# cliarie/radix-join

Hardware: AMD Instinct MI355X
Metric: probe_tuples_per_sec (higher is better)
Workload: dtype int32

## Files before the change

### radix-join_amd/csrc/rj_context.hip

```cpp
#include <dlfcn.h>

#include <chrono>
#include <cstdlib>

#include "rj_internal.hpp"

namespace rj {

[[noreturn]] void launch_failed(const char* kernel, const char* what, bool unsupported) {
    throw_fmt(unsupported ? RJ_ERR_UNSUPPORTED : RJ_ERR_DEVICE, "launch %s: %s", kernel, what);
}

static int env_int(const char* name, int def) {
    const char* v = getenv(name);
    return v && *v ? atoi(v) : def;
}

void Tuning::from_env() {
    blocked_mid = env_int("RJ_TUNE_BLOCKED_MID", blocked_mid);
    mall_chunk = env_int("RJ_TUNE_MALL_CHUNK", mall_chunk);
    radix_bits = env_int("RJ_TUNE_RADIX_BITS", radix_bits);
    p1_bits = env_int("RJ_TUNE_P1_BITS", p1_bits);
    fine = env_int("RJ_TUNE_FINE", fine);
    pack = env_int("RJ_TUNE_PACK", pack);
    aos3 = env_int("RJ_TUNE_AOS3", aos3);
    aos_mid = env_int("RJ_TUNE_AOS_MID", aos_mid);
    tpg1 = env_int("RJ_TUNE_TPG1", tpg1);
    xcd_split = env_int("RJ_TUNE_XCD_SPLIT", xcd_split);
    tpg2 = env_int("RJ_TUNE_TPG2", tpg2);
    packed_side = env_int("RJ_TUNE_PACKED_SIDE", packed_side);
    xcd_min_rows = env_int("RJ_TUNE_XCD_MIN_ROWS", xcd_min_rows);
    bcast = env_int("RJ_TUNE_BCAST", bcast);
    diag = env_int("RJ_DIAG", diag);
    varchar_dev_rows = env_int("RJ_TUNE_VARCHAR_DEV", varchar_dev_rows);
    vkey_hash_bits = env_int("RJ_DEBUG_VKEY_HASH_BITS", vkey_hash_bits);
    sync_upload = env_int("RJ_SYNC_UPLOAD", sync_upload);
    wide_carry = env_int("RJ_TUNE_WIDE_CARRY", wide_carry);
    fold_owner = env_int("RJ_TUNE_FOLD_OWNER", fold_owner);
    group_grid = env_int("RJ_TUNE_GROUP_GRID", group_grid);
    win_grid = env_int("RJ_TUNE_WIN_GRID", win_grid);
    map_grid = env_int("RJ_TUNE_MAP_GRID", map_grid);
    setop_grid = env_int("RJ_TUNE_SETOP_GRID", setop_grid);
    exchange_timeout_ms = env_int("RJ_EXCHANGE_TIMEOUT_MS", exchange_timeout_ms);
    bringup_timeout_ms = env_int("RJ_BRINGUP_TIMEOUT_MS", bringup_timeout_ms);
    debug_shard_fail = env_int("RJ_DEBUG_SHARD_FAIL", debug_shard_fail);
    debug_shard_fail_rank = env_int("RJ_DEBUG_SHARD_FAIL_RANK", debug_shard_fail_rank);
    if (const char* v = getenv("RJ_DEBUG_POISON"))
        debug_poison = (int)strtol(v, nullptr, 0) & 0x1ff;
}

static size_t round_size(size_t n) {
    const size_t small = 256, big = size_t(2) << 20;
    if (n < (size_t(1) << 20)) return (n + small - 1) / small * small;
    return (n + big - 1) / big * big;
}

void* DevPool::alloc(size_t bytes) {
    size_t need = round_size(bytes ? bytes : 1);
    int    best = -1;
    for (size_t i = 0; i < blocks_.size(); ++i) {
        Block& b = blocks_[i];
        if (!b.free || b.size < need) continue;
        if (b.size > need + need / 2 + (size_t(4) << 20)) continue;
        if (best < 0 || b.size < blocks_[best].size) best = (int)i;
    }
    if (best >= 0) {
        if (poison_) {
            hipError_t e = fill(blocks_[best].p, blocks_[best].size);
            if (e != hipSuccess) throw_fmt(RJ_ERR_DEVICE, "RJ_DEBUG_POISON: fill on alloc failed: %s", hipGetErrorString(e));
        }
        blocks_[best].free = false;
        in_use_ += blocks_[best].size;
        cached_ -= blocks_[best].size;
        return blocks_[best].p;
    }
    void*      p = nullptr;
    auto       t0 = std::chrono::steady_clock::now();
    hipError_t e = hipMalloc(&p, need);
    if (e != hipSuccess) {
        (void)hipGetLastError();
        trim();
        ++n_trim;
        e = hipMalloc(&p, need);
        if (e != hipSuccess) {
            (void)hipGetLastError();
            throw_fmt(RJ_ERR_NOMEM, "hipMalloc(%zu bytes) failed: %s", need, hipGetErrorString(e));
        }
    }
    ++n_malloc;
    malloc_ms += std::chrono::duration<double, std::milli>(std::chrono::steady_clock::now() - t0).count();
    if (poison_) {
        hipError_t f = fill(p, need);
        if (f != hipSuccess) {
            (void)hipFree(p);
            throw_fmt(RJ_ERR_DEVICE, "RJ_DEBUG_POISON: fill on alloc failed: %s", hipGetErrorString(f));
        }
    }
    blocks_.push_back({p, need, false});
    in_use_ += need;
    return p;
}

hipError_t DevPool::fill(void* p, size_t bytes) {
    Context* c = owner_;
    int      prev = -1;
    if (hipGetDevice(&prev) != hipSuccess) prev = -1;
    hipError_t e = prev == c->device ? hipSuccess : hipSetDevice(c->device);
    for (hipStream_t s : {c->stream, c->aux, c->copy_stream})
        if (e == hipSuccess && s) e = hipStreamSynchronize(s);
    if (e == hipSuccess) e = hipMemsetAsync(p, poison_ & 0xff, bytes, c->stream);
    if (e == hipSuccess) e = hipStreamSynchronize(c->stream);
    if (e == hipSuccess) {
        n_fill_.fetch_add(1, std::memory_order_relaxed);
        fill_bytes_.fetch_add(bytes, std::memory_order_relaxed);
    } else {
        (void)hipGetLastError();
    }
    if (prev >= 0 && prev != c->device) (void)hipSetDevice(prev);
    return e;
}

void DevPool::release(void* p) {
    if (!p) return;
    for (Block& b : blocks_)
        if (b.p == p && !b.free) {
            if (poison_ & 0x100) (void)fill(b.p, b.size);
            b.free = true;
            in_use_ -= b.size;
            cached_ += b.size;
            return;
        }
}

void DevPool::trim() {
    std::vector<Block> keep;
    for (Block& b : blocks_) {
        if (b.free) {
            (void)hipFree(b.p);
            cached_ -= b.size;
        } else {
            keep.push_back(b);
        }
    }
    blocks_.swap(keep);
}

DevPool::~DevPool() {
    for (Block& b : blocks_) (void)hipFree(b.p);
}

Buf::Buf(Context* c, size_t n) : ctx(c), bytes(n) { p = c->pool.alloc(n); }
Buf::~Buf() {
    if (ctx && p) ctx->pool.release(p);
}

hipEvent_t Profiler::get_event() {
    if (!spare_.empty()) {
        hipEvent_t e = spare_.back();
        spare_.pop_back();
        return e;
    }
    hipEvent_t e;
    RJ_HIP(hipEventCreate(&e));
    return e;
}

static bool hot_kernel(const char* n) {
    return !strncmp(n, "pass", 4) || !strncmp(n, "join_build", 10) || !strncmp(n, "exchange", 8);
}

bool Profiler::timed(const char* name, hipEvent_t* start, hipEvent_t* stop) {
    if (!on || (level < 2 && !hot_kernel(name))) return false;
    Rec r{name, get_event(), get_event()};
    open_.push_back(r);
    *start = r.a;
    *stop = r.b;
    return true;
}

void Profiler::drain() {
    if (open_.empty()) return;
    RJ_HIP(hipStreamSynchronize(stream));
    for (Rec& r : open_) {
        float ms = 0;
// ... 161 lines not shown
```

### radix-join_amd/csrc/rj_device.hpp

```cpp
#pragma once
#include <stdint.h>

namespace rj {

constexpr uint32_t PAGE_BYTES = 8192;
constexpr uint32_t ROWS32 = 1984;
constexpr uint32_t ROWS64 = 1007;
constexpr uint32_t HDR32 = 4;
constexpr uint32_t HDR64 = 8;

enum ColKind : int32_t {
    COL_NONE  = 0,
    COL_PAGED = 1,
    COL_DENSE = 2,
    COL_IOTA  = 3
};

struct ColRef {
    const uint8_t* ptr;
    const uint8_t* valid;
    int32_t        kind;
    int32_t        width;
};

enum CarryMode : int32_t {
    CARRY_NONE   = 0,
    CARRY_ROWIDX = 1,
    CARRY_COLUMN = 2,
    CARRY_WIDE   = 3
};

enum WideLayout : int32_t {
    WIDE_NONE = 0,
    WIDE_32S  = 1,
    WIDE_64_32 = 2
};

struct TupleSrc {
    ColRef   key;
    ColRef   carry;
    uint32_t n_rows;
    int32_t  carry_mode;
    int32_t  key_f64;
    int32_t  prehashed;
    int32_t  wide;
    int32_t  pad;
    ColRef   carry2, carry3;
};

constexpr int MAX_WORDS = 4;
struct Words {
    uint32_t* w[MAX_WORDS];
};

#ifndef RJ_PT_THREADS
#define RJ_PT_THREADS 1024
#endif
#ifndef RJ_PT_ITEMS
#define RJ_PT_ITEMS 16
#endif
constexpr int PT_THREADS = RJ_PT_THREADS;
constexpr int PT_ITEMS   = RJ_PT_ITEMS;
constexpr int PT_TILE    = PT_THREADS * PT_ITEMS;
constexpr uint32_t PT_ALL_ITEMS = PT_ITEMS >= 32 ? 0xffffffffu : ((1u << (PT_ITEMS & 31)) - 1u);
#ifndef RJ_PT_CAPBITS
#define RJ_PT_CAPBITS 9
#endif
constexpr int PT_CAPBITS = RJ_PT_CAPBITS;
constexpr int PT_MAXF    = 1 << PT_CAPBITS;
constexpr int PT_MAXBITS = 9;
static_assert(PT_CAPBITS >= PT_MAXBITS && PT_CAPBITS <= 10, "fan-out capacity");
constexpr int PT_FINEBITS = 15;
constexpr int LDS_BYTES  = 160 * 1024;
static_assert(PT_THREADS >= PT_MAXF, "thread d scans digit d");
constexpr int PT_DUMMY   = 32;
static_assert(PT_TILE * 8 + (3 * PT_MAXF + PT_DUMMY) * 4 + (PT_THREADS / 64) * 4 <= LDS_BYTES,
              "scatter tile does not fit the 160 KiB of LDS");
static_assert((4 << PT_FINEBITS) <= LDS_BYTES, "fine histogram does not fit the LDS");
constexpr uint32_t PT_RANK_MASK = PT_TILE <= 16384 ? 0x3fffu : 0x7fffu;
static_assert(PT_TILE <= 32768 && PT_ITEMS % 2 == 0, "ranks and LDS positions are packed two per register");
static_assert(PT_ITEMS % 4 == 0 && PT_ITEMS <= 32, "full tiles are loaded as 16-byte vectors; one mask bit per item");

struct PassParams {
    const uint32_t* seg_off;
    const uint32_t* grp_start;
    uint32_t        nseg;
    uint32_t        n;
    uint32_t        shift;
    uint32_t        fanout_log2;
    uint32_t        tiles_per_group;
    uint32_t*       hist;
    uint32_t*       cursor;
    uint32_t        xcd_log2;
    uint32_t        xcd_remap;
    uint16_t*       side_out;
    uint32_t        next_shift, next_mask;
    const uint32_t* seg_end;
    uint32_t        oseg_shift;
    uint32_t        grp_base;
    uint32_t        hi_shift, lo_bits;
};

__host__ __device__ inline uint32_t pass_digit(const PassParams& pp, uint32_t w, uint32_t mask) {
    if (pp.hi_shift) return (((w >> pp.shift) & ((1u << pp.lo_bits) - 1u)) | ((w >> pp.hi_shift) << pp.lo_bits)) & mask;
    return (w >> pp.shift) & mask;
}

#ifndef RJ_JN_THREADS
#define RJ_JN_THREADS 512
#endif
#ifndef RJ_JN_SPT
#define RJ_JN_SPT 8
#endif
#ifndef RJ_JN_CAP
#define RJ_JN_CAP 8192
#endif
constexpr int      JN_THREADS = RJ_JN_THREADS;
constexpr int      JN_SPT     = RJ_JN_SPT;
constexpr int      JN_SUB     = JN_THREADS * JN_SPT;
constexpr int      JN_CAP     = RJ_JN_CAP;
constexpr int      JN_RMAX    = JN_CAP / 2;
constexpr int      JN_RPT     = (JN_RMAX + JN_THREADS - 1) / JN_THREADS;
constexpr int jn_threads(int table_words) { return table_words >= 3 ? 2 * JN_THREADS : JN_THREADS; }
constexpr int jn_min_waves(int table_words) {
    int blocks = (160 * 1024) / (JN_CAP * 4 * table_words + JN_CAP + 1024);
    int w = blocks * jn_threads(table_words) / 256;
    return w > 8 ? 8 : (w < 1 ? 1 : w);
}
static_assert(JN_RPT % 4 == 0 && JN_SPT % 4 == 0, "tuples are loaded as 16-byte vectors");
static_assert(JN_CAP * 4 * 4 + JN_CAP + 1024 <= 160 * 1024, "a four-array join table does not fit the LDS");
#ifndef RJ_JN_PPW
#define RJ_JN_PPW 1
#endif
#ifndef RJ_JN_PPW3
#define RJ_JN_PPW3 4
#endif
constexpr int jn_ppw(int table_words) { return table_words >= 3 ? RJ_JN_PPW3 : RJ_JN_PPW; }
#ifndef RJ_JN_HEAVY
#define RJ_JN_HEAVY 65536
#endif
constexpr uint32_t JN_HEAVY   = RJ_JN_HEAVY;
constexpr uint32_t JN_TARGET_BUILD = JN_RMAX * 3 / 4;

enum StreamMode : int32_t {
    ST_NONE    = 0,
    ST_DENSE32 = 1,
    ST_DENSE64 = 2,
    ST_PAGED32 = 3,
    ST_PAGED64 = 4,
    ST_DENSE96 = 5
};

struct OutStream {
    uint8_t* base;
    int32_t  mode;
    int32_t  pad;
};

struct JoinParams {
    Words           R, S;
    const uint32_t* offR;
    const uint32_t* offS;
    uint32_t        NP;
    uint32_t        radix_bits;
    uint32_t        n_pass;
    uint32_t        pass_bits[4];
    OutStream       key, bc, pc;
    unsigned long long* out_cursor;
    uint64_t        out_cap;
    const uint32_t* heavy_tasks;
    const uint32_t* n_heavy;
    uint32_t        heavy_grid;
    int32_t         packR, packS;
    int32_t         aosR, aosS;
    int32_t         pad;
    unsigned long long* diag;
};

struct SplitParams {
    const uint32_t* rec;
    uint32_t        cw;
    int32_t         n_cols;
    int32_t         valid_word;
    int32_t         pad;
    struct Col {
        uint8_t* out;
        uint8_t* valid;
        int32_t  word;
        int32_t  width;
        int32_t  valid_bit;
        int32_t  paged;
    } col[3];
};

struct VcRow {
    uint32_t page;
    uint32_t beg;
    uint32_t len;
};
struct VcPage {
    uint32_t first;
    uint32_t nr;
    uint32_t kind;
};
constexpr uint32_t VC_CHUNK = 512;

struct BcastParams {
    TupleSrc        R, S;
    OutStream       key, bc, pc;
    unsigned long long* out_cursor;
    uint64_t        out_cap;
};

struct FilterParams {
    TupleSrc        F, P;
    Words           Fw, Pw;
    const uint32_t* offF;
    const uint32_t* offP;
    uint32_t        NP;
    uint32_t        radix_bits;
    int32_t         packP, aosP;
    const uint32_t* heavy_tasks;
    const uint32_t* n_heavy;
    uint32_t        heavy_grid;
    int32_t         anti;
    int32_t         keyless;
    int32_t         pad;
    OutStream       key, pc;
    unsigned long long* out_cursor;
    uint64_t        out_cap;
};

constexpr uint32_t OUTER_NO_ROW = 0xffffffffu;
struct OuterParams {
    TupleSrc        B, P;
    Words           Bw, Pw;
    const uint32_t* offB;
    const uint32_t* offP;
    uint32_t        NP;
    uint32_t        radix_bits;
    int32_t         packB, aosB;
    int32_t         packP, aosP;
    const uint32_t* heavy_tasks;
    const uint32_t* n_heavy;
    uint32_t        heavy_grid;
    int32_t         keyless;
    uint32_t        pad_bc;
    int32_t         pad;
    OutStream       key, bc, pc;
    unsigned long long* out_cursor;
    uint64_t        out_cap;
};

struct FullParams {
    OuterParams     o;
    uint32_t*       flags;
    uint32_t        pad_pc;
    int32_t         use_flags;
};
// ... 160 lines not shown
```

### radix-join_amd/csrc/rj_exec.hip

```cpp
#include <algorithm>
#include <chrono>
#include <cstdlib>
#include <functional>
#include <set>

#include "rj_expr.hpp"
#include "rj_internal.hpp"
#include "rj_xplan.hpp"

namespace rj {

const NodeKind* node_kind(int kind) {
    static const NodeKind kinds[] = {
        {RJ_NODE_SCAN, "a scan", "RJ_NODE_SCAN", 0, true},
        {RJ_NODE_JOIN, "a join", "RJ_NODE_JOIN", 2, true},
        {RJ_NODE_SEMI, "a semi join", "RJ_NODE_SEMI", 2, false},
        {RJ_NODE_ANTI, "an anti join", "RJ_NODE_ANTI", 2, false},
        {RJ_NODE_OUTER, "an outer join", "RJ_NODE_OUTER", 2, false},
        {RJ_NODE_FULL, "a full outer join", "RJ_NODE_FULL", 2, false},
        {RJ_NODE_AGG, "an aggregation", "RJ_NODE_AGG", 1, false},
        {RJ_NODE_SELECT, "a selection", "RJ_NODE_SELECT", 1, false},
        {RJ_NODE_SORT, "a sort", "RJ_NODE_SORT", 1, false},
        {RJ_NODE_GROUP, "a grouping", "RJ_NODE_GROUP", 1, false},
        {RJ_NODE_WINDOW, "a window", "RJ_NODE_WINDOW", 1, false},
        {RJ_NODE_MAP, "a map", "RJ_NODE_MAP", 1, false},
        {RJ_NODE_SETOP, "a set operation", "RJ_NODE_SETOP", 2, false},
    };
    for (const NodeKind& k : kinds)
        if (k.kind == kind) return &k;
    return nullptr;
}

namespace {

template <class T>
T* ptr(const BufP& b) {
    return b ? b->as<T>() : nullptr;
}

struct DCol {
    int32_t        type = RJ_INT32;
    int32_t        kind = COL_NONE;
    int32_t        width = 4;
    const uint8_t* ptr = nullptr;
    const uint8_t* valid = nullptr;
    BufP           hold, hold_valid;
    int            vc_table = -1, vc_col = -1;
    const TableColumn* tcol = nullptr;
    ColRef ref() const { return ColRef{ptr, valid, kind, width}; }
};

struct Rel {
    uint64_t          n = 0;
    std::vector<DCol> cols;
};

struct Parted {
    int      NW = 0;
    BufP     wbuf[MAX_WORDS];
    Words    w{};
    BufP     off;
    uint32_t NP = 0;
    std::vector<uint32_t> pbits;
    bool     packed = false;
    bool     aos3 = false;
    uint64_t n_tuples = 0;
};

struct WordSrc {
    Words    w{};
    uint64_t n = 0;
    bool     packed = false;
};

struct PassShape {
    uint32_t        hi_shift = 0, lo_bits = 0;
    const uint32_t* seg_begin = nullptr;
    const uint32_t* seg_end = nullptr;
    uint32_t        nseg = 0;
    uint32_t        oseg_shift = 0;
    const uint32_t* oseg_off = nullptr;
    uint32_t        n_oseg = 0;
    std::vector<uint32_t> prior_bits;
};

struct JoinSpec {
    bool                  build_left = true;
    uint64_t              left_attr = 0, right_attr = 0;
    std::vector<uint64_t> out_idx;
    std::vector<int32_t>  out_type;
    bool                  prehashed = false;
    int                   forced_bits = 0;
    uint32_t              top_bits_taken = 0;
};

JoinSpec join_spec(const rj_node& n, int forced_bits) {
    JoinSpec js;
    js.build_left = n.build_left != 0;
    js.left_attr = n.left_attr;
    js.right_attr = n.right_attr;
    js.out_idx.assign(n.out_idx, n.out_idx + n.n_out);
    js.out_type.assign(n.out_type, n.out_type + n.n_out);
    js.forced_bits = forced_bits;
    return js;
}

struct JoinKind {
    int         node;
    const char* name;
    bool        emits_unmatched;
    bool        build_optional, probe_optional;
    int         attempts;
};
const JoinKind& join_kind(int node) {
    static const JoinKind kinds[] = {
        {RJ_NODE_JOIN, "join", false, false, false, 2},
        {RJ_NODE_SEMI, "semi join", false, false, false, 1},
        {RJ_NODE_ANTI, "anti join", true, false, false, 1},
        {RJ_NODE_OUTER, "outer join", true, true, false, 2},
        {RJ_NODE_FULL, "full outer join", true, true, true, 2},
    };
    for (const JoinKind& k : kinds)
        if (k.node == node) return k;
    throw_fmt(RJ_ERR_ARG, "bad node kind");
}

uint32_t ceil_log2(uint64_t v) {
    uint32_t b = 0;
    while ((uint64_t(1) << b) < v) ++b;
    return b;
}

class Exec {
   public:
    Exec(Context* c, const rj_plan* p, Table* const* t, uint64_t nt, int fl)
        : ctx(c), plan(p), tables(t), n_tables(nt), flags(fl), L(c->launch()) {}
    void set_fetch(TableFetch* f) { fetch = f; }

    Result* run() {
        if (!plan || plan->root >= plan->n_nodes) throw_fmt(RJ_ERR_ARG, "bad plan root");
        std::unique_ptr<Result> res(new rj_result());
        res->ctx = ctx;
        const rj_node& root = plan->nodes[plan->root];
        if (root.kind == RJ_NODE_SCAN) {
            root_scan(root, *res);
        } else {
            (void)node(plan->root, res.get(), 0);
        }
        ctx->sync();
        return res.release();
    }

    Result* run_tuples(const rj_tuples* b, const rj_tuples* p, uint32_t skip_rank_bits) {
        std::unique_ptr<Result> res(new rj_result());
        res->ctx = ctx;
        auto mk = [](const rj_tuples* t) {
            Rel r;
            r.n = t->n;
            DCol k = dense_col(RJ_INT32, BufP());
            k.ptr = static_cast<const uint8_t*>(t->key);
            DCol c = k;
            c.ptr = static_cast<const uint8_t*>(t->carry);
            r.cols = {k, c};
            return r;
        };
        if (b->n > 0xfffffff0ull || p->n > 0xfffffff0ull)
            throw_fmt(RJ_ERR_UNSUPPORTED, "more than 2^32 tuples");
        if (b->hashed != p->hashed) throw_fmt(RJ_ERR_ARG, "build/probe disagree on `hashed`");
        Rel      lb = mk(b), rp = mk(p);
        JoinSpec js;
        js.build_left = true;
        js.out_idx = {0, 1, 3};
        js.out_type = {RJ_INT32, RJ_INT32, RJ_INT32};
        js.prehashed = b->hashed != 0;
        if (skip_rank_bits > 16) throw_fmt(RJ_ERR_ARG, "skip_rank_bits > 16");
        js.top_bits_taken = js.prehashed ? skip_rank_bits : 0u;
        (void)join_core(lb, rp, js, res.get());
        ctx->sync();
        return res.release();
    }

    void run_shard(const Table* t, uint64_t key_col, uint64_t carry_col, uint32_t n_ranks,
                   rj_tuples* out, uint64_t* counts) {
        if (n_ranks == 0 || (n_ranks & (n_ranks - 1)) || n_ranks > (1u << PT_MAXBITS))
            throw_fmt(RJ_ERR_UNSUPPORTED, "n_ranks must be a power of two <= %d", 1 << PT_MAXBITS);
        if (key_col >= t->cols.size() || carry_col >= t->cols.size())
            throw_fmt(RJ_ERR_ARG, "column out of range");
        DCol k = table_col(t, (int)key_col), c = table_col(t, (int)carry_col);
        if (k.type != RJ_INT32 || c.type != RJ_INT32)
            throw_fmt(RJ_ERR_UNSUPPORTED, "sharded path carries INT32 key + INT32 payload");
        if (c.valid) throw_fmt(RJ_ERR_UNSUPPORTED, "sharded path: payload column has NULLs");
        TupleSrc src{};
        src.key = k.ref();
        src.carry = c.ref();
        src.n_rows = (uint32_t)t->num_rows;
        src.carry_mode = CARRY_COLUMN;
        if (!out->key || !out->carry) throw_fmt(RJ_ERR_ARG, "rj_shard_partition: null output buffers");
        uint32_t rb = ceil_log2(n_ranks);
        Words    ext{};
        ext.w[0] = static_cast<uint32_t*>(out->key);
        ext.w[1] = static_cast<uint32_t*>(out->carry);
        Parted P = partition(&src, nullptr, 1, 1, rb, rb ? 32 - rb : 31,  true, &ext);
        std::vector<uint32_t> off(n_ranks + 1);
        read_back(off.data(), P.off->p, (n_ranks + 1) * 4);
        for (uint32_t r = 0; r < n_ranks; ++r) counts[r] = off[r + 1] - off[r];
        out->n = off[n_ranks];
        out->hashed = 1;
        out->reserved = 0;
    }

    Context*       ctx;
    const rj_plan* plan;
    Table* const*  tables;
    uint64_t       n_tables;
    int            flags;
    TableFetch*    fetch = nullptr;
    Launch         L;
    std::map<std::pair<const Table*, int>, DCol> decoded_;
    std::map<std::pair<int, int>, std::vector<uint64_t>> vc_dir_;
// ... 55 lines not shown
        void add(uint64_t id, Make&& make) {
            if (!made.count(id)) made[id] = make();
            if (!res) {
                out.cols.push_back(made.at(id));
                return;
            }
            if (!encoded.count(id)) encoded[id] = E->col_to_result(made.at(id), out.n);
            res->cols.push_back(encoded.at(id));
        }
    };

    DCol table_col(const Table* t, int c) {
        const TableColumn& tc = t->cols[c];
        if (tc.skipped) throw_fmt(RJ_ERR_ARG, "column was not uploaded (not referenced by a scan)");
        DCol d = dense_col(tc.type, BufP());
        d.tcol = &tc;
        if (tc.type == RJ_VARCHAR) {
            d.kind = COL_IOTA;
            return d;
        }
        if (t->num_rows == 0) return d;
        if (tc.regular) {
            d.kind = COL_PAGED;
            d.ptr = tc.dev_pages;
            return d;
        }
        auto key = std::make_pair(t, c);
        auto it = decoded_.find(key);
        if (it != decoded_.end()) return it->second;
        uint64_t n = t->num_rows;
        d = new_col(tc.type, n, true);
        d.tcol = &tc;
        RJ_HIP(hipMemsetAsync(d.hold->p, 0, n * d.width, ctx->stream));
        RJ_HIP(hipMemsetAsync(d.hold_valid->p, 0, n, ctx->stream));
        if (tc.n_pages) {
            BufP row_base = ctx->buf((tc.n_pages + 1) * 4);
            launch_scan_bins(L, tc.page_rows->as<uint32_t>(), (uint32_t)tc.n_pages,
                             row_base->as<uint32_t>(), nullptr);
            launch_decode_pages(L, tc.dev_pages, (uint32_t)tc.n_pages, d.width,
                                row_base->as<uint32_t>(), n, d.hold->as<uint8_t>(),
                                d.hold_valid->as<uint8_t>());
        }
        decoded_[key] = d;
        return d;
    }

    const Table* table_of(const rj_node& n) {
        return table_by_id(n.base_table_id);
    }
    const Table* table_by_id(uint64_t id) {
        if (id >= n_tables) throw_fmt(RJ_ERR_ARG, "scan: bad base_table_id");
        return fetch ? fetch->get(id) : tables[id];
    }

    Rel scan(const rj_node& n) {
        const Table* t = table_of(n);
        Rel          r;
        r.n = t->num_rows;
        for (uint64_t k = 0; k < n.n_out; ++k) {
            uint64_t c = n.out_idx[k];
            if (c >= t->cols.size()) throw_fmt(RJ_ERR_ARG, "scan: output attr out of range");
            if (t->cols[c].type != n.out_type[k])
                throw_fmt(RJ_ERR_ARG, "scan: declared type differs from the column's type");
            DCol d = table_col(t, (int)c);
            if (d.type == RJ_VARCHAR) {
                d.vc_table = (int)n.base_table_id;
                d.vc_col = (int)c;
            }
            r.cols.push_back(d);
        }
        return r;
    }

    void root_scan(const rj_node& n, Result& res) {
        const Table* t = table_of(n);
        res.num_rows = t->num_rows;
        for (uint64_t k = 0; k < n.n_out; ++k) {
            uint64_t c = n.out_idx[k];
            if (c >= t->cols.size()) throw_fmt(RJ_ERR_ARG, "scan: output attr out of range");
            const TableColumn& tc = t->cols[c];
            if (tc.type != n.out_type[k])
                throw_fmt(RJ_ERR_ARG, "scan: declared type differs from the column's type");
            ResultColumn rc;
            rc.type = tc.type;
            if (tc.skipped) throw_fmt(RJ_ERR_ARG, "column was not uploaded");
            if (t->num_rows == 0) {
            } else if (tc.type == RJ_VARCHAR) {
                if (vc_directory((int)n.base_table_id, (int)c, t).back() == t->num_rows) {
                    rc.n_pages = tc.vc_pages.size();
                    rc.host_pages.resize(rc.n_pages * PAGE_BYTES);
                    for (uint64_t pg = 0; pg < rc.n_pages; ++pg)
                        memcpy(rc.host_pages.data() + pg * PAGE_BYTES, tc.vc_pages[pg], PAGE_BYTES);
                } else {
                    DCol d = table_col(t, (int)c);
                    d.vc_table = (int)n.base_table_id;
                    d.vc_col = (int)c;
                    BufP rowids = ctx->buf(t->num_rows * 4);
                    launch_gather(L, d.ref(), nullptr, t->num_rows, OutStream{rowids->as<uint8_t>(), ST_DENSE32, 0}, nullptr);
                    varchar_root(rowids->as<uint32_t>(), t->num_rows, d, rc);
                }
            } else if (tc.regular) {
                rc.n_pages = tc.n_pages;
                rc.dev_pages = ctx->buf(tc.n_pages * PAGE_BYTES);
                RJ_HIP(hipMemcpyAsync(rc.dev_pages->p, tc.dev_pages, tc.n_pages * PAGE_BYTES,
                                      hipMemcpyDeviceToDevice, ctx->stream));
            } else {
                rc = col_to_result(table_col(t, (int)c), t->num_rows);
            }
            res.cols.push_back(std::move(rc));
        }
    }

    Rel node(uint64_t idx, Result* root_res, int depth, bool ordered = false) {
        if (idx >= plan->n_nodes) throw_fmt(RJ_ERR_ARG, "bad node index");
        if (depth > 4096) throw_fmt(RJ_ERR_ARG, "plan too deep (cycle?)");
        const rj_node& n = plan->nodes[idx];
        if (n.kind == RJ_NODE_SCAN) return scan(n);
        const NodeKind* nk = node_kind(n.kind);
        if (nk && nk->children == 1) {
            Rel child = node(n.left, nullptr, depth + 1, n.kind == RJ_NODE_MAP && (root_res != nullptr || ordered));
            switch (n.kind) {
            case RJ_NODE_AGG: return agg(child, n, root_res);
            case RJ_NODE_SELECT: return select(child, n, root_res);
            case RJ_NODE_SORT: return sort(child, n, root_res, ordered);
            case RJ_NODE_GROUP: return group(child, n, root_res);
            case RJ_NODE_WINDOW: return window(child, n, root_res);
            case RJ_NODE_MAP: return map(child, n, root_res);
            }
        }
        if (n.kind == RJ_NODE_SETOP) {
            Rel l = node(n.left, nullptr, depth + 1);
            Rel r = node(n.right, nullptr, depth + 1);
            return setop(l, r, n, root_res);
        }
        const JoinKind& K = join_kind(n.kind);
        Rel             l = node(n.left, nullptr, depth + 1);
        Rel             r = node(n.right, nullptr, depth + 1);
        const JoinSpec  js = join_spec(n, ctx->radix_bits_override);
        if (n.kind == RJ_NODE_OUTER) return outer_join(l, r, js, K, root_res);
        if (n.kind == RJ_NODE_FULL) return full_join(l, r, js, K, root_res);
        if (n.kind != RJ_NODE_JOIN) return filter_join(l, r, js, K, root_res);
        return join_core(l, r, js, root_res);
    }

    static uint32_t tiles_per_group(uint64_t tuples_per_segment, uint64_t target_groups) {
        uint64_t k = (tuples_per_segment + (uint64_t)PT_TILE * target_groups - 1) /
                     ((uint64_t)PT_TILE * target_groups);
        return (uint32_t)std::min<uint64_t>(std::max<uint64_t>(k, 1), 8);
    }

    Parted partition(const TupleSrc* srcp, const WordSrc* ws, int KW, int CW, uint32_t bits,
                     uint32_t shift0 = 0, bool single_pass = false, const Words* external = nullptr,
                     const std::function<void(const uint32_t*)>* after_offsets = nullptr,
                     const PassShape* shape = nullptr) {
        Parted P;
        const bool preseg = shape && shape->nseg > 0;
        P.NW = KW + CW;
        const TupleSrc none{};
        const TupleSrc& src = srcp ? *srcp : none;
        const uint64_t  n = ws ? ws->n : src.n_rows;
        uint32_t       passes = single_pass ? 1 : (bits + PT_MAXBITS - 1) / PT_MAXBITS;
        if (passes == 0) passes = 1;
        std::vector<uint32_t> pbits(passes, bits / passes);
        for (uint32_t i = 0; i < bits % passes; ++i) pbits[i]++;
        if (passes == 2 && ctx->tune.p1_bits > 0) {
            uint32_t b1 = (uint32_t)ctx->tune.p1_bits;
            if (b1 < bits && b1 <= PT_CAPBITS && bits - b1 <= PT_CAPBITS) {
                pbits[0] = b1;
                pbits[1] = bits - b1;
            }
        }

        const bool fine = passes == 2 && bits <= (uint32_t)PT_FINEBITS && !external && !shape &&
                          ctx->tune.fine != 0;
        const int pack_mode = ctx->tune.pack;
        P.packed = ws ? ws->packed
                      : (!external && KW == 1 && CW == 1 && (pack_mode == 1 || (pack_mode == 2 && fine)));
        P.aos3 = KW == 1 && CW == 2 && !external && !single_pass && ctx->tune.aos3 != 0;
        const bool aos_mid = P.aos3 && passes >= 2 &&
                             (ctx->tune.aos_mid == 1 || ctx->tune.aos_mid == 3 || (ctx->tune.aos_mid == 2 && fine));
        const bool mid_side = aos_mid && !fine && ctx->tune.aos_mid != 3;
        BufP  A[MAX_WORDS], B[MAX_WORDS], AOS, MID[2], SIDE[2];
        Words wa{}, wb{}, waos{};
        if (P.aos3) {
            AOS = ctx->buf(std::max<uint64_t>(n, 1) * 12);
            waos.w[0] = AOS->as<uint32_t>();
        }
        if (aos_mid) {
            for (uint32_t k = 0; k < std::min<uint32_t>(passes - 1, 2); ++k) {
                MID[k] = ctx->buf(std::max<uint64_t>(n, 1) * 12);
                if (mid_side) SIDE[k] = ctx->buf(std::max<uint64_t>(n, 1) * 2 + 16);
            }
        }
        const bool packed_side = P.packed && !fine && passes >= 2 && ctx->tune.packed_side != 0 &&
                                 n >= (uint64_t)ctx->tune.xcd_min_rows;
        if (packed_side)
            for (uint32_t k = 0; k < std::min<uint32_t>(passes - 1, 2); ++k)
                SIDE[k] = ctx->buf(std::max<uint64_t>(n, 1) * 2 + 16);
        const int pair_word = CW >= 2 ? KW + CW - 2 : -1;
        for (int a = 0; a < (P.packed ? 1 : P.NW); ++a) {
            if (pair_word >= 0 && a == pair_word + 1) continue;
            const uint64_t wbytes = (P.packed || a == pair_word) ? 8 : 4;
            if (external) {
                wa.w[a] = external->w[a];
                continue;
            }
            if ((P.aos3 && passes == 1) || aos_mid) continue;
            A[a] = ctx->buf(n * wbytes + 2048);
            wa.w[a] = A[a]->as<uint32_t>();
            if (passes > (P.aos3 ? 2u : 1u)) {
                B[a] = ctx->buf(n * wbytes + 2048);
                wb.w[a] = B[a]->as<uint32_t>();
            }
        }
        BufP     seg_off;
        uint32_t nseg = 1, shift = shift0;
        Words    cur = ws ? ws->w : Words{}, nxt = (P.aos3 && passes == 1) ? waos : wa;
        bool     cur_is_a = false;
        BufP       fine_off, fine_cursor, coarse_off, coarse_cursor;
        uint32_t tpg_first = tiles_per_group(n, 4096);
        if (ctx->tune.tpg1 > 0) tpg_first = (uint32_t)ctx->tune.tpg1;
        bool fine_xcd = false;
        if (fine) {
            const uint32_t NB = 1u << bits, F1 = 1u << pbits[0], F2 = 1u << pbits[1];
            BufP           fh = ctx->buf((uint64_t)NB * 4);
            const uint64_t tiles = (n + PT_TILE - 1) / PT_TILE;
            uint32_t       fgrid = (uint32_t)std::min<uint64_t>(tiles, (uint64_t)ctx->compute_units());
            fine_xcd = ctx->tune.xcd_split && n >= (uint64_t)ctx->tune.xcd_min_rows && fgrid >= 8;
            if (fine_xcd) fgrid &= ~7u;
            fine_off = ctx->buf(((uint64_t)NB + 1) * 4);
            fine_cursor = ctx->buf((uint64_t)NB * 4);
            coarse_off = ctx->buf(((uint64_t)F1 + 1) * 4);
            coarse_cursor = ctx->buf((uint64_t)F1 * 4 * (fine_xcd ? 8 : 1));
            BufP coarse_x;
            RJ_HIP(hipMemsetAsync(fh->p, 0, (uint64_t)NB * 4, ctx->stream));
            if (fine_xcd) {
                coarse_x = ctx->buf((uint64_t)F1 * 8 * 4);
                RJ_HIP(hipMemsetAsync(coarse_x->p, 0, (uint64_t)F1 * 8 * 4, ctx->stream));
            }
            uint32_t* cx = fine_xcd ? coarse_x->as<uint32_t>() : nullptr;
            if (ws)
                launch_fine_hist_words(L, ws->w, ws->packed, (uint32_t)n, shift0, pbits[0], pbits[1], fgrid,
                                       fh->as<uint32_t>(), fine_xcd ? tpg_first : 0u, cx);
            else
                launch_fine_hist_src(L, src, KW, shift0, pbits[0], pbits[1], fgrid, fh->as<uint32_t>(),
                                     fine_xcd ? tpg_first : 0u, cx);
            launch_scan_fine(L, fh->as<uint32_t>(), F1, F2, fine_off->as<uint32_t>(),
                             fine_cursor->as<uint32_t>(), coarse_off->as<uint32_t>(),
                             coarse_cursor->as<uint32_t>(), cx);
        }
        struct Ev2 {
            hipEvent_t e = nullptr;
            void       make() { RJ_HIP(hipEventCreateWithFlags(&e, hipEventDisableTiming)); }
            ~Ev2() {
                if (e) (void)hipEventDestroy(e);
            }
        } chunk_ev;
        const bool chunk_second = ctx->tune.mall_chunk > 0 && passes == 2 && !fine && !shape && !ws && !external && P.packed &&
                                  !packed_side && ctx->tune.xcd_split && n >= (uint64_t)ctx->tune.xcd_min_rows;
        const bool blocked_mid = ctx->tune.blocked_mid != 0 && P.packed && passes >= 2 && !fine && !shape && !ws && !external &&
                                 !packed_side && !chunk_second;
        for (uint32_t p = 0; p < passes; ++p) {
            const uint32_t F = 1u << pbits[p];
            PassParams     pp{};
            pp.nseg = nseg;
            pp.n = (uint32_t)n;
            pp.shift = shift;
            pp.fanout_log2 = pbits[p];
            uint32_t n_groups;
            BufP     grp_start;
            const bool      first_preseg = p == 0 && preseg;
            const uint32_t  nseg_in = first_preseg ? shape->nseg : nseg;
            const uint32_t  n_oseg = first_preseg ? shape->n_oseg : nseg;
            const uint64_t  bins = (uint64_t)n_oseg * F;
            if (p == 0 && shape && shape->hi_shift) {
                pp.hi_shift = shape->hi_shift;
                pp.lo_bits = shape->lo_bits;
            }
            if (p == 0 && !preseg) {
                pp.tiles_per_group = tpg_first;
                uint64_t gt = (uint64_t)pp.tiles_per_group * PT_TILE;
                n_groups = (uint32_t)((n + gt - 1) / gt);
            } else {
                pp.tiles_per_group = tiles_per_group(n / nseg_in + 1, 16);
                if (P.aos3 && p + 1 == passes) pp.tiles_per_group = std::min<uint32_t>(pp.tiles_per_group, 2u);
                uint64_t gt = (uint64_t)pp.tiles_per_group * PT_TILE;
                if (ctx->tune.tpg2 > 0) {
                    pp.tiles_per_group = (uint32_t)ctx->tune.tpg2;
                    gt = (uint64_t)pp.tiles_per_group * PT_TILE;
                }
                n_groups = (uint32_t)(n / gt + nseg_in);
                if (ctx->tune.xcd_split && n >= (uint64_t)ctx->tune.xcd_min_rows) {
                    pp.xcd_remap = 1;
                    n_groups += 8;
                }
                const uint32_t* in_off = first_preseg ? shape->seg_begin : seg_off->as<uint32_t>();
                grp_start = ctx->buf(((uint64_t)nseg_in + 1) * 4);
                launch_group_table(L, in_off, nseg_in, (uint32_t)gt, grp_start->as<uint32_t>(),
                                   first_preseg ? shape->seg_end : nullptr);
                pp.nseg = nseg_in;
                pp.seg_off = in_off;
                pp.seg_end = first_preseg ? shape->seg_end : nullptr;
                pp.oseg_shift = first_preseg ? shape->oseg_shift : 0u;
                pp.grp_start = grp_start->as<uint32_t>();
            }
            BufP off, hist, cursor;
            if (fine) {
                off = p == 0 ? coarse_off : fine_off;
                cursor = p == 0 ? coarse_cursor : fine_cursor;
                pp.cursor = cursor->as<uint32_t>();
                pp.xcd_log2 = (p == 0 && fine_xcd) ? 3u : 0u;
            } else {
                pp.xcd_log2 = (ctx->tune.xcd_split && p == 0 && !preseg && n >= (uint64_t)ctx->tune.xcd_min_rows) ? 3u : 0u;
                hist = ctx->buf((bins << pp.xcd_log2) * 4);
                off = ctx->buf((bins + 1) * 4);
                cursor = ctx->buf((bins << pp.xcd_log2) * 4);
                RJ_HIP(hipMemsetAsync(hist->p, 0, (bins << pp.xcd_log2) * 4, ctx->stream));
                pp.hist = hist->as<uint32_t>();
                pp.cursor = cursor->as<uint32_t>();
                if (p == 1 && chunk_second) {
                    RJ_HIP(hipEventSynchronize(chunk_ev.e));
                    const uint32_t* hoff = static_cast<const uint32_t*>(ctx->small_pinned());
                    const uint64_t  gt = (uint64_t)pp.tiles_per_group * PT_TILE;
                    std::vector<uint32_t> gstart(nseg_in + 1, 0);
                    for (uint32_t sgi = 0; sgi < nseg_in; ++sgi)
                        gstart[sgi + 1] = gstart[sgi] + (uint32_t)(((uint64_t)(hoff[sgi + 1] - hoff[sgi]) + gt - 1) / gt);
                    Ev2 e_in, e_aux;
                    e_in.make();
                    e_aux.make();
                    hipStream_t aux = ctx->aux_stream();
                    RJ_HIP(hipEventRecord(e_in.e, ctx->stream));
                    RJ_HIP(hipStreamWaitEvent(aux, e_in.e, 0));
                    Launch L2 = L;
                    L2.stream = aux;
                    const uint32_t CH = (uint32_t)ctx->tune.mall_chunk;
                    uint32_t       c = 0;
                    for (uint32_t s0 = 0; s0 < nseg_in; s0 += CH, ++c) {
                        const uint32_t s1 = std::min(nseg_in, s0 + CH), G = gstart[s1] - gstart[s0];
                        const Launch& Lc = (c & 1u) ? L2 : L;
                        PassParams    pc = pp;
                        pc.nseg = s1 - s0;
                        pc.seg_off = pp.seg_off + s0;
                        pc.grp_start = pp.grp_start + s0;
                        pc.grp_base = gstart[s0];
                        pc.hist = pp.hist + (size_t)s0 * F;
                        pc.cursor = pp.cursor + (size_t)s0 * F;
                        const uint32_t grid = pp.xcd_remap ? ((G + 7u) & ~7u) : G;
                        if (G) launch_pass_hist_packed(Lc, cur.w[0], pc, grid);
                        launch_scan_segments(Lc, pc.hist, pc.seg_off, pc.nseg, F, 0, off->as<uint32_t>() + (size_t)s0 * F, pc.cursor);
                        if (G) launch_pass_scatter_packed(Lc, cur.w[0], pc, grid, nxt.w[0]);
                    }
                    RJ_HIP(hipEventRecord(e_aux.e, aux));
                    RJ_HIP(hipStreamWaitEvent(ctx->stream, e_aux.e, 0));
                    seg_off = off;
                    nseg = (uint32_t)bins;
                    shift += pbits[p];
                    cur = nxt;
                    cur_is_a = (p % 2 == 0);
                    nxt = cur_is_a ? wb : wa;
                    continue;
                }
                if (p == 0 && !ws)
                    launch_pass_hist_src(L, src, KW, pp, n_groups);
                else if ((mid_side || packed_side) && p > 0)
                    launch_pass_hist_digits(L, SIDE[(p - 1) % 2]->as<uint16_t>(), pp, n_groups);
                else if (aos_mid && p > 0)
                    launch_pass_hist_aos3(L, MID[(p - 1) % 2]->as<uint32_t>(), pp, n_groups);
                else if (P.packed && blocked_mid && p > 0)
                    launch_pass_hist_blocked(L, cur.w[0], pp, n_groups);
                else if (P.packed)
                    launch_pass_hist_packed(L, cur.w[0], pp, n_groups);
                else
                    launch_pass_hist_dense(L, cur, pp, n_groups);
                launch_scan_segments(L, pp.hist, first_preseg ? shape->oseg_off : (p == 0 ? nullptr : pp.seg_off),
                                     n_oseg, F, pp.xcd_log2, off->as<uint32_t>(), pp.cursor);
            }
            if (p == 0 && after_offsets) (*after_offsets)(off->as<uint32_t>());
            if (p == 0 && chunk_second) {
                if ((bins + 1) * 4 > Context::SMALL_PINNED / 4) throw_fmt(RJ_ERR_DEVICE, "chunked pass: too many segments");
                RJ_HIP(hipMemcpyAsync(ctx->small_pinned(), off->p, (bins + 1) * 4, hipMemcpyDeviceToHost, ctx->stream));
                chunk_ev.make();
                RJ_HIP(hipEventRecord(chunk_ev.e, ctx->stream));
            }
            if (aos_mid) {
                const bool last = p + 1 == passes;
                Words      o{};
                o.w[0] = last ? waos.w[0] : MID[p % 2]->as<uint32_t>();
                if (!last && mid_side) {
                    pp.side_out = SIDE[p % 2]->as<uint16_t>();
                    pp.next_shift = shift + pbits[p];
                    pp.next_mask = (1u << pbits[p + 1]) - 1u;
                }
                if (p == 0 && !ws)
                    launch_pass_scatter_src(L, src, KW, CW, pp, n_groups, o, true);
                else if (p == 0)
                    launch_pass_scatter_dense(L, cur, P.NW, KW, pp, n_groups, o, true);
                else
                    launch_pass_scatter_aos3(L, MID[(p - 1) % 2]->as<uint32_t>(), pp, n_groups, o.w[0]);
                nxt = o;
            } else if (P.packed) {
                if (packed_side && p + 1 < passes) {
                    pp.side_out = SIDE[p % 2]->as<uint16_t>();
                    pp.next_shift = shift + pbits[p];
                    pp.next_mask = (1u << pbits[p + 1]) - 1u;
                }
                const bool blk_out = blocked_mid && p + 1 < passes;
                if (p == 0 && !ws)
                    launch_pass_scatter_src_packed(L, src, pp, n_groups, nxt.w[0], blk_out);
                else if (blocked_mid)
                    launch_pass_scatter_blocked(L, cur.w[0], pp, n_groups, nxt.w[0], blk_out);
                else
                    launch_pass_scatter_packed(L, cur.w[0], pp, n_groups, nxt.w[0]);
            } else if (p == 0 && !ws) {
                launch_pass_scatter_src(L, src, KW, CW, pp, n_groups, nxt, P.aos3 && p + 1 == passes);
            } else {
                launch_pass_scatter_dense(L, cur, P.NW, pair_word, pp, n_groups, nxt,
                                          P.aos3 && p + 1 == passes);
            }
            seg_off = off;
            nseg = (uint32_t)bins;
            shift += pbits[p];
            cur = nxt;
            cur_is_a = (p % 2 == 0);
            nxt = cur_is_a ? wb : wa;
            if (P.aos3 && p + 2 == passes) nxt = waos;
            if (aos_mid) {
            }
        }
        P.w = cur;
        for (int a = 0; a < P.NW; ++a) P.wbuf[a] = cur_is_a ? A[a] : B[a];
        if (P.aos3) P.wbuf[0] = AOS;
        P.off = seg_off;
        P.NP = nseg;
        P.pbits = pbits;
        if (shape && !shape->prior_bits.empty()) P.pbits.insert(P.pbits.begin(), shape->prior_bits.begin(), shape->prior_bits.end());
        P.n_tuples = n;
        return P;
    }

    struct Side {
        Rel*          rel = nullptr;
        uint64_t      key_col = 0;
        std::set<int> need;
        int           carry_mode = CARRY_NONE;
        int           carry_col = -1;
        int           CW = 0;
        BufP          stream;
        int           stream_mode = ST_NONE;
        std::vector<int> wide_cols;
        int              wide = WIDE_NONE;
        int              valid_word = -1;
        BufP             vword;
        struct WideOut {
            BufP values, valid;
            int  mode = ST_NONE;
        };
        std::map<int, WideOut> wide_out;
        uint64_t null_mask = 0;
        bool     shared = false;
        bool     optional = false;
        bool     nullable(int c) const {
            if (optional || rel->cols[c].valid != nullptr) return true;
            return shared && (c >= 64 || ((null_mask >> c) & 1u));
        }
    };
    static uint64_t null_columns(const Rel& r) {
        uint64_t m = 0;
        for (size_t c = 0; c < r.cols.size() && c < 64; ++c)
            if (r.cols[c].valid != nullptr) m |= 1ull << c;
        return m;
    }

    static uint64_t pages_for(uint64_t rows, int width) {
        uint64_t rf = width == 4 ? ROWS32 : ROWS64;
        return (rows + rf - 1) / rf;
    }

    Rel empty_rel(const int32_t* types, uint64_t n_types, Result* root_res) {
        Rel r;
        r.n = 0;
        if (root_res) root_res->num_rows = 0;
        for (uint64_t k = 0; k < n_types; ++k) {
            r.cols.push_back(dense_col(types[k], BufP()));
            if (!root_res) continue;
            ResultColumn rc;
            rc.type = types[k];
            root_res->cols.push_back(std::move(rc));
        }
        return r;
    }
    Rel empty_rel(const rj_node& n, Result* root_res) { return empty_rel(n.out_type, n.n_out, root_res); }
    Rel empty_rel(const JoinSpec& js, Result* root_res) { return empty_rel(js.out_type.data(), js.out_type.size(), root_res); }

    struct JoinState {
        Side     ls, rs;
        bool     build_left = true, is_root = false, f64 = false, need_key_stream = false;
        bool     type_mismatch = false;
        size_t   lw = 0, rw = 0;
        int      KW = 1;
        uint64_t cap_hint = 0;
        const JoinKind* kind = nullptr;
        bool vkey = false;
        struct VKey {
            Rel            rel;
            BufP           rows, hash, valid;
            const uint8_t* pages = nullptr;
            uint32_t       n_pages = 0;
        } vk[2];
        Side&    bs() { return build_left ? ls : rs; }
        Side&    ps() { return build_left ? rs : ls; }
    };

    void join_prepare(Rel& left, Rel& right, const JoinSpec& js, bool is_root, JoinState& st, const JoinKind& K,
                      const uint64_t* shared_nulls = nullptr) {
        st.kind = &K;
        const size_t lw = left.cols.size(), rw = right.cols.size();
        st.lw = lw;
        st.rw = rw;
        st.is_root = is_root;
        st.build_left = js.build_left;
        if (js.left_attr >= lw || js.right_attr >= rw)
            throw_fmt(RJ_ERR_ARG, "join: key attr out of range");
        for (size_t k = 0; k < js.out_idx.size(); ++k) {
            if (js.out_idx[k] >= lw + rw) throw_fmt(RJ_ERR_ARG, "join: output attr out of range");
            const DCol& c = js.out_idx[k] < lw ? left.cols[js.out_idx[k]]
                                               : right.cols[js.out_idx[k] - lw];
            if (c.type != js.out_type[k])
                throw_fmt(RJ_ERR_ARG, "join: declared type differs from the child column's type");
        }
        Side &ls = st.ls, &rs = st.rs;
        ls.rel = &left;
        ls.key_col = js.left_attr;
        rs.rel = &right;
        rs.key_col = js.right_attr;
        if (shared_nulls) {
            ls.shared = rs.shared = true;
            ls.null_mask = shared_nulls[0];
            rs.null_mask = shared_nulls[1];
        }
        const DCol& bk = st.bs().rel->cols[st.bs().key_col];
        const DCol& pk = st.ps().rel->cols[st.ps().key_col];
        if (bk.type < RJ_INT32 || bk.type > RJ_VARCHAR) throw_fmt(RJ_ERR_ARG, "Unsupported join type");
        st.type_mismatch = pk.type != bk.type;
        st.vkey = bk.type == RJ_VARCHAR && !st.type_mismatch;
        st.KW = bk.type == RJ_INT32 ? 1 : 2;
        st.f64 = bk.type == RJ_FP64;
        const bool key_stream_ok =
            K.node == RJ_NODE_JOIN ||
            (!st.type_mismatch && !(K.emits_unmatched && st.ps().rel->cols[st.ps().key_col].valid));
        st.bs().optional = K.build_optional;
        st.ps().optional = K.probe_optional;
        for (size_t k = 0; k < js.out_idx.size(); ++k) {
            bool  is_left = js.out_idx[k] < lw;
            Side& s = is_left ? ls : rs;
            int   c = (int)(is_left ? js.out_idx[k] : js.out_idx[k] - lw);
            if ((uint64_t)c == s.key_col && !st.vkey && key_stream_ok && !s.optional)
                st.need_key_stream = true;
            else
                s.need.insert(c);
        }
        for (Side* s : {&ls, &rs}) {
            if (st.vkey) {
                s->carry_mode = CARRY_ROWIDX;
                s->CW = 1;
            } else if (s->need.empty()) {
                s->carry_mode = CARRY_NONE;
                s->CW = 0;
            } else if (s->need.size() == 1 && !s->nullable(*s->need.begin())) {
                s->carry_mode = CARRY_COLUMN;
                s->carry_col = *s->need.begin();
                s->CW = s->rel->cols[s->carry_col].width / 4;
            } else if (plan_wide_carry(*s, st.KW)) {
                s->carry_mode = CARRY_WIDE;
            } else {
                s->carry_mode = CARRY_ROWIDX;
                s->CW = 1;
            }
        }
        st.cap_hint = std::max(left.n, right.n);
    }

    bool plan_wide_carry(Side& s, int KW, bool honour_switch = true) {
        if ((honour_switch && !ctx->tune.wide_carry) || s.need.empty()) return false;
        int  words = 0, n64 = 0;
        bool any_null = false;
        for (int c : s.need) {
            const DCol& col = s.rel->cols[c];
            if (col.width != 4 && col.width != 8) return false;
            words += col.width / 4;
            n64 += col.width == 8;
            any_null = any_null || s.nullable(c);
        }
        if (any_null) ++words;
        if (words < 2 || words > MAX_WORDS - KW || n64 > 1 || (n64 == 1 && words != 3)) return false;
        s.wide_cols.clear();
        for (int c : s.need)
            if (s.rel->cols[c].width == 8) s.wide_cols.push_back(c);
        for (int c : s.need)
            if (s.rel->cols[c].width == 4) s.wide_cols.push_back(c);
        s.wide = n64 ? WIDE_64_32 : WIDE_32S;
        s.valid_word = any_null ? words - 1 : -1;
        s.CW = words;
        return true;
    }

    void prepare_wide(Side& s) {
        if (s.carry_mode != CARRY_WIDE || s.valid_word < 0 || s.rel->n == 0) return;
        const uint8_t* v[3] = {nullptr, nullptr, nullptr};
        for (size_t i = 0; i < s.wide_cols.size() && i < 3; ++i) v[i] = s.rel->cols[s.wide_cols[i]].valid;
        s.vword = ctx->buf(s.rel->n * 4);
        launch_pack_validity(L, v[0], v[1], v[2], (uint32_t)s.rel->n, s.vword->as<uint32_t>());
    }

    uint32_t join_bits(const JoinSpec& js, uint64_t build_n, uint32_t top_bits_taken = 0) {
        uint32_t bits = js.forced_bits > 0 ? (uint32_t)js.forced_bits
                                           : ceil_log2((build_n + JN_TARGET_BUILD - 1) / JN_TARGET_BUILD);
        if (js.forced_bits <= 0 && bits > 2 * PT_MAXBITS &&
            (build_n >> (2 * PT_MAXBITS)) <= (uint64_t)(JN_RMAX * 0.95))
            bits = 2 * PT_MAXBITS;
        bits = std::min<uint32_t>(std::max<uint32_t>(bits, 1), 21);
        if (top_bits_taken && bits > 32 - top_bits_taken) bits = 32 - top_bits_taken;
        return bits;
    }

    TupleSrc make_src(const JoinState& st, const Side& s, const JoinSpec& js) {
        TupleSrc src{};
        src.key = s.rel->cols[s.key_col].ref();
        src.n_rows = (uint32_t)s.rel->n;
        src.carry_mode = s.carry_mode;
        if (s.carry_mode == CARRY_COLUMN) {
            src.carry = s.rel->cols[s.carry_col].ref();
            if (src.carry.kind == COL_IOTA) src.carry_mode = CARRY_ROWIDX;
        }
        if (s.carry_mode == CARRY_WIDE) {
            ColRef refs[3] = {};
            size_t k = 0;
            for (int c : s.wide_cols) refs[k++] = s.rel->cols[c].ref();
            if (s.valid_word >= 0)
                refs[k++] = ColRef{ptr<uint8_t>(s.vword), nullptr, COL_DENSE, 4};
            src.wide = s.wide;
            src.carry = refs[0];
            src.carry2 = refs[1];
            src.carry3 = refs[2];
        }
        src.key_f64 = st.f64 ? 1 : 0;
        src.prehashed = js.prehashed ? 1 : 0;
        return src;
    }


    bool broadcast_form(JoinState& st, const JoinSpec& js) const {
        const uint64_t nb = st.bs().rel->n;
        return (nb <= (uint64_t)JN_RMAX && js.forced_bits <= 0 && !js.prehashed && ctx->tune.bcast != 0) || nb == 0 ||
               st.type_mismatch;
    }
    uint32_t stride_grid(uint64_t rows) const {
        return (uint32_t)std::min<uint64_t>((rows + JN_SUB - 1) / JN_SUB, (uint64_t)ctx->compute_units() * 8);
    }

    struct CoParts {
        Parted   B, P;
        BufP     tasks;
        uint32_t max_tasks = 0;
    };
    CoParts partition_sides(JoinState& st, const JoinSpec& js, uint32_t bits) {
        CoParts        cp;
        const TupleSrc sb = make_src(st, st.bs(), js), sp = make_src(st, st.ps(), js);
        cp.B = partition(&sb, nullptr, st.KW, st.bs().CW, bits);
        cp.P = partition(&sp, nullptr, st.KW, st.ps().CW, bits);
        return cp;
    }
    void heavy_tasks(CoParts& cp, const BufP& counters) {
        cp.max_tasks = (uint32_t)(2 * (cp.P.n_tuples / JN_HEAVY) + 2);
        cp.tasks = ctx->buf((uint64_t)cp.max_tasks * 12);
        launch_heavy_tasks_zeroed(cp.B, cp.P, cp.tasks, counters, cp.max_tasks);
    }
    CoParts co_partition(JoinState& st, const JoinSpec& js, uint32_t bits, const BufP& counters) {
        CoParts cp = partition_sides(st, js, bits);
        heavy_tasks(cp, counters);
        return cp;
    }
    BufP zeroed_counters() {
        BufP counters = ctx->buf(16);
        RJ_HIP(hipMemsetAsync(counters->p, 0, 16, ctx->stream));
        return counters;
    }
    template <class Params>
    static void set_heavy(Params& p, const CoParts& cp, const BufP& counters, uint32_t bits) {
        p.NP = cp.B.NP;
        p.radix_bits = bits;
        p.heavy_tasks = cp.tasks->as<uint32_t>();
        p.n_heavy = counters->as<uint32_t>() + 2;
        p.heavy_grid = cp.max_tasks;
    }
    static void set_parts(OuterParams& op, const CoParts& cp, const BufP& counters, uint32_t bits) {
        set_heavy(op, cp, counters, bits);
        op.Bw = cp.B.w;
        op.Pw = cp.P.w;
        op.offB = cp.B.off->as<uint32_t>();
        op.offP = cp.P.off->as<uint32_t>();
        op.packB = cp.B.packed ? 1 : 0;
        op.aosB = cp.B.aos3 ? 1 : 0;
        op.packP = cp.P.packed ? 1 : 0;
        op.aosP = cp.P.aos3 ? 1 : 0;
    }

    static OutStream out_stream(const BufP& b, int mode) { return OutStream{ptr<uint8_t>(b), mode, 0}; }
    static OutStream out_stream(const Side& s) { return out_stream(s.stream, s.stream_mode); }
    static uint64_t first_cap(uint64_t rows) { return std::min<uint64_t>(rows + 1024, 0xfffffff0ull); }

    struct Emitted {
        uint64_t        nrows = 0;
        BufP            key_stream;
        int             key_mode = ST_NONE;
        std::set<void*> finished;
    };
    template <class LaunchFn>
    Emitted emit_with_retry(JoinState& st, const BufP& counters, uint64_t cap, LaunchFn&& launch) {
        const JoinKind& K = *st.kind;
        Emitted         e;
        e.key_mode = st.need_key_stream ? stream_mode_of(st.is_root, st.KW * 4, true) : ST_NONE;
        for (int attempt = 1;; ++attempt) {
            e.key_stream = e.key_mode != ST_NONE ? ctx->buf(stream_bytes(e.key_mode, cap)) : BufP();
            for (Side* s : {&st.ls, &st.rs})
                s->stream = s->stream_mode != ST_NONE ? ctx->buf(stream_bytes(s->stream_mode, cap)) : BufP();
            if (K.attempts > 1) RJ_HIP(hipMemsetAsync(counters->p, 0, 8, ctx->stream));
            launch(out_stream(e.key_stream, e.key_mode), cap);
            e.finished.clear();
            finish_paged_streams(st, e, counters, cap);
            unsigned long long h = 0;
            read_back(&h, counters->p, 8);
            e.nrows = h;
            if (e.nrows <= cap) return e;
            if (K.attempts == 1)
                throw_fmt(RJ_ERR_DEVICE, "%s emitted %llu rows out of %llu", K.name, h, (unsigned long long)cap);
            if (e.nrows > 0xfffffff0ull) throw_fmt(RJ_ERR_UNSUPPORTED, "%s result exceeds 2^32 rows (%llu)", K.name, h);
            if (attempt == K.attempts) throw_fmt(RJ_ERR_DEVICE, "%s output overflowed twice", K.name);
            cap = e.nrows;
        }
    }

    Rel join_core(Rel& left, Rel& right, const JoinSpec& js, Result* root_res) {
        if (left.n == 0 || right.n == 0) return empty_rel(js, root_res);
        JoinState st;
        join_prepare(left, right, js, root_res != nullptr, st, join_kind(RJ_NODE_JOIN));
        if (st.type_mismatch) return empty_rel(js, root_res);
        if (st.vkey) hash_varchar_keys(st);
        prepare_wide(st.ls);
        prepare_wide(st.rs);
        Side&          bs = st.bs();
        Side&          ps = st.ps();
        const uint32_t bits = join_bits(js, bs.rel->n, js.top_bits_taken);
        if (ctx->tune.diag >= 2)
            fprintf(stderr, "[rj diag] join build=%llu probe=%llu bits=%u cw=%d/%d\n",
                    (unsigned long long)bs.rel->n, (unsigned long long)ps.rel->n, bits, bs.CW, ps.CW);
        if (broadcast_form(st, js)) return join_finish(st, js, nullptr, bits, root_res);
        CoParts cp = partition_sides(st, js, bits);
        return join_finish(st, js, &cp, bits, root_res);
    }

    Rel join_finish(JoinState& st, const JoinSpec& js, CoParts* cp, uint32_t bits, Result* root_res) {
        Side &    bs = st.bs(), &ps = st.ps();
        const int KW = st.KW;
        BufP counters = ctx->buf(16);
        if (cp) heavy_tasks(*cp, counters);
        plan_carry_streams(st);
        Emitted e = emit_with_retry(st, counters, first_cap(st.cap_hint), [&](const OutStream& key, uint64_t cap) {
            if (!cp) {
                BcastParams bp{};
                bp.R = make_src(st, bs, js);
                bp.S = make_src(st, ps, js);
                bp.key = key;
                bp.bc = out_stream(bs);
                bp.pc = out_stream(ps);
                bp.out_cursor = counters->as<unsigned long long>();
                bp.out_cap = cap;
                launch_join_bcast(L, KW, bs.CW, ps.CW, bp, stride_grid(ps.rel->n));
                return;
            }
            const Parted &PB = cp->B, &PP = cp->P;
            JoinParams    jp{};
            set_heavy(jp, *cp, counters, bits);
            jp.R = PB.w;
            jp.S = PP.w;
            jp.packR = PB.packed ? 1 : 0;
            jp.packS = PP.packed ? 1 : 0;
            jp.aosR = PB.aos3 ? 1 : 0;
            jp.aosS = PP.aos3 ? 1 : 0;
            jp.offR = PB.off->as<uint32_t>();
            jp.offS = PP.off->as<uint32_t>();
            jp.n_pass = (uint32_t)PB.pbits.size();
            for (size_t i = 0; i < PB.pbits.size() && i < 4; ++i) jp.pass_bits[i] = PB.pbits[i];
            jp.key = key;
            jp.bc = out_stream(bs);
            jp.pc = out_stream(ps);
            jp.out_cursor = counters->as<unsigned long long>();
            jp.out_cap = cap;
            BufP diag;
            if (ctx->tune.diag) {
                diag = ctx->buf(16 * 8);
                RJ_HIP(hipMemsetAsync(diag->p, 0, 16 * 8, ctx->stream));
                jp.diag = diag->as<unsigned long long>();
            }
            const uint32_t ppw = join_partitions_per_workgroup(KW, bs.CW, jp);
            launch_join(L, KW, bs.CW, ps.CW, jp, cp->max_tasks + (PB.NP + ppw - 1) / ppw);
            if (diag) {
                unsigned long long hd[16];
                read_back(hd, diag->p, sizeof hd);
                static const char* names[] = {"loads issued", "table clear", "build", "count/probe",
                                              "prefix+barrier", "reserve", "emit"};
                double tot = 0;
                for (int i = 0; i < 7; ++i) tot += (double)hd[i];
                fprintf(stderr, "[rj diag] join phases (cycles of thread 0, summed over %u workgroups):\n", PB.NP);
                for (int i = 0; i < 7; ++i)
                    fprintf(stderr, "[rj diag]   %-16s %6.1f %%  %8.0f cyc/wg\n", names[i],
                            100.0 * hd[i] / tot, (double)hd[i] / PB.NP);
            }
        });
        if (st.vkey && e.nrows) e.nrows = verify_varchar_pairs(st, e.nrows);
        return join_assemble(st, js, e, root_res);
    }

    Rel filter_join(Rel& left, Rel& right, const JoinSpec& js, const JoinKind& K, Result* root_res) {
        const bool   anti = K.node == RJ_NODE_ANTI;
        Rel&         fil = js.build_left ? left : right;
        Rel&         pre = js.build_left ? right : left;
        const size_t lw = left.cols.size();
        for (uint64_t o : js.out_idx)
            if (o < lw + right.cols.size() && (o < lw) == js.build_left)
                throw_fmt(RJ_ERR_ARG, "%s: output attr %llu names a column of the filter side", K.name,
                          (unsigned long long)o);
        const uint64_t fattr = js.build_left ? js.left_attr : js.right_attr;
        if (fattr < fil.cols.size() && fil.cols[fattr].type == RJ_VARCHAR)
            throw_fmt(RJ_ERR_UNSUPPORTED, "%s on a VARCHAR key", K.name);
        if (pre.n == 0 || (!anti && fil.n == 0)) return empty_rel(js, root_res);
        JoinState st;
        join_prepare(left, right, js, root_res != nullptr, st, K);
        if (st.type_mismatch && !anti) return empty_rel(js, root_res);
        Side&     fs = st.bs();
        Side&     ps = st.ps();
        const int KW = st.KW;
        prepare_wide(ps);
        plan_carry_streams(st);
        const bool     bcast = broadcast_form(st, js);
        const uint32_t bits = join_bits(js, fs.rel->n);
        if (ctx->tune.diag >= 2)
            fprintf(stderr, "[rj diag] %s filter=%llu preserved=%llu %s bits=%u cw=%d\n", K.name,
                    (unsigned long long)fs.rel->n, (unsigned long long)ps.rel->n, bcast ? "broadcast" : "partitioned",
                    bits, ps.CW);

        FilterParams fp{};
        fp.anti = anti ? 1 : 0;
        fp.keyless = st.type_mismatch ? 1 : 0;
        fp.P = make_src(st, ps, js);
        if (bcast && !fp.keyless) fp.F = make_src(st, fs, js);
        BufP counters = zeroed_counters();
        fp.out_cursor = counters->as<unsigned long long>();
        CoParts cp;
        if (!bcast) {
            cp = co_partition(st, js, bits, counters);
            set_heavy(fp, cp, counters, bits);
            fp.Fw = cp.B.w;
            fp.Pw = cp.P.w;
            fp.offF = cp.B.off->as<uint32_t>();
            fp.offP = cp.P.off->as<uint32_t>();
            fp.packP = cp.P.packed ? 1 : 0;
            fp.aosP = cp.P.aos3 ? 1 : 0;
        }
        Emitted e = emit_with_retry(st, counters, ps.rel->n, [&](const OutStream& key, uint64_t cap) {
            fp.key = key;
            fp.pc = out_stream(ps);
            fp.out_cap = cap;
            if (bcast) {
                launch_filter_bcast(L, KW, ps.CW, fp, stride_grid(ps.rel->n));
            } else {
                launch_filter_join(L, KW, ps.CW, fp, cp.max_tasks + cp.B.NP);
                if (anti && (fp.P.key.valid || fp.P.key_f64))
                    launch_filter_nullkeys(L, KW, ps.CW, fp, stride_grid(ps.rel->n));
            }
        });
        return join_assemble(st, js, e, root_res);
    }

    Rel outer_join(Rel& left, Rel& right, const JoinSpec& js, const JoinKind& K, Result* root_res) {
        Rel&           opt = js.build_left ? left : right;
        Rel&           pre = js.build_left ? right : left;
        const uint64_t oattr = js.build_left ? js.left_attr : js.right_attr;
        if (oattr < opt.cols.size() && opt.cols[oattr].type == RJ_VARCHAR)
            throw_fmt(RJ_ERR_UNSUPPORTED, "%s on a VARCHAR key", K.name);
        if (pre.n == 0) return empty_rel(js, root_res);
        JoinState st;
        join_prepare(left, right, js, root_res != nullptr, st, K);
        return outer_probe(st, js, root_res);
    }

    Rel full_join(Rel& left, Rel& right, const JoinSpec& js_in, const JoinKind& K, Result* root_res) {
        for (int side = 0; side < 2; ++side) {
            const Rel&     r = side == 0 ? left : right;
            const uint64_t a = side == 0 ? js_in.left_attr : js_in.right_attr;
            if (a < r.cols.size() && r.cols[a].type == RJ_VARCHAR)
                throw_fmt(RJ_ERR_UNSUPPORTED, "%s on a VARCHAR key", K.name);
        }
        if (left.n == 0 && right.n == 0) {
            JoinState chk;
            join_prepare(left, right, js_in, root_res != nullptr, chk, K);
            refuse_varchar_outputs(chk);
            return empty_rel(js_in, root_res);
        }
        JoinSpec js = js_in;
        if ((js.build_left ? right : left).n == 0) js.build_left = !js.build_left;
        JoinState st;
        join_prepare(left, right, js, root_res != nullptr, st, K);
        return outer_probe(st, js, root_res);
    }

    static void refuse_varchar_outputs(JoinState& st) {
        for (Side* s : {&st.ls, &st.rs})
            for (int c : s->need) {
                if (!s->optional || s->rel->cols[c].type != RJ_VARCHAR) continue;
                if (st.kind->probe_optional)
                    throw_fmt(RJ_ERR_UNSUPPORTED,
                              "full outer join: a VARCHAR column in the output is not supported (%s child column %d)",
                              s == &st.ls ? "left" : "right", c);
                throw_fmt(RJ_ERR_UNSUPPORTED,
                          "outer join: a VARCHAR column of the optional side in the output is not supported "
                          "(child column %d)", c);
            }
    }

    Rel outer_probe(JoinState& st, const JoinSpec& js, Result* root_res) {
        const bool full = st.kind->probe_optional;
        Side&      bs = st.bs();
        Side&      ps = st.ps();
        const int  KW = st.KW;
        refuse_varchar_outputs(st);
        prepare_wide(bs);
        prepare_wide(ps);
        plan_carry_streams(st);
        const bool     bcast = broadcast_form(st, js);
        const uint32_t bits = join_bits(js, bs.rel->n);
        if (ctx->tune.diag >= 2)
            fprintf(stderr, "[rj diag] %s %s=%llu %s=%llu %s bits=%u cw=%d/%d\n", st.kind->name, full ? "built" : "optional",
                    (unsigned long long)bs.rel->n, full ? "probed" : "preserved", (unsigned long long)ps.rel->n,
                    bcast ? "broadcast" : "partitioned", bits, bs.CW, ps.CW);

        FullParams   fp{};
        OuterParams& op = fp.o;
        op.keyless = st.type_mismatch ? 1 : 0;
        op.pad_bc = bs.carry_mode == CARRY_ROWIDX ? OUTER_NO_ROW : 0u;
        op.P = make_src(st, ps, js);
        if (full || !op.keyless) op.B = make_src(st, bs, js);
        BufP counters = zeroed_counters();
        op.out_cursor = counters->as<unsigned long long>();
        CoParts cp;
        if (!bcast) {
            cp = co_partition(st, js, bits, counters);
            set_parts(op, cp, counters, bits);
        }
        BufP flags;
        if (full) {
            fp.pad_pc = ps.carry_mode == CARRY_ROWIDX ? OUTER_NO_ROW : 0u;
            const uint64_t flag_bytes = ((bcast ? (uint64_t)JN_RMAX : cp.B.n_tuples) / 32 + 2) * 4;
            flags = ctx->buf(flag_bytes);
            RJ_HIP(hipMemsetAsync(flags->p, 0, flag_bytes, ctx->stream));
            fp.flags = flags->as<uint32_t>();
            fp.use_flags = bcast ? 1 : 0;
        }
        const uint32_t probe_grid = stride_grid(ps.rel->n), build_grid = stride_grid(bs.rel->n);
        const uint64_t rows0 = std::max(st.cap_hint, full ? bs.rel->n + ps.rel->n : ps.rel->n);
        Emitted e = emit_with_retry(st, counters, first_cap(rows0), [&](const OutStream& key, uint64_t cap) {
            op.key = key;
            op.bc = out_stream(bs);
            op.pc = out_stream(ps);
            op.out_cap = cap;
            const bool probe_dropped = !bcast && (op.P.key.valid || op.P.key_f64);
            if (!full) {
                if (bcast)
                    launch_outer_bcast(L, KW, bs.CW, ps.CW, op, probe_grid);
                else
                    launch_outer_join(L, KW, bs.CW, ps.CW, op, cp.max_tasks + cp.B.NP);
                if (probe_dropped) launch_outer_nullkeys(L, KW, ps.CW, op, probe_grid);
            } else if (bcast) {
                launch_full_bcast(L, KW, bs.CW, ps.CW, fp, probe_grid);
                launch_full_buildrows(L, KW, bs.CW, fp, build_grid);
            } else {
                launch_full_join(L, KW, bs.CW, ps.CW, fp, cp.max_tasks + cp.B.NP);
                launch_full_unmatched(L, KW, bs.CW, fp, build_grid);
                if (probe_dropped) launch_outer_nullkeys(L, KW, ps.CW, op, probe_grid);
                if (op.B.key.valid || op.B.key_f64) launch_full_buildrows(L, KW, bs.CW, fp, build_grid);
            }
        });
        return join_assemble(st, js, e, root_res);
    }

    struct AggOut {
        uint32_t func;
        int      col;
        int      slot;
    };
    uint32_t agg_bits(uint64_t rows) const {
        uint32_t bits = ctx->radix_bits_override > 0 ? (uint32_t)ctx->radix_bits_override
                                                     : ceil_log2((rows + AGG_TARGET - 1) / AGG_TARGET);
        return std::min<uint32_t>(std::max<uint32_t>(bits, 1), 21);
    }
    Rel agg(Rel& child, const rj_node& n, Result* root_res) {
        const size_t cw = child.cols.size();
        if (n.left_attr >= cw) throw_fmt(RJ_ERR_ARG, "aggregation: key attr out of range");
        const DCol& kc = child.cols[n.left_attr];
        if (kc.type != RJ_INT32 && kc.type != RJ_INT64)
            throw_fmt(RJ_ERR_UNSUPPORTED, "aggregation on %s key: group keys are INT32 or INT64",
                      kc.type == RJ_FP64 ? "an FP64" : "a VARCHAR");
        Side s;
        s.rel = &child;
        s.key_col = n.left_attr;
        std::vector<AggOut> outs;
        for (uint64_t k = 0; k < n.n_out; ++k) {
            const uint32_t func = RJ_AGG_FUNC(n.out_idx[k]);
            const uint64_t col = RJ_AGG_COL(n.out_idx[k]);
            const int32_t  type = n.out_type[k];
            if (func == RJ_AGG_FSUM) throw_fmt(RJ_ERR_ARG, "aggregation: RJ_AGG_FSUM is RJ_NODE_GROUP's, this kind has no FP64 sum");
            if (func > RJ_AGG_MAX) throw_fmt(RJ_ERR_ARG, "aggregation: unknown function code %u", func);
            int32_t expect = RJ_INT64;
            if (func == RJ_AGG_COUNT_STAR) {
                if (col != 0) throw_fmt(RJ_ERR_ARG, "aggregation: COUNT(*) takes no column");
            } else {
                if (col >= cw) throw_fmt(RJ_ERR_ARG, "aggregation: output attr out of range");
                const DCol& c = child.cols[col];
                if (func == RJ_AGG_KEY) {
                    if (col != n.left_attr) throw_fmt(RJ_ERR_ARG, "aggregation: RJ_AGG_KEY names another column than the key");
                    expect = kc.type;
                } else {
                    if (c.type != RJ_INT32 && c.type != RJ_INT64)
                        throw_fmt(RJ_ERR_UNSUPPORTED, "aggregation over %s column (child column %llu): INT32 and INT64 only",
                                  c.type == RJ_FP64 ? "an FP64" : "a VARCHAR", (unsigned long long)col);
                    if (func == RJ_AGG_MIN || func == RJ_AGG_MAX) expect = c.type;
                    s.need.insert((int)col);
                }
            }
            if (type != expect) throw_fmt(RJ_ERR_ARG, "aggregation: declared type differs from the function's result type");
            outs.push_back(AggOut{func, (int)col, -1});
        }
        const int KW = kc.type == RJ_INT32 ? 1 : 2;
        if (s.need.empty()) {
            s.carry_mode = CARRY_NONE;
            s.CW = 0;
        } else if (s.need.size() == 1 && !s.nullable(*s.need.begin())) {
            s.carry_mode = CARRY_COLUMN;
            s.carry_col = *s.need.begin();
            s.CW = child.cols[s.carry_col].width / 4;
            s.wide_cols = {s.carry_col};
        } else if (plan_wide_carry(s, KW, false)) {
            s.carry_mode = CARRY_WIDE;
        } else {
            int words = 0;
            bool any_null = false;
            for (int c : s.need) {
                words += child.cols[c].width / 4;
                any_null = any_null || s.nullable(c);
            }
            throw_fmt(RJ_ERR_UNSUPPORTED,
                      "aggregation: the aggregated columns take %d carry words; at most %d travel behind an %s key (every "
                      "distinct column its width, one more word if any is nullable, at most one 64-bit column next to "
                      "another word)",
                      words + (any_null ? 1 : 0), MAX_WORDS - KW, KW == 1 ? "INT32" : "INT64");
        }
        if (child.n == 0) return empty_rel(n, root_res);
        check_rows(child);
        for (AggOut& o : outs)
            for (size_t i = 0; i < s.wide_cols.size(); ++i)
                if (o.func >= RJ_AGG_COUNT && s.wide_cols[i] == o.col) o.slot = (int)i;

        AggParams ap{};
        ap.n_cols = (int32_t)s.wide_cols.size();
        ap.valid_word = s.valid_word;
        bool need_key = false, need_rows = false;
        {
            int word = 0;
            for (int i = 0; i < ap.n_cols; ++i) {
                const DCol& c = child.cols[s.wide_cols[i]];
                ap.col[i].word = word;
                ap.col[i].width = c.width;
                ap.col[i].valid_bit = s.valid_word >= 0 ? i : -1;
                word += c.width / 4;
            }
            for (const AggOut& o : outs) {
                need_key = need_key || o.func == RJ_AGG_KEY;
                need_rows = need_rows || o.func == RJ_AGG_COUNT_STAR;
                if (o.slot < 0) continue;
                const bool nullable = s.nullable(o.col);
                uint32_t&  need = ap.col[o.slot].need;
                if (o.func == RJ_AGG_COUNT || nullable) need |= AGG_NEED_COUNT;
                if (o.func == RJ_AGG_SUM) need |= AGG_NEED_SUM;
                if (o.func == RJ_AGG_MIN) need |= AGG_NEED_MIN;
                if (o.func == RJ_AGG_MAX) need |= AGG_NEED_MAX;
            }
        }
        prepare_wide(s);
        const TupleSrc src = make_src(JoinState(), s, JoinSpec());
        const uint32_t bits = agg_bits(child.n);
        const uint64_t cap = child.n + 1;
        if (ctx->tune.diag >= 2)
            fprintf(stderr, "[rj diag] aggregation rows=%llu bits=%u cw=%d cols=%d\n", (unsigned long long)child.n, bits, s.CW,
                    ap.n_cols);

        struct Arrays {
            BufP key, keyvalid, rows, nn[AGG_MAX_COLS], sum[AGG_MAX_COLS], mn[AGG_MAX_COLS], mx[AGG_MAX_COLS];
        } O, M;
        auto fill = [](AggArrays& a, const Arrays& b) {
            a.key = ptr<uint8_t>(b.key);
            a.rows = ptr<unsigned long long>(b.rows);
            for (int i = 0; i < AGG_MAX_COLS; ++i) {
                a.nn[i] = ptr<unsigned long long>(b.nn[i]);
                a.sum[i] = ptr<unsigned long long>(b.sum[i]);
                a.mn[i] = ptr<long long>(b.mn[i]);
                a.mx[i] = ptr<long long>(b.mx[i]);
            }
        };
        if (need_key) O.key = ctx->buf(cap * KW * 4);
        if (need_key && kc.valid) O.keyvalid = ctx->buf(cap);
        if (need_rows) O.rows = ctx->buf(cap * 8);
        for (int i = 0; i < ap.n_cols; ++i) {
            if (ap.col[i].need & AGG_NEED_COUNT) O.nn[i] = ctx->buf(cap * 8);
            if (ap.col[i].need & AGG_NEED_SUM) O.sum[i] = ctx->buf(cap * 8);
            if (ap.col[i].need & AGG_NEED_MIN) O.mn[i] = ctx->buf(cap * 8);
            if (ap.col[i].need & AGG_NEED_MAX) O.mx[i] = ctx->buf(cap * 8);
        }
        fill(ap.out, O);
        ap.out_keyvalid = ptr<uint8_t>(O.keyvalid);
        ap.out_cap = cap;
        ap.src = src;

        uint64_t nrows = 0;
        for (int attempt = 0;; ++attempt) {
            BufP counters = zeroed_counters();
            Parted P = partition(&src, nullptr, KW, s.CW, bits);
            const uint32_t max_tasks = (uint32_t)(2 * (P.n_tuples / JN_HEAVY) + 2);
            BufP           tasks = ctx->buf((uint64_t)max_tasks * 12);
            launch_heavy_tasks(L, P.off->as<uint32_t>(), P.off->as<uint32_t>(), P.NP, tasks->as<uint32_t>(),
                               counters->as<uint32_t>() + 2, max_tasks);
            uint32_t n_heavy = 0;
            read_back(&n_heavy, counters->as<uint32_t>() + 2, 4);
            n_heavy = std::min(n_heavy, max_tasks);
            uint64_t heavy_tuples = std::min<uint64_t>(P.n_tuples, (uint64_t)n_heavy * JN_HEAVY);
            if (attempt == 0) heavy_tuples = std::min<uint64_t>(heavy_tuples, 1u << 20);
// ... 1831 lines not shown
```

### radix-join_amd/csrc/rj_internal.hpp

```cpp
#pragma once
#include <hip/hip_runtime.h>

#include <atomic>
#include <cstdarg>
#include <cstdio>
#include <cstring>
#include <functional>
#include <map>
#include <memory>
#include <mutex>
#include <stdexcept>
#include <string>
#include <vector>

#include "../../include/rj.h"
#include "rj_comm.hpp"
#include "rj_device.hpp"
#include "rj_kernels.hpp"

namespace rj {

struct Context;

struct Error : std::runtime_error {
// ... 7 lines not shown
    va_start(ap, fmt);
    vsnprintf(buf, sizeof buf, fmt, ap);
    va_end(ap);
    throw Error(code, buf);
}

#define RJ_HIP(expr)                                                                          \
    do {                                                                                      \
        hipError_t _e = (expr);                                                               \
        if (_e != hipSuccess)                                                                 \
            ::rj::throw_fmt(_e == hipErrorOutOfMemory ? RJ_ERR_NOMEM : RJ_ERR_DEVICE,         \
                            "%s failed: %s (%s:%d)", #expr, hipGetErrorString(_e), __FILE__, \
                            __LINE__);                                                        \
    } while (0)

class DevPool {
   public:
    void* alloc(size_t bytes);
    void  release(void* p);
    void     set_poison(Context* owner, int mode) { owner_ = owner, poison_ = mode; }
    int      poison() const { return poison_; }
    uint64_t n_fills() const { return n_fill_.load(std::memory_order_relaxed); }
    uint64_t bytes_filled() const { return fill_bytes_.load(std::memory_order_relaxed); }
    void  trim();
    ~DevPool();
    size_t bytes_in_use() const { return in_use_; }
    size_t bytes_cached() const { return cached_; }
    uint64_t n_malloc = 0, n_trim = 0;
    double   malloc_ms = 0;

   private:
    struct Block {
        void*  p;
        size_t size;
        bool   free;
    };
    std::vector<Block> blocks_;
    size_t             in_use_ = 0, cached_ = 0;
    Context*           owner_ = nullptr;
    int                poison_ = 0;
    std::atomic<uint64_t> n_fill_{0}, fill_bytes_{0};
    hipError_t         fill(void* p, size_t bytes);
};

struct Buf {
    Context* ctx = nullptr;
    void*    p = nullptr;
    size_t   bytes = 0;
    Buf(Context* c, size_t n);
    ~Buf();
    Buf(const Buf&) = delete;
    Buf& operator=(const Buf&) = delete;
    template <class T>
    T* as() const {
        return reinterpret_cast<T*>(p);
    }
};
using BufP = std::shared_ptr<Buf>;

class Profiler {
   public:
    bool        on = false;
    int         level = 1;
    hipStream_t stream = nullptr;
    bool        timed(const char* name, hipEvent_t* start, hipEvent_t* stop);
    void        drain();
    void        reset();
    struct Tot {
        uint64_t launches = 0;
        double   ms = 0;
    };
    std::map<std::string, Tot> totals;
    std::vector<std::string>   order;
    ~Profiler();

   private:
    struct Rec {
        const char* name;
        hipEvent_t  a, b;
    };
    std::vector<Rec>        open_;
    std::vector<hipEvent_t> spare_;
    hipEvent_t              get_event();
};

class LaunchLog {
   public:
    bool on = false;
    void add(const void* kernel);
    void clear();
    void merge_into(std::map<std::string, uint64_t>& out);

   private:
    std::mutex                         mu_;
    std::map<const void*, uint64_t>    counts_;
    std::map<const void*, std::string> names_;
};

struct TableColumn {
    int32_t  type = 0;
    uint64_t n_pages = 0;
    const uint8_t* dev_pages = nullptr;
    BufP           owned;
    bool           regular = false;
    uint64_t       page_rows_total = 0;
    BufP           page_rows;
    std::vector<uint32_t> page_rows_host;
    std::vector<uint8_t>        host_pages;
    std::vector<const uint8_t*> vc_pages;
    mutable BufP vc_dev, vc_dev_dir;
    bool                        skipped = false;
};

struct Table {
    Context*                 ctx = nullptr;
    uint64_t                 num_rows = 0;
    std::vector<TableColumn> cols;
};

struct ResultColumn {
    int32_t              type = 0;
    uint64_t             n_pages = 0;
    BufP                 dev_pages;
    std::vector<uint8_t> host_pages;
    struct Part {
        Context* ctx;
        BufP     pages;
        uint64_t n_pages;
    };
    std::vector<Part> more;
    uint64_t          n_first = 0;
};

struct Result {
    Context*                  ctx = nullptr;
    uint64_t                  num_rows = 0;
    std::vector<ResultColumn> cols;
};

struct Tuning {
    int blocked_mid = 1;
    int mall_chunk = 0;
    int radix_bits = 0;
    int p1_bits = 0;
    int fine = 1;
    int pack = 1;
    int aos3 = 1;
    int aos_mid = 2;
    int tpg1 = 0;
    int packed_side = 0;
    int tpg2 = 0;
    int xcd_min_rows = 40 << 20;
    int xcd_split = 1;
    int bcast = 1;
    int diag = 0;
    int varchar_dev_rows = 200000;
    int vkey_hash_bits = 0;
    int sync_upload = 0;
    int wide_carry = 1;
    int fold_owner = 1;
    int group_grid = 0;
    int map_grid = 0;
    int win_grid = 0;
    int setop_grid = 0;
    int exchange_timeout_ms = 120000;
    int bringup_timeout_ms = 0;
    int debug_shard_fail = 0, debug_shard_fail_rank = 0;
    int debug_poison = 0;
    void from_env();
};

struct Context {
    Tuning      tune;
    int         device = 0;
    hipStream_t stream = nullptr;
    bool        own_stream = false;
    int         radix_bits_override = 0;
    DevPool     pool;
    Profiler    prof;
    LaunchLog   klog;
    std::string last_error;
    void*  pinned = nullptr;
    size_t pinned_bytes = 0;
    static constexpr size_t SMALL_PINNED = 32768;
    void*  pinned_small = nullptr;
    void*  small_pinned();
    hipStream_t copy_stream = nullptr;
    void*       pinned_up = nullptr;
    size_t      pinned_up_bytes = 0;
    hipStream_t upload_stream();
    hipStream_t aux = nullptr;
    hipStream_t aux_stream();
    void*       upload_staging(size_t bytes);
    Launch launch() {
        Launch L;
        L.stream = stream;
        L.self = this;
        L.timed = prof.on ? [](void* s, const char* n, hipEvent_t* a, hipEvent_t* b) {
            return static_cast<Context*>(s)->prof.timed(n, a, b);
        } : (bool (*)(void*, const char*, hipEvent_t*, hipEvent_t*)) nullptr;
        L.logged = klog.on ? [](void* s, const void* k) { static_cast<Context*>(s)->klog.add(k); }
                           : (void (*)(void*, const void*)) nullptr;
        return L;
    }
    std::vector<Context*>  peers;
    std::unique_ptr<Comm>  comm;
    Context*               group = nullptr;
    int                    n_lanes() const { return 1 + (int)peers.size(); }
    Context*               lane(int i) { return i == 0 ? this : peers[(size_t)i - 1]; }
    int   n_cu = 0;
    int   compute_units();
    void  prewarm();
    BufP  buf(size_t bytes) { return std::make_shared<Buf>(this, bytes ? bytes : 16); }
    void* staging(size_t bytes);
    void  sync() { RJ_HIP(hipStreamSynchronize(stream)); }
    ~Context();
};

struct TableFetch {
    virtual Table* get(uint64_t id) = 0;
    virtual ~TableFetch() = default;
};

Result* execute_plan(Context* ctx, const rj_plan* plan, Table* const* tables, uint64_t n_tables,
                     int flags, TableFetch* fetch = nullptr);
Result* join_tuples(Context* ctx, const rj_tuples* build, const rj_tuples* probe,
                    uint32_t skip_rank_bits, int flags);
void    execute_sharded(Context* group, const rj_plan* plan, Table* const* tables, uint64_t n_inputs,
                        int flags, Result** out);
bool    plan_shardable(const rj_plan* plan, std::string* why);
struct NodeKind {
    int         kind;
    const char* name;
    const char* token;
    int         children;
    bool        sharded;
};
const NodeKind* node_kind(int kind);
void    shard_partition(Context* ctx, const Table* t, uint64_t key_col, uint64_t carry_col,
                        uint32_t n_ranks, rj_tuples* out, uint64_t* counts);

struct MapOp;
struct MapExpr {
    int32_t f64;
    bool    nullable;
};
void map_check(const rj_expr_op* ops, uint64_t n_ops, uint64_t n_cols, const int32_t* col_type, const uint8_t* col_nullable,
               std::vector<MapOp>& dev_ops, std::vector<MapExpr>& exprs);
void map_eval_row(const rj_expr_op* ops, uint64_t n_ops, uint64_t n_cols, const int32_t* col_type, const uint64_t* col_bits,
                  const uint8_t* col_null, uint64_t out_cap, uint64_t* out_bits, uint8_t* out_null, int32_t* out_kind, uint64_t* n_out);

Table* table_upload(Context* ctx, const rj_input* host, const std::vector<bool>* col_used = nullptr,
                    bool borrow_varchar = false);
class AsyncUpload : public TableFetch {
   public:
    AsyncUpload(Context* ctx, const rj_plan* plan, const std::vector<bool>& used,
                const std::vector<std::vector<bool>>& col_used);
    ~AsyncUpload() override;
    Table* get(uint64_t id) override;
    double busy_ms() const { return busy_ms_; }
    double wait_ms() const { return wait_ms_; }

   private:
    struct Impl;
    std::unique_ptr<Impl> im_;
    double                busy_ms_ = 0, wait_ms_ = 0;
};
Table* table_adopt(Context* ctx, uint64_t num_rows, uint64_t n_cols, const int32_t* types,
                   const void* const* dev_pages, const uint64_t* n_pages);
void   result_copy_pages(Result* r, uint64_t col, void* const* dst, uint64_t n_dst);
void   upload_host_pages(Context* ctx, const uint8_t* const* pages, uint64_t n_pages, uint8_t* dev);
Result* execute_host_sharded(Context* group, const rj_plan* plan, const std::vector<bool>& used,
                             const std::vector<std::vector<bool>>& col_used);

Table*   table_from_csv(Context* ctx, const char* text, uint64_t n_bytes, uint64_t n_cols, const int32_t* col_type,
                        const rj_filter_op* filter, uint64_t n_filter_ops);
int parse_fp64_host(const char* s, uint64_t n, uint64_t* bits);
uint64_t table_col_pages(const Table* t, uint64_t col);
void     table_copy_pages(Context* ctx, const Table* t, uint64_t col, void* const* dst, uint64_t n_dst);

void parallel_for(size_t n, size_t grain, const std::function<void(size_t, size_t)>& fn);

void copy_page(void* dst, const void* src);
void copy_pages_fence();

void varchar_dir_build(const uint8_t* const* pages, uint64_t n_pages, uint64_t num_rows,
                       std::vector<uint64_t>& row_base);
void varchar_gather_encode(const uint8_t* const* pages, uint64_t n_pages,
                           const std::vector<uint64_t>& row_base, const uint32_t* idx, uint64_t n,
                           std::vector<uint8_t>& out_pages, uint64_t& n_out_pages);

}

struct rj_context : rj::Context {};
struct rj_table : rj::Table {};
struct rj_result : rj::Result {};
```

### radix-join_amd/csrc/rj_kernels.hpp

```cpp
#pragma once
#include <hip/hip_runtime.h>

#include "rj_device.hpp"

namespace rj {

struct Launch {
    hipStream_t stream;
    bool (*timed)(void* self, const char* name, hipEvent_t* start, hipEvent_t* stop);
    void* self;
    void (*logged)(void* self, const void* kernel);
};

[[noreturn]] void launch_failed(const char* kernel, const char* what, bool unsupported);

void launch_page_headers(const Launch& L, const uint8_t* pages, uint32_t n_pages, uint32_t rows_full,
                         uint32_t* page_rows, unsigned long long* flags);
void launch_rows_beyond(const Launch& L, const uint8_t* pages, uint32_t n_pages,
                        const uint32_t* row_base, uint64_t num_rows, unsigned long long* flag);
void launch_decode_pages(const Launch& L, const uint8_t* pages, uint32_t n_pages, int width,
                         const uint32_t* row_base, uint64_t num_rows, uint8_t* values,
                         uint8_t* valid);

void launch_gather(const Launch& L, const ColRef& src, const uint32_t* idx, uint64_t n,
                   const OutStream& dst, uint8_t* dst_valid);
void launch_outer_gather(const Launch& L, const ColRef& src, const uint32_t* idx, uint64_t n, uint8_t* dst,
                         uint8_t* dst_valid);
void launch_finish_pages(const Launch& L, uint8_t* pages, uint64_t n_rows, int width);
void launch_finish_streams(const Launch& L, uint8_t* const* pages, const int* widths, uint32_t n,
                           const unsigned long long* n_rows_dev, uint64_t cap_rows);
void launch_encode_nullable(const Launch& L, const uint8_t* values, const uint8_t* valid,
                            uint64_t n_rows, int width, uint8_t* pages);
void launch_pack_validity(const Launch& L, const uint8_t* v0, const uint8_t* v1, const uint8_t* v2, uint32_t n,
                          uint32_t* out);
void launch_split_records(const Launch& L, const SplitParams& sp, uint64_t n);
void launch_debug_stall(const Launch& L, uint32_t ms);

void launch_scan_bins(const Launch& L, const uint32_t* in, uint32_t n, uint32_t* off,
                      uint32_t* cursor);
void launch_scan_segments(const Launch& L, const uint32_t* hist, const uint32_t* seg_off,
                          uint32_t nseg, uint32_t F, uint32_t xcd_log2, uint32_t* off, uint32_t* cursor);
void launch_group_table(const Launch& L, const uint32_t* seg_off, uint32_t nseg,
                        uint32_t group_tuples, uint32_t* grp_start, const uint32_t* seg_end = nullptr);

void launch_pass_hist_src(const Launch& L, const TupleSrc& src, int key_words, const PassParams& pp,
                          uint32_t n_groups);
void launch_fine_hist_src(const Launch& L, const TupleSrc& src, int key_words, uint32_t shift,
                          uint32_t b1, uint32_t b2, uint32_t grid, uint32_t* fine, uint32_t xcd_tpg = 0,
                          uint32_t* coarse_x = nullptr);
void launch_fine_hist_words(const Launch& L, const Words& in, bool packed, uint32_t n, uint32_t shift,
                            uint32_t b1, uint32_t b2, uint32_t grid, uint32_t* fine, uint32_t xcd_tpg = 0,
                            uint32_t* coarse_x = nullptr);
void launch_scan_fine(const Launch& L, const uint32_t* fine, uint32_t F1, uint32_t F2,
                      uint32_t* off2, uint32_t* cursor2, uint32_t* off1, uint32_t* cursor1,
                      const uint32_t* coarse_x = nullptr);
void launch_pass_scatter_src(const Launch& L, const TupleSrc& src, int key_words, int carry_words,
                             const PassParams& pp, uint32_t n_groups, const Words& out, bool aos3 = false);
void launch_pass_hist_dense(const Launch& L, const Words& in, const PassParams& pp,
                            uint32_t n_groups);
void launch_pass_scatter_dense(const Launch& L, const Words& in, int n_words, int pair_word,
                               const PassParams& pp, uint32_t n_groups, const Words& out, bool aos3 = false);

void launch_pass_hist_digits(const Launch& L, const uint16_t* digits, const PassParams& pp, uint32_t n_groups);
void launch_pass_hist_aos3(const Launch& L, const uint32_t* in_tuples, const PassParams& pp, uint32_t n_groups);
void launch_pass_scatter_aos3(const Launch& L, const uint32_t* in_tuples, const PassParams& pp, uint32_t n_groups,
                              uint32_t* out_tuples);

void launch_pass_hist_packed(const Launch& L, const uint32_t* in_pairs, const PassParams& pp,
                             uint32_t n_groups);
void launch_pass_scatter_src_packed(const Launch& L, const TupleSrc& src, const PassParams& pp,
                                    uint32_t n_groups, uint32_t* out_pairs, bool blocked_out = false);
void launch_pass_hist_blocked(const Launch& L, const uint32_t* in_blocked, const PassParams& pp, uint32_t n_groups);
void launch_pass_scatter_blocked(const Launch& L, const uint32_t* in_blocked, const PassParams& pp, uint32_t n_groups,
                                 uint32_t* out_pairs, bool blocked_out);
void launch_pass_scatter_packed(const Launch& L, const uint32_t* in_pairs, const PassParams& pp,
                                uint32_t n_groups, uint32_t* out_pairs);

void launch_heavy_tasks(const Launch& L, const uint32_t* offR, const uint32_t* offS, uint32_t NP,
                        uint32_t* tasks, uint32_t* n_heavy, uint32_t max_tasks);

uint32_t join_partitions_per_workgroup(int key_words, int cw_build, const JoinParams& jp);
void launch_join(const Launch& L, int key_words, int cw_build, int cw_probe, const JoinParams& jp,
                 uint32_t grid);

void launch_join_bcast(const Launch& L, int key_words, int cw_build, int cw_probe,
                       const BcastParams& bp, uint32_t grid);

void launch_filter_bcast(const Launch& L, int key_words, int cw_preserved, const FilterParams& fp, uint32_t grid);
void launch_filter_join(const Launch& L, int key_words, int cw_preserved, const FilterParams& fp, uint32_t grid);
void launch_filter_nullkeys(const Launch& L, int key_words, int cw_preserved, const FilterParams& fp, uint32_t grid);

void launch_outer_bcast(const Launch& L, int key_words, int cw_optional, int cw_preserved, const OuterParams& op,
                        uint32_t grid);
void launch_outer_join(const Launch& L, int key_words, int cw_optional, int cw_preserved, const OuterParams& op,
                       uint32_t grid);
void launch_outer_nullkeys(const Launch& L, int key_words, int cw_preserved, const OuterParams& op, uint32_t grid);

void launch_full_bcast(const Launch& L, int key_words, int cw_optional, int cw_preserved, const FullParams& fp,
                       uint32_t grid);
void launch_full_join(const Launch& L, int key_words, int cw_optional, int cw_preserved, const FullParams& fp,
                      uint32_t grid);
void launch_full_unmatched(const Launch& L, int key_words, int cw_built, const FullParams& fp, uint32_t grid);
void launch_full_buildrows(const Launch& L, int key_words, int cw_built, const FullParams& fp, uint32_t grid);

void launch_agg_merge_init(const Launch& L, const AggParams& ap, uint32_t grid);
void launch_agg_parts(const Launch& L, int key_words, int carry_words, const AggParams& ap, uint32_t grid);
void launch_agg_nullkey(const Launch& L, int carry_words, const AggParams& ap, uint32_t grid);
void launch_agg_emit(const Launch& L, int key_words, const AggParams& ap, uint32_t grid);
void launch_agg_column(const Launch& L, const unsigned long long* src, const unsigned long long* nn, uint64_t n, int width,
                       uint8_t* dst, uint8_t* dst_valid);

void launch_select(const Launch& L, const SelectProg* prog, uint32_t n_ops, uint32_t n_rows, uint32_t* out_ids,
                   unsigned long long* cursor, uint32_t grid);

struct MapProg;
void launch_map(const Launch& L, const MapProg* prog, uint32_t n_ops, uint32_t n_rows, uint32_t grid);

void launch_sort_encode(const Launch& L, const ColRef& col, const uint32_t* perm, uint32_t n_rows, bool f64, int32_t flags,
                        uint8_t* keys_out, uint32_t* hist, uint32_t grid);
void launch_sort_count(const Launch& L, int mode, const uint8_t* keys, const uint32_t* ids, const uint8_t* valid, uint32_t null_digit,
                       uint32_t n_rows, uint32_t shift, uint32_t* table);
void launch_sort_scan(const Launch& L, const uint32_t* hist, uint32_t n_rows, uint32_t* table);
void launch_sort_scatter(const Launch& L, int mode, const uint8_t* keys_in, const uint32_t* ids_in, const uint8_t* valid,
                         uint32_t null_digit, uint32_t n_rows, uint32_t shift, const uint32_t* table, uint8_t* keys_out,
                         uint32_t* ids_out);
void launch_sort_iota(const Launch& L, uint32_t* out, uint32_t base, uint32_t n);

void launch_group_heads(const Launch& L, const ColRef& col, const uint32_t* perm, uint32_t n_rows, bool f64, bool first, bool last,
                        unsigned long long* masks, uint32_t* tile_heads);
void launch_group_scan(const Launch& L, const uint32_t* tile_heads, uint32_t n_rows, uint32_t* tile_base, uint32_t* total);
void launch_group_keys(const Launch& L, const ColRef& col, const uint32_t* perm, uint32_t n_rows, bool f64,
                       const unsigned long long* masks, const uint32_t* tile_base, uint32_t n_groups, uint8_t* out, uint8_t* out_valid);
void launch_group_reduce(const Launch& L, const ColRef* col, const uint32_t* perm, uint32_t n_rows, bool f64,
                         const unsigned long long* masks, const uint32_t* tile_base, uint32_t n_groups, const GroupAcc& acc,
                         uint32_t max_grid);
void launch_group_column(const Launch& L, const unsigned long long* src, const unsigned long long* nn, uint64_t n, int decode, int width,
                         uint8_t* dst, uint8_t* dst_valid);

uint64_t fsum_scratch_bytes(uint32_t n_rows, uint32_t max_grid);
void     launch_fsum(const Launch& L, const ColRef& col, const uint32_t* perm, uint32_t n_rows, const unsigned long long* masks,
                     const uint32_t* tile_base, uint32_t n_groups, unsigned long long* out, uint32_t max_grid, uint8_t* scratch);

void launch_win_one_head(const Launch& L, unsigned long long* masks, uint32_t n_rows);
void launch_win_ranks(const Launch& L, const unsigned long long* P, const unsigned long long* Q, uint32_t n_rows, const WinMarks& m,
                      const WinRanks& out, uint32_t max_chunk);
void launch_win_scan(const Launch& L, const ColRef& col, const uint32_t* perm, uint32_t n_rows, bool f64, const unsigned long long* P,
                     const WinTails& tails, const WinScan& out, uint32_t max_chunk);
void launch_win_column(const Launch& L, const unsigned long long* src, const uint32_t* nn, const uint32_t* peer_end, uint64_t n, int decode,
                       int width, uint8_t* dst, uint8_t* dst_valid);

void launch_setop_concat(const Launch& L, const ColRef& l, const ColRef& r, uint32_t n_left, uint64_t n, const OutStream& dst,
                         uint8_t* dst_valid);
void launch_setop_runs(const Launch& L, const uint32_t* perm, uint32_t n_rows, uint32_t n_left, const unsigned long long* masks,
                       const uint32_t* tile_base, uint32_t n_runs, uint32_t* tile_left, uint32_t* tile_lbase, const SetopRuns& runs,
                       uint32_t max_grid);
void launch_setop_offsets(const Launch& L, const SetopRuns& runs, uint32_t n_runs, int op, uint32_t* tile_m, uint32_t* tile_mbase,
                          uint32_t* off, uint32_t* total, uint32_t max_grid);
void launch_setop_emit(const Launch& L, const uint32_t* off, uint32_t n_runs, uint32_t n_out, uint32_t* run_of, uint32_t max_grid);

void launch_vc_resolve(const Launch& L, const uint8_t* pages, uint32_t n_pages, const uint32_t* row_base,
                       const uint32_t* rowids, uint32_t n, VcRow* out);
void launch_vc_hash(const Launch& L, const uint8_t* pages, uint32_t n_pages, const uint32_t* row_base,
                    const uint32_t* rowids, uint32_t n, VcRow* rows, uint64_t* hash, uint8_t* valid,
                    uint64_t hash_mask = ~0ull);
void launch_vc_verify(const Launch& L, const uint8_t* pages_b, uint32_t np_b, const VcRow* rows_b,
                      const uint8_t* pages_p, uint32_t np_p, const VcRow* rows_p, const uint32_t* bidx,
                      const uint32_t* pidx, uint32_t n, uint8_t* keep, unsigned long long* n_bad);
void launch_vc_compact(const Launch& L, const uint8_t* keep, const uint32_t* bidx, const uint32_t* pidx, uint32_t n,
                       uint32_t* out_b, uint32_t* out_p, unsigned long long* cursor);
void launch_vc_walk(const Launch& L, const VcRow* rows, uint32_t n, uint32_t* pages_in_chunk,
                    const uint32_t* page_base, VcPage* page_out);
void launch_vc_encode(const Launch& L, const uint8_t* pages, uint32_t n_pages, const VcRow* rows,
                      const VcPage* plist, uint32_t n_out_pages, uint8_t* out);

void prewarm_pages(const Launch& L, uint32_t* zeroed);
void prewarm_partition(const Launch& L, uint32_t* zeroed);
void prewarm_join(const Launch& L, uint32_t* zeroed);
void prewarm_bcast(const Launch& L, uint32_t* zeroed);
void prewarm_filter(const Launch& L, uint32_t* zeroed);
void prewarm_outer(const Launch& L, uint32_t* zeroed);
void prewarm_full(const Launch& L, uint32_t* zeroed);
void prewarm_agg(const Launch& L, uint32_t* zeroed);
void prewarm_select(const Launch& L, uint32_t* zeroed);
void prewarm_varchar_dev(const Launch& L, uint32_t* zeroed);

}
```

### radix-join_amd/csrc/rj_partition.hip

```cpp
#include <hip/hip_ext.h>

#include "rj_kernels.hpp"
#include "rj_kernel_util.hpp"
#include "rj_tuple_util.hpp"

#include <algorithm>
#include <type_traits>

namespace rj {

template <int MODE>
__global__ __launch_bounds__(1024) void k_scan_bins(const uint32_t* in, const uint32_t* in_end, uint32_t n,
                                                    uint32_t div, uint32_t* off, uint32_t* cursor) {
    __shared__ uint32_t s_wsum[16];
    const uint32_t      chunk = (n + 1023u) / 1024u;
    const uint32_t      b = threadIdx.x * chunk;
    const uint32_t      e = min(n, b + chunk);
    uint32_t            sum = 0;
    for (uint32_t i = b; i < e; ++i) {
        uint32_t v = MODE == 0 ? in[i] : ((in_end ? in_end[i] : in[i + 1]) - in[i] + div - 1u) / div;
        sum += v;
    }
    uint32_t total;
    uint32_t run = block_excl_scan(sum, s_wsum, total);
// ... 486 lines not shown
    }
    template <int NW>
    __device__ __forceinline__ uint32_t issue_tile(uint32_t base, uint32_t end,
                                                   uint32_t (&w)[PT_ITEMS][NW]) const {
        static_assert(NW == KW + CW, "word count");
        const bool vec = base + PT_TILE <= end;
        uint32_t   lo[PT_ITEMS], hi[PT_ITEMS];
        const uint32_t tid = tile_tid();
        uint32_t       ok = raw_keys(vec, base, end, lo, hi, tid);
        if constexpr (WIDE == WIDE_32S) {
            uint32_t c0[PT_ITEMS];
            load_col32_any(s.carry, vec, base, end, c0, tid);
#pragma unroll
            for (int j = 0; j < PT_ITEMS; ++j) w[j][KW] = c0[j];
            load_col32_any(s.carry2, vec, base, end, c0, tid);
#pragma unroll
            for (int j = 0; j < PT_ITEMS; ++j) w[j][KW + 1] = c0[j];
            if constexpr (CW == 3) {
                load_col32_any(s.carry3, vec, base, end, c0, tid);
#pragma unroll
                for (int j = 0; j < PT_ITEMS; ++j) w[j][KW + 2] = c0[j];
            }
        } else if constexpr (WIDE == WIDE_64_32) {
            uint32_t c0[PT_ITEMS], c1[PT_ITEMS];
            load_col64(s.carry, vec, base, end, c0, c1, tid);
#pragma unroll
            for (int j = 0; j < PT_ITEMS; ++j) {
                w[j][KW] = c0[j];
                w[j][KW + 1] = c1[j];
            }
            load_col32_any(s.carry2, vec, base, end, c0, tid);
#pragma unroll
            for (int j = 0; j < PT_ITEMS; ++j) w[j][KW + 2] = c0[j];
        } else if constexpr (CW == 1) {
            if (s.carry_mode == CARRY_ROWIDX) {
#pragma unroll
                for (int j = 0; j < PT_ITEMS; ++j) w[j][KW] = item_row(vec, base, j, tid);
            } else {
                uint32_t c0[PT_ITEMS];
                load_col32(s.carry, vec, base, end, c0, tid);
#pragma unroll
                for (int j = 0; j < PT_ITEMS; ++j) w[j][KW] = c0[j];
            }
        } else if constexpr (CW >= 2) {
            uint32_t c0[PT_ITEMS], c1[PT_ITEMS];
            load_col64(s.carry, vec, base, end, c0, c1, tid);
#pragma unroll
            for (int j = 0; j < PT_ITEMS; ++j) {
                w[j][KW] = c0[j];
                w[j][KW + 1] = c1[j];
            }
        }
#pragma unroll
        for (int j = 0; j < PT_ITEMS; ++j) {
            w[j][0] = lo[j];
            if constexpr (KW == 2) w[j][1] = hi[j];
        }
        return ok;
    }
    template <int NW>
    __device__ __forceinline__ uint32_t finish_tile(uint32_t base, uint32_t end, uint32_t ok,
                                                    uint32_t (&w)[PT_ITEMS][NW]) const {
        const bool vec = base + PT_TILE <= end;
        uint32_t   lo[PT_ITEMS], hi[PT_ITEMS];
#pragma unroll
        for (int j = 0; j < PT_ITEMS; ++j) {
            lo[j] = w[j][0];
            hi[j] = KW == 2 ? w[j][KW - 1] : 0u;
        }
        ok = drop_invalid(vec, base, end, ok, tile_tid());
        ok = hash_keys(ok, lo, hi);
#pragma unroll
        for (int j = 0; j < PT_ITEMS; ++j) {
            w[j][0] = lo[j];
            if constexpr (KW == 2) w[j][1] = hi[j];
        }
        return ok;
    }
    template <int NW>
    __device__ __forceinline__ uint32_t load_tile(uint32_t base, uint32_t end,
                                                  uint32_t (&w)[PT_ITEMS][NW]) const {
        return finish_tile<NW>(base, end, issue_tile<NW>(base, end, w), w);
    }
};

__device__ __forceinline__ bool group_range(const PassParams& pp, uint32_t g, uint32_t& seg,
                                            uint32_t& begin, uint32_t& end) {
    const uint32_t gt = pp.tiles_per_group * (uint32_t)PT_TILE;
    if (pp.seg_off == nullptr) {
        seg = 0;
        uint64_t b = (uint64_t)g * gt;
        if (b >= pp.n) return false;
        begin = (uint32_t)b;
        end = (uint32_t)min((uint64_t)pp.n, b + gt);
        return true;
    }
    const uint32_t G = pp.grp_start[pp.nseg] - pp.grp_base;
    if (pp.xcd_remap) {
        const uint32_t per = (G + 7u) >> 3;
        if ((g >> 3) >= per) return false;
        g = (g & 7u) * per + (g >> 3);
    }
    if (g >= G) return false;
    uint32_t lo = 0, hi = pp.nseg;
    while (hi - lo > 1) {
        uint32_t mid = (lo + hi) >> 1;
        if (pp.grp_start[mid] - pp.grp_base <= g)
            lo = mid;
        else
            hi = mid;
    }
    seg = lo >> pp.oseg_shift;
    uint32_t gi = g - (pp.grp_start[lo] - pp.grp_base);
    uint64_t b = (uint64_t)pp.seg_off[lo] + (uint64_t)gi * gt;
    begin = (uint32_t)b;
    end = (uint32_t)min((uint64_t)(pp.seg_end ? pp.seg_end[lo] : pp.seg_off[lo + 1]), b + gt);
    return begin < end;
}

template <class L, class = void>
struct loader_needs_begin : std::false_type {};
template <class L>
struct loader_needs_begin<L, std::enable_if_t<L::kNeedsBegin>> : std::true_type {};

template <class Loader>
__global__ __launch_bounds__(PT_THREADS) void k_pass_hist(Loader ld, PassParams pp) {
    __shared__ uint32_t s_h[PT_MAXF];
    uint32_t            seg, begin, end;
    if (!group_range(pp, blockIdx.x, seg, begin, end)) return;
    const uint32_t F = 1u << pp.fanout_log2, mask = F - 1u;
    for (uint32_t d = threadIdx.x; d < F; d += PT_THREADS) s_h[d] = 0;
    lds_barrier();
    for (uint32_t base = begin; base < end; base += PT_TILE) {
        uint32_t hk[PT_ITEMS];
        uint32_t ok;
        if constexpr (loader_needs_begin<Loader>::value)
            ok = ld.key_tile(base, begin, end, hk);
        else
            ok = ld.key_tile(base, end, hk);
#pragma unroll
        for (int j = 0; j < PT_ITEMS; ++j) {
            if ((ok >> j) & 1u) atomicAdd(&s_h[pass_digit(pp, hk[j], mask)], 1u);
        }
    }
    if constexpr (loader_needs_begin<Loader>::value) {
        uint32_t hx;
        if (ld.extra(begin, end, hx)) atomicAdd(&s_h[pass_digit(pp, hx, mask)], 1u);
    }
    lds_barrier();
    for (uint32_t d = threadIdx.x; d < F; d += PT_THREADS) {
        uint32_t c = s_h[d];
        if (c) atomicAdd(&pp.hist[(((size_t)seg * F + d) << pp.xcd_log2) | (blockIdx.x & ((1u << pp.xcd_log2) - 1u))], c);
    }
}

template <class Loader>
__global__ __launch_bounds__(PT_THREADS) void k_fine_hist(Loader ld, uint32_t n, uint32_t shift,
                                                          uint32_t b1, uint32_t b2,
                                                          uint32_t* fine, uint32_t xcd_tpg,
                                                          uint32_t* coarse_x) {
    __shared__ uint32_t s_f[1u << PT_FINEBITS];
    const uint32_t      NB = 1u << (b1 + b2), m1 = (1u << b1) - 1u, m2 = (1u << b2) - 1u;
    for (uint32_t d = threadIdx.x; d < NB; d += PT_THREADS) s_f[d] = 0;
    lds_barrier();
    const uint32_t tiles = (uint32_t)(((uint64_t)n + PT_TILE - 1) / PT_TILE);
    const uint32_t x = blockIdx.x & 7u, gstride = gridDim.x >> 3;
    uint32_t       gk = blockIdx.x >> 3, gj = 0;
    auto           tile_of = [&](uint32_t k, uint32_t j) { return (x + 8u * k) * xcd_tpg + j; };
    auto           advance = [&](uint32_t t) -> uint32_t {
        if (!xcd_tpg) return t + gridDim.x;
        if (++gj < xcd_tpg && tile_of(gk, gj) < tiles) return tile_of(gk, gj);
        gk += gstride;
        gj = 0;
        const uint64_t nt = (uint64_t)(x + 8ull * gk) * xcd_tpg;
        return nt < tiles ? (uint32_t)nt : 0xffffffffu;
    };
    uint32_t t = xcd_tpg ? tile_of(gk, 0) : blockIdx.x;
    uint32_t lo[PT_ITEMS], hi[PT_ITEMS], raw = 0;
    if (t < tiles) raw = ld.issue_keys(t * (uint32_t)PT_TILE, n, lo, hi);
    while (t < tiles) {
        const uint32_t ok = ld.finish_keys(t * (uint32_t)PT_TILE, n, raw, lo, hi);
        uint32_t       q[PT_ITEMS];
#pragma unroll
        for (int j = 0; j < PT_ITEMS; ++j) {
            const uint32_t h = lo[j] >> shift;
            q[j] = ((h & m1) << b2) | ((h >> b1) & m2);
        }
        const uint32_t t2 = advance(t);
        if (t2 < tiles) raw = ld.issue_keys(t2 * (uint32_t)PT_TILE, n, lo, hi);
#pragma unroll
        for (int j = 0; j < PT_ITEMS; ++j)
            if ((ok >> j) & 1u) atomicAdd(&s_f[q[j]], 1u);
        t = t2;
    }
    lds_barrier();
    for (uint32_t d = threadIdx.x; d < NB; d += PT_THREADS) {
        uint32_t c = s_f[d];
        if (c) atomicAdd(&fine[d], c);
    }
    if (xcd_tpg) {
        const uint32_t F2 = 1u << b2;
        for (uint32_t d1 = threadIdx.x; d1 <= m1; d1 += PT_THREADS) {
            uint32_t sum = 0;
            for (uint32_t i = 0; i < F2; ++i) sum += s_f[d1 * F2 + ((i + d1) & m2)];
            if (sum) atomicAdd(&coarse_x[(d1 << 3) | x], sum);
        }
    }
}

__global__ __launch_bounds__(PT_MAXF) void k_scan_fine(const uint32_t* fine, uint32_t F1,
                                                       uint32_t F2, uint32_t* off2,
                                                       uint32_t* cursor2, uint32_t* off1,
                                                       uint32_t* cursor1, const uint32_t* coarse_x) {
    __shared__ uint32_t s_wsum[PT_MAXF / 64];
    const uint32_t      d1 = blockIdx.x, below = d1 * F2;
    uint32_t            sum = 0;
    if ((F2 & 3u) == 0) {
        const uint4* f4 = reinterpret_cast<const uint4*>(fine);
        for (uint32_t i = threadIdx.x; i < below / 4; i += PT_MAXF) {
            const uint4 v = f4[i];
            sum += v.x + v.y + v.z + v.w;
        }
    } else {
        for (uint32_t i = threadIdx.x; i < below; i += PT_MAXF) sum += fine[i];
    }
    uint32_t base, tot;
    (void)block_excl_scan(sum, s_wsum, base);
    lds_barrier();
    const uint32_t v = threadIdx.x < F2 ? fine[below + threadIdx.x] : 0u;
    const uint32_t ex = block_excl_scan(v, s_wsum, tot);
    if (threadIdx.x < F2) {
        off2[below + threadIdx.x] = base + ex;
        cursor2[below + threadIdx.x] = base + ex;
    }
    if (threadIdx.x == 0) {
        off1[d1] = base;
        if (coarse_x) {
            uint32_t at = base;
            for (uint32_t x = 0; x < 8; ++x) {
                cursor1[(d1 << 3) | x] = at;
                at += coarse_x[(d1 << 3) | x];
            }
        } else {
            cursor1[d1] = base;
        }
        if (d1 + 1 == F1) {
            off1[F1] = base + tot;
            off2[(size_t)F1 * F2] = base + tot;
        }
    }
}

template <int NW>
__device__ __forceinline__ void rank_tile(const PassParams& pp, uint32_t mask, uint32_t ok,
                                          const uint32_t (&w)[PT_ITEMS][NW], uint32_t* s_cnt,
                                          uint32_t (&rk)[PT_ITEMS / 2]) {
    const uint32_t dummy = PT_MAXF + (threadIdx.x & (PT_DUMMY - 1));
    uint32_t       r[PT_ITEMS];
#pragma unroll
    for (int j = 0; j < PT_ITEMS; ++j) {
        const uint32_t m = 0u - ((ok >> j) & 1u);
        r[j] = atomicAdd(&s_cnt[(pass_digit(pp, w[j][0], mask) & m) | (dummy & ~m)], 1u);
    }
#pragma unroll
    for (int j = 0; j < PT_ITEMS; j += 2)
        rk[j / 2] = (r[j] & PT_RANK_MASK) | ((r[j + 1] & PT_RANK_MASK) << 16);
}
constexpr uint32_t PT_NO_POS = 0xffffu;
template <int NW>
__device__ __forceinline__ void place_tile(const PassParams& pp, uint32_t mask, uint32_t ok,
                                           const uint32_t (&w)[PT_ITEMS][NW], const uint32_t* s_base,
                                           uint32_t (&rk)[PT_ITEMS / 2]) {
    uint32_t b[PT_ITEMS];
#pragma unroll
    for (int j = 0; j < PT_ITEMS; ++j) b[j] = s_base[pass_digit(pp, w[j][0], mask)];
#pragma unroll
    for (int j = 0; j < PT_ITEMS; j += 2) {
        const uint32_t p0 = ((ok >> j) & 1u) ? b[j] + (rk[j / 2] & 0xffffu) : PT_NO_POS;
        const uint32_t p1 = ((ok >> (j + 1)) & 1u) ? b[j + 1] + (rk[j / 2] >> 16) : PT_NO_POS;
        rk[j / 2] = p0 | (p1 << 16);
    }
}
__device__ __forceinline__ uint32_t tile_pos(const uint32_t (&ps)[PT_ITEMS / 2], int j) {
    return (j & 1) ? ps[j / 2] >> 16 : ps[j / 2] & 0xffffu;
}

template <class L>
struct is_src_loader : std::false_type {};
template <int KW, int CW, int WIDE>
struct is_src_loader<SrcLoader<KW, CW, WIDE>> : std::true_type {};

template <int NW, class Loader, int PAIR, bool AOS>
__global__ __launch_bounds__(PT_THREADS) void k_pass_scatter(Loader ld, PassParams pp, Words out) {
    static_assert(PAIR < 0 || (PAIR >= 1 && PAIR + 1 < NW), "pair = two carry words behind the key");
    static_assert(!AOS || (NW == 3 && PAIR == 1), "12-byte tuples: one key word + a two-word carry");
    __shared__ uint2    s_stage2[PT_TILE];
    uint32_t* const     s_stage = reinterpret_cast<uint32_t*>(s_stage2);
    __shared__ uint32_t s_cnt[PT_MAXF + PT_DUMMY];
    __shared__ uint32_t s_base[PT_MAXF];
    __shared__ uint32_t s_delta[PT_MAXF];
    __shared__ uint32_t s_wsum[PT_THREADS / 64];
    uint32_t            seg, begin, end;
    if (!group_range(pp, blockIdx.x, seg, begin, end)) return;
    const uint32_t F = 1u << pp.fanout_log2, mask = F - 1u;

    uint32_t run = 0;
    uint32_t w[PT_ITEMS][NW];

    for (uint32_t base = begin; base < end; base += PT_TILE) {
        for (uint32_t d = threadIdx.x; d < F; d += PT_THREADS) s_cnt[d] = 0;
        lds_barrier();

        const uint32_t ok = ld.template load_tile<NW>(base, end, w);
        constexpr bool BATCHED = NW == 3 && PAIR == 1 && is_src_loader<Loader>::value;
        uint32_t       ps[PT_ITEMS / 2];
        uint32_t       dr[PT_ITEMS];
        if constexpr (BATCHED) {
            rank_tile<NW>(pp, mask, ok, w, s_cnt, ps);
        } else {
#pragma unroll
            for (int j = 0; j < PT_ITEMS; ++j) {
                dr[j] = 0xffffffffu;
                if ((ok >> j) & 1u) {
                    uint32_t d = pass_digit(pp, w[j][0], mask);
                    uint32_t r = atomicAdd(&s_cnt[d], 1u);
                    dr[j] = (d << 16) | r;
                }
            }
        }
        lds_barrier();

        uint32_t c = threadIdx.x < F ? s_cnt[threadIdx.x] : 0u;
        if (c) {
            run = atomicAdd(&pp.cursor[(((size_t)seg * F + threadIdx.x) << pp.xcd_log2) |
                                       (blockIdx.x & ((1u << pp.xcd_log2) - 1u))], c);
        }
        uint32_t total;
        uint32_t ex = block_excl_scan(c, s_wsum, total);
        if (threadIdx.x < F) s_base[threadIdx.x] = ex;
        lds_barrier();

        if constexpr (BATCHED) {
            place_tile<NW>(pp, mask, ok, w, s_base, ps);
        } else {
#pragma unroll
            for (int j = 0; j < PT_ITEMS; ++j)
                if (dr[j] != 0xffffffffu) dr[j] = s_base[dr[j] >> 16] + (dr[j] & 0xffffu);
        }

        const uint32_t tid = BATCHED ? tile_tid() : threadIdx.x;
        if constexpr (NW == 3 && PAIR == 1) {
            constexpr uint32_t HALF = PT_TILE / 2;
            uint2* const       s_p = s_stage2;
            uint32_t* const    s_k = reinterpret_cast<uint32_t*>(s_stage2 + HALF);
            if (!BATCHED && threadIdx.x < F) s_delta[threadIdx.x] = run - ex;
#pragma unroll
            for (int h = 0; h < 2; ++h) {
#pragma unroll
                for (int j = 0; j < PT_ITEMS; ++j) {
                    const uint32_t lp = (BATCHED ? tile_pos(ps, j) : dr[j]) - h * HALF;
                    if (lp < HALF) {
                        s_k[lp] = w[j][0];
                        s_p[lp] = make_uint2(w[j][1], w[j][2]);
                    }
                }
                if (BATCHED && h == 0 && threadIdx.x < F) s_delta[threadIdx.x] = run - ex;
                lds_barrier();
#pragma unroll
                for (int k = 0; k < PT_ITEMS / 2; ++k) {
                    const uint32_t i = k * PT_THREADS + tid, gi = h * HALF + i;
                    if (gi < total) {
                        const uint32_t v = s_k[i];
                        const uint2    c = s_p[i];
                        const uint32_t g = s_delta[pass_digit(pp, v, mask)] + gi;
                        if constexpr (AOS) {
                            uint32_t* o = out.w[0] + (size_t)g * 3u;
                            o[0] = v;
                            o[1] = c.x;
                            o[2] = c.y;
                            if (pp.side_out) pp.side_out[g] = (uint16_t)((v >> pp.next_shift) & pp.next_mask);
                        } else {
                            out.w[0][g] = v;
                            reinterpret_cast<uint2*>(out.w[1])[g] = c;
                        }
                    }
                }
                lds_barrier();
            }
            continue;
        }
#pragma unroll
        for (int j = 0; j < PT_ITEMS; ++j)
            if (dr[j] != 0xffffffffu) s_stage[dr[j]] = w[j][0];
        if (threadIdx.x < F) s_delta[threadIdx.x] = run - ex;
        lds_barrier();
        uint32_t dest[PT_ITEMS];
#pragma unroll
        for (int k = 0; k < PT_ITEMS; ++k) {
            const uint32_t i = k * PT_THREADS + tid;
            dest[k] = 0;
            if (i < total) {
                const uint32_t v = s_stage[i];
                dest[k] = s_delta[pass_digit(pp, v, mask)] + i;
                out.w[0][dest[k]] = v;
            }
        }
        lds_barrier();
#pragma unroll
        for (int a = 1; a < NW; ++a) {
            if constexpr (PAIR >= 0) {
                if (a == PAIR + 1) continue;
                if (a == PAIR) {
#pragma unroll
                    for (int j = 0; j < PT_ITEMS; ++j)
                        if (dr[j] != 0xffffffffu)
                            s_stage2[dr[j]] = make_uint2(w[j][a], w[j][a + 1 < NW ? a + 1 : a]);
                    lds_barrier();
                    uint2* dst2 = reinterpret_cast<uint2*>(out.w[a]);
#pragma unroll
                    for (int k = 0; k < PT_ITEMS; ++k) {
                        const uint32_t i = k * PT_THREADS + tid;
                        if (i < total) dst2[dest[k]] = s_stage2[i];
                    }
                    lds_barrier();
                    continue;
                }
            }
#pragma unroll
            for (int j = 0; j < PT_ITEMS; ++j)
                if (dr[j] != 0xffffffffu) s_stage[dr[j]] = w[j][a];
            lds_barrier();
            uint32_t* dst = out.w[a];
#pragma unroll
            for (int k = 0; k < PT_ITEMS; ++k) {
                const uint32_t i = k * PT_THREADS + tid;
                if (i < total) dst[dest[k]] = s_stage[i];
            }
            lds_barrier();
        }
    }
}

template <class Loader, bool BLK_OUT = false>
__global__ __launch_bounds__(PT_THREADS) void k_pass_scatter_packed(Loader ld, PassParams pp, uint2* out) {
    __shared__ uint2    s_stage[PT_TILE];
    __shared__ uint32_t s_cnt[PT_MAXF];
    __shared__ uint32_t s_base[PT_MAXF];
    __shared__ uint32_t s_delta[PT_MAXF];
    __shared__ uint32_t s_wsum[PT_THREADS / 64];
    uint32_t            seg, begin, end;
    if (!group_range(pp, blockIdx.x, seg, begin, end)) return;
    const uint32_t F = 1u << pp.fanout_log2, mask = F - 1u;

    uint32_t run = 0;
    uint32_t w[PT_ITEMS][2];
    uint32_t ok_raw = ld.template issue_tile<2>(begin, end, w);
    for (uint32_t base = begin; base < end; base += PT_TILE) {
        for (uint32_t d = threadIdx.x; d < F; d += PT_THREADS) s_cnt[d] = 0;
        lds_barrier();

        uint32_t       dr[PT_ITEMS];
        const uint32_t ok = ld.template finish_tile<2>(base, end, ok_raw, w);
#pragma unroll
        for (int j = 0; j < PT_ITEMS; ++j) {
            dr[j] = 0xffffffffu;
            if ((ok >> j) & 1u) {
                uint32_t d = pass_digit(pp, w[j][0], mask);
                uint32_t r = atomicAdd(&s_cnt[d], 1u);
                dr[j] = (d << 16) | r;
            }
        }
        lds_barrier();

        uint32_t c = threadIdx.x < F ? s_cnt[threadIdx.x] : 0u;
        if (c)
            run = atomicAdd(&pp.cursor[(((size_t)seg * F + threadIdx.x) << pp.xcd_log2) |
                                       (blockIdx.x & ((1u << pp.xcd_log2) - 1u))], c);
        uint32_t total;
        uint32_t ex = block_excl_scan(c, s_wsum, total);
        if (threadIdx.x < F) s_base[threadIdx.x] = ex;
        lds_barrier();

#pragma unroll
        for (int j = 0; j < PT_ITEMS; ++j)
            if (dr[j] != 0xffffffffu)
                s_stage[s_base[dr[j] >> 16] + (dr[j] & 0xffffu)] = make_uint2(w[j][0], w[j][1]);
        if (base + PT_TILE < end) ok_raw = ld.template issue_tile<2>(base + PT_TILE, end, w);
        if (threadIdx.x < F) s_delta[threadIdx.x] = run - ex;
        lds_barrier();

#pragma unroll
        for (int k = 0; k < PT_ITEMS; ++k) {
            const uint32_t i = k * PT_THREADS + threadIdx.x;
            if (i < total) {
                const uint2    v = s_stage[i];
                const uint32_t g = s_delta[pass_digit(pp, v.x, mask)] + i;
                if constexpr (BLK_OUT) {
                    uint32_t* o = reinterpret_cast<uint32_t*>(out) + BlockedLoader::key_at(g);
                    o[0] = v.x;
                    o[BlockedLoader::BLK] = v.y;
                } else {
                    out[g] = v;
                }
                if (pp.side_out) pp.side_out[g] = (uint16_t)((v.x >> pp.next_shift) & pp.next_mask);
            }
        }
    }
}

__global__ void k_heavy_tasks(const uint32_t* offR, const uint32_t* offS, uint32_t NP,
                              uint32_t* tasks, uint32_t* n_heavy, uint32_t max_tasks) {
    uint32_t q = blockIdx.x * blockDim.x + threadIdx.x;
    if (q >= NP) return;
    uint32_t sb = offS[q], se = offS[q + 1];
    uint32_t len = se - sb;
    if (len <= JN_HEAVY || offR[q + 1] == offR[q]) return;
    uint32_t nt = (len + JN_HEAVY - 1) / JN_HEAVY;
    uint32_t b = atomicAdd(n_heavy, nt);
    for (uint32_t t = 0; t < nt; ++t) {
        uint32_t k = b + t;
        if (k >= max_tasks) break;
        tasks[3 * k + 0] = q;
        tasks[3 * k + 1] = (uint32_t)((uint64_t)sb + (uint64_t)t * JN_HEAVY);
        tasks[3 * k + 2] = (uint32_t)min((uint64_t)se, (uint64_t)sb + (uint64_t)(t + 1) * JN_HEAVY);
    }
}

void launch_scan_bins(const Launch& L, const uint32_t* in, uint32_t n, uint32_t* off,
                      uint32_t* cursor) {
    RJ_KLAUNCH(L, "scan_bins", (k_scan_bins<0>), 1, 1024, in, (const uint32_t*)nullptr, n, 1u, off, cursor);
}

void launch_scan_segments(const Launch& L, const uint32_t* hist, const uint32_t* seg_off,
                          uint32_t nseg, uint32_t F, uint32_t xcd_log2, uint32_t* off, uint32_t* cursor) {
    RJ_KLAUNCH(L, "scan_segments", k_scan_segments, nseg, PT_MAXF, hist, seg_off, nseg, F, xcd_log2, off,
               cursor);
}

void launch_group_table(const Launch& L, const uint32_t* seg_off, uint32_t nseg,
                        uint32_t group_tuples, uint32_t* grp_start, const uint32_t* seg_end) {
    RJ_KLAUNCH(L, "group_table", (k_scan_bins<1>), 1, 1024, seg_off, seg_end, nseg, group_tuples, grp_start,
               (uint32_t*)nullptr);
}

void launch_pass_hist_src(const Launch& L, const TupleSrc& src, int key_words, const PassParams& pp,
                          uint32_t n_groups) {
    if (!n_groups) return;
    if (key_words == 1) {
        SrcLoader<1, 0> ld{src};
        RJ_KLAUNCH(L, "pass1_hist", (k_pass_hist<SrcLoader<1, 0>>), n_groups, PT_THREADS, ld, pp);
    } else {
        SrcLoader<2, 0> ld{src};
        RJ_KLAUNCH(L, "pass1_hist", (k_pass_hist<SrcLoader<2, 0>>), n_groups, PT_THREADS, ld, pp);
    }
}

void launch_fine_hist_src(const Launch& L, const TupleSrc& src, int key_words, uint32_t shift,
                          uint32_t b1, uint32_t b2, uint32_t grid, uint32_t* fine, uint32_t xcd_tpg,
                          uint32_t* coarse_x) {
    if (!grid || !src.n_rows) return;
    if (key_words == 1) {
        SrcLoader<1, 0> ld{src};
        RJ_KLAUNCH(L, "pass1_hist", (k_fine_hist<SrcLoader<1, 0>>), grid, PT_THREADS, ld, src.n_rows,
                   shift, b1, b2, fine, xcd_tpg, coarse_x);
    } else {
        SrcLoader<2, 0> ld{src};
        RJ_KLAUNCH(L, "pass1_hist", (k_fine_hist<SrcLoader<2, 0>>), grid, PT_THREADS, ld, src.n_rows,
                   shift, b1, b2, fine, xcd_tpg, coarse_x);
    }
}

void launch_fine_hist_words(const Launch& L, const Words& in, bool packed, uint32_t n, uint32_t shift,
                            uint32_t b1, uint32_t b2, uint32_t grid, uint32_t* fine, uint32_t xcd_tpg,
                            uint32_t* coarse_x) {
    if (!grid || !n) return;
    if (packed) {
        PackedLoader ld{reinterpret_cast<const uint2*>(in.w[0])};
        RJ_KLAUNCH(L, "pass1_hist", (k_fine_hist<PackedLoader>), grid, PT_THREADS, ld, n, shift, b1, b2, fine,
                   xcd_tpg, coarse_x);
    } else {
        DenseLoader ld{in};
        RJ_KLAUNCH(L, "pass1_hist", (k_fine_hist<DenseLoader>), grid, PT_THREADS, ld, n, shift, b1, b2, fine,
                   xcd_tpg, coarse_x);
    }
}

void launch_scan_fine(const Launch& L, const uint32_t* fine, uint32_t F1, uint32_t F2,
                      uint32_t* off2, uint32_t* cursor2, uint32_t* off1, uint32_t* cursor1,
                      const uint32_t* coarse_x) {
    RJ_KLAUNCH(L, "scan_fine", k_scan_fine, F1, PT_MAXF, fine, F1, F2, off2, cursor2, off1, cursor1,
               coarse_x);
}

template <int KW, int CW, int WIDE = WIDE_NONE>
static void scatter_src_t(const Launch& L, const TupleSrc& src, const PassParams& pp,
                          uint32_t n_groups, const Words& out) {
    SrcLoader<KW, CW, WIDE> ld{src};
    RJ_KLAUNCH(L, "pass1_scatter", (k_pass_scatter<KW + CW, SrcLoader<KW, CW, WIDE>, (CW >= 2 ? KW + CW - 2 : -1), false>),
               n_groups, PT_THREADS, ld, pp, out);
}

void launch_pass_scatter_src(const Launch& L, const TupleSrc& src, int key_words, int carry_words,
                             const PassParams& pp, uint32_t n_groups, const Words& out, bool aos3) {
    if (!n_groups) return;
    const int wide = src.carry_mode == CARRY_WIDE ? src.wide : WIDE_NONE;
    if (aos3) {
        if (key_words != 1 || carry_words != 2) launch_failed("pass1_scatter", "12-byte tuples need KW=1, CW=2", true);
        if (wide == WIDE_32S) {
            SrcLoader<1, 2, WIDE_32S> ld{src};
            RJ_KLAUNCH(L, "pass1_scatter", (k_pass_scatter<3, SrcLoader<1, 2, WIDE_32S>, 1, true>), n_groups, PT_THREADS, ld, pp, out);
            return;
        }
        SrcLoader<1, 2> ld{src};
        RJ_KLAUNCH(L, "pass1_scatter", (k_pass_scatter<3, SrcLoader<1, 2>, 1, true>), n_groups, PT_THREADS, ld, pp, out);
        return;
    }
    if (wide != WIDE_NONE) {
        switch (key_words * 100 + carry_words * 10 + wide) {
        case 121: scatter_src_t<1, 2, WIDE_32S>(L, src, pp, n_groups, out); break;
        case 131: scatter_src_t<1, 3, WIDE_32S>(L, src, pp, n_groups, out); break;
        case 132: scatter_src_t<1, 3, WIDE_64_32>(L, src, pp, n_groups, out); break;
        case 221: scatter_src_t<2, 2, WIDE_32S>(L, src, pp, n_groups, out); break;
        default: launch_failed("pass1_scatter", "no kernel for this wide carry layout", true);
        }
        return;
    }
    for_shape("pass1_scatter", key_words, carry_words, [&](auto KW, auto CW) {
        if constexpr (CW <= 2)
            scatter_src_t<KW, CW>(L, src, pp, n_groups, out);
        else
            launch_failed("pass1_scatter", "no kernel for this key/carry word count", true);
    });
}

void launch_pass_hist_dense(const Launch& L, const Words& in, const PassParams& pp,
                            uint32_t n_groups) {
    if (!n_groups) return;
    DenseLoader ld{in};
    RJ_KLAUNCH(L, "pass2_hist", (k_pass_hist<DenseLoader>), n_groups, PT_THREADS, ld, pp);
}

void launch_pass_scatter_dense(const Launch& L, const Words& in, int n_words, int pair_word,
                               const PassParams& pp, uint32_t n_groups, const Words& out, bool aos3) {
    if (!n_groups) return;
    if (aos3) {
        if (n_words != 3 || pair_word != 1) launch_failed("pass2_scatter", "12-byte tuples need KW=1, CW=2", true);
        RJ_KLAUNCH(L, "pass2_scatter", (k_pass_scatter<3, DenseLoaderT<1>, 1, true>), n_groups, PT_THREADS,
                   DenseLoaderT<1>{in}, pp, out);
        return;
    }
    switch (n_words * 10 + (pair_word < 0 ? 9 : pair_word)) {
    case 19:
        RJ_KLAUNCH(L, "pass2_scatter", (k_pass_scatter<1, DenseLoader, -1, false>), n_groups, PT_THREADS,
                   DenseLoader{in}, pp, out);
        break;
    case 29:
        RJ_KLAUNCH(L, "pass2_scatter", (k_pass_scatter<2, DenseLoader, -1, false>), n_groups, PT_THREADS,
                   DenseLoader{in}, pp, out);
        break;
    case 39:
        RJ_KLAUNCH(L, "pass2_scatter", (k_pass_scatter<3, DenseLoader, -1, false>), n_groups, PT_THREADS,
                   DenseLoader{in}, pp, out);
        break;
    case 31:
        RJ_KLAUNCH(L, "pass2_scatter", (k_pass_scatter<3, DenseLoaderT<1>, 1, false>), n_groups, PT_THREADS,
                   DenseLoaderT<1>{in}, pp, out);
        break;
    case 42:
        RJ_KLAUNCH(L, "pass2_scatter", (k_pass_scatter<4, DenseLoaderT<2>, 2, false>), n_groups, PT_THREADS,
                   DenseLoaderT<2>{in}, pp, out);
        break;
    default: launch_failed("pass2_scatter", "no kernel for this word layout", true);
    }
}

void launch_pass_hist_digits(const Launch& L, const uint16_t* digits, const PassParams& pp, uint32_t n_groups) {
    if (!n_groups) return;
    DigitLoader ld{digits, pp.shift};
    RJ_KLAUNCH(L, "pass2_hist", (k_pass_hist<DigitLoader>), n_groups, PT_THREADS, ld, pp);
}

void launch_pass_hist_aos3(const Launch& L, const uint32_t* in_tuples, const PassParams& pp, uint32_t n_groups) {
    if (!n_groups) return;
    RJ_KLAUNCH(L, "pass2_hist", (k_pass_hist<Aos3KeyLoader>), n_groups, PT_THREADS, Aos3KeyLoader{in_tuples}, pp);
}

void launch_pass_scatter_aos3(const Launch& L, const uint32_t* in_tuples, const PassParams& pp, uint32_t n_groups,
                              uint32_t* out_tuples) {
    if (!n_groups) return;
    Words out{};
    out.w[0] = out_tuples;
    RJ_KLAUNCH(L, "pass2_scatter", (k_pass_scatter<3, Aos3Loader, 1, true>), n_groups, PT_THREADS,
               Aos3Loader{in_tuples}, pp, out);
}

void launch_pass_hist_packed(const Launch& L, const uint32_t* in_pairs, const PassParams& pp,
                             uint32_t n_groups) {
    if (!n_groups) return;
    PackedLoader ld{reinterpret_cast<const uint2*>(in_pairs)};
    RJ_KLAUNCH(L, "pass2_hist", (k_pass_hist<PackedLoader>), n_groups, PT_THREADS, ld, pp);
}

void launch_pass_scatter_src_packed(const Launch& L, const TupleSrc& src, const PassParams& pp,
                                    uint32_t n_groups, uint32_t* out_pairs, bool blocked_out) {
    if (!n_groups) return;
    SrcLoader<1, 1> ld{src};
    if (blocked_out)
        RJ_KLAUNCH(L, "pass1_scatter", (k_pass_scatter_packed<SrcLoader<1, 1>, true>), n_groups, PT_THREADS, ld,
                   pp, reinterpret_cast<uint2*>(out_pairs));
    else
        RJ_KLAUNCH(L, "pass1_scatter", (k_pass_scatter_packed<SrcLoader<1, 1>>), n_groups, PT_THREADS, ld,
                   pp, reinterpret_cast<uint2*>(out_pairs));
}

void launch_pass_hist_blocked(const Launch& L, const uint32_t* in_blocked, const PassParams& pp, uint32_t n_groups) {
    if (!n_groups) return;
    RJ_KLAUNCH(L, "pass2_hist", (k_pass_hist<BlockedLoader>), n_groups, PT_THREADS, BlockedLoader{in_blocked}, pp);
}
void launch_pass_scatter_blocked(const Launch& L, const uint32_t* in_blocked, const PassParams& pp, uint32_t n_groups,
                                 uint32_t* out_pairs, bool blocked_out) {
    if (!n_groups) return;
    BlockedLoader ld{in_blocked};
    if (blocked_out)
        RJ_KLAUNCH(L, "pass2_scatter", (k_pass_scatter_packed<BlockedLoader, true>), n_groups, PT_THREADS, ld, pp,
                   reinterpret_cast<uint2*>(out_pairs));
    else
        RJ_KLAUNCH(L, "pass2_scatter", (k_pass_scatter_packed<BlockedLoader>), n_groups, PT_THREADS, ld, pp,
                   reinterpret_cast<uint2*>(out_pairs));
}

void launch_pass_scatter_packed(const Launch& L, const uint32_t* in_pairs, const PassParams& pp,
                                uint32_t n_groups, uint32_t* out_pairs) {
    if (!n_groups) return;
    PackedLoader ld{reinterpret_cast<const uint2*>(in_pairs)};
    RJ_KLAUNCH(L, "pass2_scatter", (k_pass_scatter_packed<PackedLoader>), n_groups, PT_THREADS, ld, pp,
               reinterpret_cast<uint2*>(out_pairs));
}

void launch_heavy_tasks(const Launch& L, const uint32_t* offR, const uint32_t* offS, uint32_t NP,
                        uint32_t* tasks, uint32_t* n_heavy, uint32_t max_tasks) {
    RJ_KLAUNCH(L, "heavy_tasks", k_heavy_tasks, (NP + 255) / 256, 256, offR, offS, NP, tasks,
               n_heavy, max_tasks);
}

void prewarm_partition(const Launch& L, uint32_t* zeroed) {
    RJ_KLAUNCH(L, "prewarm", k_heavy_tasks, 1, 256, zeroed, zeroed, 0u, zeroed, zeroed, 0u);
}

}
```

Measured before the change: 33.02 billion.

## Add speculative first partition pass with sampled histogram capacities and exact fallback

Replaces the exact histogram pass of the first radix pass with a sampled histogram. Each output sub-range gets a statistically bounded capacity, and the scatter claims space with a 64-bit atomic that tracks both the cursor and the remaining room. If any range overflows, a flag is set and the join redoes the partition exactly after reading back the counters. The aim is to skip one full read of the input (the first histogram pass). In exchange it over-allocates the intermediate buffer, makes the second pass read 8x more segments with explicit ends, and adds a host read-back plus a retry path.

```diff
diff --git a/radix-join_amd/csrc/rj_context.hip b/radix-join_amd/csrc/rj_context.hip
--- a/radix-join_amd/csrc/rj_context.hip
+++ b/radix-join_amd/csrc/rj_context.hip
@@ -1,5 +1,6 @@
 #include <dlfcn.h>
 
+#include <algorithm>
 #include <chrono>
 #include <cstdlib>
 
@@ -30,6 +31,10 @@
     tpg2 = env_int("RJ_TUNE_TPG2", tpg2);
     packed_side = env_int("RJ_TUNE_PACKED_SIDE", packed_side);
     xcd_min_rows = env_int("RJ_TUNE_XCD_MIN_ROWS", xcd_min_rows);
+    spec_p1 = env_int("RJ_TUNE_SPEC_P1", spec_p1);
+    spec_min_rows = env_int("RJ_TUNE_SPEC_MIN_ROWS", spec_min_rows);
+    spec_sample = std::min(5, std::max(1, env_int("RJ_TUNE_SPEC_SAMPLE", spec_sample)));
+    spec_z = std::max(0, env_int("RJ_TUNE_SPEC_Z", spec_z));
     bcast = env_int("RJ_TUNE_BCAST", bcast);
     diag = env_int("RJ_DIAG", diag);
     varchar_dev_rows = env_int("RJ_TUNE_VARCHAR_DEV", varchar_dev_rows);
diff --git a/radix-join_amd/csrc/rj_device.hpp b/radix-join_amd/csrc/rj_device.hpp
--- a/radix-join_amd/csrc/rj_device.hpp
+++ b/radix-join_amd/csrc/rj_device.hpp
@@ -105,6 +105,14 @@
     if (pp.hi_shift) return (((w >> pp.shift) & ((1u << pp.lo_bits) - 1u)) | ((w >> pp.hi_shift) << pp.lo_bits)) & mask;
     return (w >> pp.shift) & mask;
 }
+
+constexpr uint32_t SPEC_BINS = (1u << PT_MAXBITS) * 8u;
+struct SpecParams {
+    unsigned long long* cursor;
+    uint32_t*           flag;
+    uint32_t            sink;
+    uint32_t            sample_log2;
+};
 
 #ifndef RJ_JN_THREADS
 #define RJ_JN_THREADS 512
diff --git a/radix-join_amd/csrc/rj_exec.hip b/radix-join_amd/csrc/rj_exec.hip
--- a/radix-join_amd/csrc/rj_exec.hip
+++ b/radix-join_amd/csrc/rj_exec.hip
@@ -1,5 +1,6 @@
 #include <algorithm>
 #include <chrono>
+#include <cmath>
 #include <cstdlib>
 #include <functional>
 #include <set>
@@ -65,6 +66,7 @@
     bool     packed = false;
     bool     aos3 = false;
     uint64_t n_tuples = 0;
+    bool     spec = false;
 };
 
 struct WordSrc {
@@ -426,7 +428,7 @@
     Parted partition(const TupleSrc* srcp, const WordSrc* ws, int KW, int CW, uint32_t bits,
                      uint32_t shift0 = 0, bool single_pass = false, const Words* external = nullptr,
                      const std::function<void(const uint32_t*)>* after_offsets = nullptr,
-                     const PassShape* shape = nullptr) {
+                     const PassShape* shape = nullptr, uint32_t* spec_flag = nullptr) {
         Parted P;
         const bool preseg = shape && shape->nseg > 0;
         P.NW = KW + CW;
@@ -472,6 +474,21 @@
             for (uint32_t k = 0; k < std::min<uint32_t>(passes - 1, 2); ++k)
                 SIDE[k] = ctx->buf(std::max<uint64_t>(n, 1) * 2 + 16);
         const int pair_word = CW >= 2 ? KW + CW - 2 : -1;
+        const uint32_t spec_s = (uint32_t)ctx->tune.spec_sample;
+        const double   spec_z = ctx->tune.spec_z / 10.0;
+        uint64_t       spec_cap_max = 0;
+        {
+            const double Bn = (double)((uint64_t)8 << pbits[0]);
+            const double C = (double)((n + PT_TILE - 1) / PT_TILE) * (double)(PT_TILE >> spec_s);
+            const double bound = std::ldexp(C + spec_z * std::sqrt(Bn * (C + Bn)) + 0.5 * spec_z * spec_z * Bn, (int)spec_s) + 32.0 * Bn;
+            spec_cap_max = bound < 4.0e9 ? (((uint64_t)std::ceil(bound) + 255u) & ~(uint64_t)255u) : ~(uint64_t)0 >> 1;
+        }
+        const bool spec = spec_flag && ctx->tune.spec_p1 != 0 && passes == 2 && !fine && !ws && !external && !shape &&
+                          !after_offsets && !aos_mid && !packed_side && ctx->tune.mall_chunk <= 0 && ctx->tune.xcd_split &&
+                          n >= (uint64_t)ctx->tune.xcd_min_rows && n >= (uint64_t)ctx->tune.spec_min_rows &&
+                          spec_cap_max < (uint64_t(1) << 31) && n < (uint64_t(1) << 31);
+        P.spec = spec;
+        const uint64_t n_first_out = spec ? spec_cap_max + PT_TILE : n;
         for (int a = 0; a < (P.packed ? 1 : P.NW); ++a) {
             if (pair_word >= 0 && a == pair_word + 1) continue;
             const uint64_t wbytes = (P.packed || a == pair_word) ? 8 : 4;
@@ -480,7 +497,7 @@
                 continue;
             }
             if ((P.aos3 && passes == 1) || aos_mid) continue;
-            A[a] = ctx->buf(n * wbytes + 2048);
+            A[a] = ctx->buf(n_first_out * wbytes + 2048);
             wa.w[a] = A[a]->as<uint32_t>();
             if (passes > (P.aos3 ? 2u : 1u)) {
                 B[a] = ctx->buf(n * wbytes + 2048);
@@ -492,6 +509,7 @@
         Words    cur = ws ? ws->w : Words{}, nxt = (P.aos3 && passes == 1) ? waos : wa;
         bool     cur_is_a = false;
         BufP       fine_off, fine_cursor, coarse_off, coarse_cursor;
+        BufP       spec_start, spec_limit, spec_end;
         uint32_t tpg_first = tiles_per_group(n, 4096);
         if (ctx->tune.tpg1 > 0) tpg_first = (uint32_t)ctx->tune.tpg1;
         bool fine_xcd = false;
@@ -543,10 +561,11 @@
             pp.fanout_log2 = pbits[p];
             uint32_t n_groups;
             BufP     grp_start;
-            const bool      first_preseg = p == 0 && preseg;
-            const uint32_t  nseg_in = first_preseg ? shape->nseg : nseg;
+            const bool      first_preseg = p == 0 && preseg, spec_in = p == 1 && spec;
+            const uint32_t  nseg_in = first_preseg ? shape->nseg : (spec_in ? nseg << 3 : nseg);
             const uint32_t  n_oseg = first_preseg ? shape->n_oseg : nseg;
             const uint64_t  bins = (uint64_t)n_oseg * F;
+            const uint32_t* in_end = first_preseg ? shape->seg_end : (spec_in ? spec_end->as<uint32_t>() : nullptr);
             if (p == 0 && shape && shape->hi_shift) {
                 pp.hi_shift = shape->hi_shift;
                 pp.lo_bits = shape->lo_bits;
@@ -556,7 +575,7 @@
                 uint64_t gt = (uint64_t)pp.tiles_per_group * PT_TILE;
                 n_groups = (uint32_t)((n + gt - 1) / gt);
             } else {
-                pp.tiles_per_group = tiles_per_group(n / nseg_in + 1, 16);
+                pp.tiles_per_group = tiles_per_group(n / (spec_in ? n_oseg : nseg_in) + 1, 16);
                 if (P.aos3 && p + 1 == passes) pp.tiles_per_group = std::min<uint32_t>(pp.tiles_per_group, 2u);
                 uint64_t gt = (uint64_t)pp.tiles_per_group * PT_TILE;
                 if (ctx->tune.tpg2 > 0) {
@@ -568,18 +587,36 @@
                     pp.xcd_remap = 1;
                     n_groups += 8;
                 }
-                const uint32_t* in_off = first_preseg ? shape->seg_begin : seg_off->as<uint32_t>();
+                const uint32_t* in_off = first_preseg ? shape->seg_begin : (spec_in ? spec_start->as<uint32_t>() : seg_off->as<uint32_t>());
                 grp_start = ctx->buf(((uint64_t)nseg_in + 1) * 4);
-                launch_group_table(L, in_off, nseg_in, (uint32_t)gt, grp_start->as<uint32_t>(),
-                                   first_preseg ? shape->seg_end : nullptr);
+                launch_group_table(L, in_off, nseg_in, (uint32_t)gt, grp_start->as<uint32_t>(), in_end);
                 pp.nseg = nseg_in;
                 pp.seg_off = in_off;
-                pp.seg_end = first_preseg ? shape->seg_end : nullptr;
-                pp.oseg_shift = first_preseg ? shape->oseg_shift : 0u;
+                pp.seg_end = in_end;
+                pp.oseg_shift = first_preseg ? shape->oseg_shift : (spec_in ? 3u : 0u);
                 pp.grp_start = grp_start->as<uint32_t>();
             }
             BufP off, hist, cursor;
-            if (fine) {
+            SpecParams sp{};
+            if (p == 0 && spec) {
+                pp.xcd_log2 = 3u;
+                const uint32_t nb = (uint32_t)bins << 3;
+                hist = ctx->buf((uint64_t)nb * 4);
+                off = ctx->buf((bins + 1) * 4);
+                cursor = ctx->buf((uint64_t)nb * 8);
+                spec_start = ctx->buf((uint64_t)nb * 4);
+                spec_limit = ctx->buf((uint64_t)nb * 4);
+                spec_end = ctx->buf((uint64_t)nb * 4);
+                RJ_HIP(hipMemsetAsync(hist->p, 0, (uint64_t)nb * 4, ctx->stream));
+                pp.hist = hist->as<uint32_t>();
+                sp.cursor = cursor->as<unsigned long long>();
+                sp.flag = spec_flag;
+                sp.sink = (uint32_t)spec_cap_max;
+                sp.sample_log2 = spec_s;
+                launch_pass_sample_src(L, src, KW, pp, sp, n_groups);
+                launch_spec_caps(L, pp.hist, nb, spec_s, (float)spec_z, (uint32_t)spec_cap_max, spec_start->as<uint32_t>(),
+                                 spec_limit->as<uint32_t>(), sp.cursor);
+            } else if (fine) {
                 off = p == 0 ? coarse_off : fine_off;
                 cursor = p == 0 ? coarse_cursor : fine_cursor;
                 pp.cursor = cursor->as<uint32_t>();
@@ -646,7 +683,8 @@
                     launch_pass_hist_packed(L, cur.w[0], pp, n_groups);
                 else
                     launch_pass_hist_dense(L, cur, pp, n_groups);
-                launch_scan_segments(L, pp.hist, first_preseg ? shape->oseg_off : (p == 0 ? nullptr : pp.seg_off),
+                launch_scan_segments(L, pp.hist,
+                                     first_preseg ? shape->oseg_off : (p == 0 ? nullptr : (spec_in ? seg_off->as<uint32_t>() : pp.seg_off)),
                                      n_oseg, F, pp.xcd_log2, off->as<uint32_t>(), pp.cursor);
             }
             if (p == 0 && after_offsets) (*after_offsets)(off->as<uint32_t>());
@@ -680,16 +718,21 @@
                 }
                 const bool blk_out = blocked_mid && p + 1 < passes;
                 if (p == 0 && !ws)
-                    launch_pass_scatter_src_packed(L, src, pp, n_groups, nxt.w[0], blk_out);
+                    launch_pass_scatter_src_packed(L, src, pp, n_groups, nxt.w[0], blk_out, p == 0 && spec ? &sp : nullptr);
                 else if (blocked_mid)
                     launch_pass_scatter_blocked(L, cur.w[0], pp, n_groups, nxt.w[0], blk_out);
                 else
                     launch_pass_scatter_packed(L, cur.w[0], pp, n_groups, nxt.w[0]);
             } else if (p == 0 && !ws) {
-                launch_pass_scatter_src(L, src, KW, CW, pp, n_groups, nxt, P.aos3 && p + 1 == passes);
+                launch_pass_scatter_src(L, src, KW, CW, pp, n_groups, nxt, P.aos3 && p + 1 == passes, p == 0 && spec ? &sp : nullptr);
             } else {
                 launch_pass_scatter_dense(L, cur, P.NW, pair_word, pp, n_groups, nxt,
                                           P.aos3 && p + 1 == passes);
+            }
+            if (p == 0 && spec) {
+                launch_spec_close(L, sp.cursor, spec_start->as<uint32_t>(), spec_limit->as<uint32_t>(), F, spec_end->as<uint32_t>(),
+                                  off->as<uint32_t>());
+                if (ctx->tune.diag >= 1) spec_report(cursor, spec_limit, spec_start, (uint32_t)bins << 3, n, n_first_out);
             }
             seg_off = off;
             nseg = (uint32_t)bins;
@@ -710,6 +753,23 @@
         if (shape && !shape->prior_bits.empty()) P.pbits.insert(P.pbits.begin(), shape->prior_bits.begin(), shape->prior_bits.end());
         P.n_tuples = n;
         return P;
+    }
+
+    void spec_report(const BufP& cursor, const BufP& limit, const BufP& start, uint32_t nb, uint64_t n, uint64_t n_alloc) {
+        std::vector<unsigned long long> c(nb);
+        std::vector<uint32_t>           lim(nb), st(nb);
+        read_back(c.data(), cursor->p, (size_t)nb * 8);
+        read_back(lim.data(), limit->p, (size_t)nb * 4);
+        read_back(st.data(), start->p, (size_t)nb * 4);
+        double   worst = 0;
+        uint32_t over = 0;
+        for (uint32_t i = 0; i < nb; ++i) {
+            const double used = (double)((uint32_t)c[i] - st[i]), room = (double)(lim[i] - st[i]);
+            if (used > room) ++over;
+            if (room > 0) worst = std::max(worst, used / room);
+        }
+        fprintf(stderr, "[rj diag] speculative pass 1: rows=%llu sub-ranges=%u fullest=%.4f of its capacity, over=%u, room for %llu tuples (+%.3f)\n",
+                (unsigned long long)n, nb, worst, over, (unsigned long long)n_alloc, (double)n_alloc / (double)std::max<uint64_t>(n, 1) - 1.0);
     }
 
     struct Side {
@@ -937,12 +997,34 @@
         BufP     tasks;
         uint32_t max_tasks = 0;
     };
-    CoParts partition_sides(JoinState& st, const JoinSpec& js, uint32_t bits) {
+    CoParts partition_sides(JoinState& st, const JoinSpec& js, uint32_t bits, const BufP* counters = nullptr) {
         CoParts        cp;
         const TupleSrc sb = make_src(st, st.bs(), js), sp = make_src(st, st.ps(), js);
-        cp.B = partition(&sb, nullptr, st.KW, st.bs().CW, bits);
-        cp.P = partition(&sp, nullptr, st.KW, st.ps().CW, bits);
+        uint32_t*      fl = counters ? (*counters)->as<uint32_t>() + 4 : nullptr;
+        cp.B = partition(&sb, nullptr, st.KW, st.bs().CW, bits, 0, false, nullptr, nullptr, nullptr, fl);
+        cp.P = partition(&sp, nullptr, st.KW, st.ps().CW, bits, 0, false, nullptr, nullptr, nullptr, fl ? fl + 1 : nullptr);
         return cp;
+    }
+    int  spec_fallbacks = 0;
+    void repartition_exact(JoinState& st, const JoinSpec& js, uint32_t bits, CoParts& cp, const BufP& counters, bool flag_b,
+                           bool flag_p) {
+        ++spec_fallbacks;
+        if (ctx->tune.diag >= 1)
+            fprintf(stderr, "[rj diag] %s: speculative pass 1 overflowed (build side %d, probe side %d): exact partition again (fallback %d of this plan)\n",
+                    st.kind->name, (int)flag_b, (int)flag_p, spec_fallbacks);
+        if (flag_b) {
+            const TupleSrc sb = make_src(st, st.bs(), js);
+            cp.B = Parted();
+            cp.B = partition(&sb, nullptr, st.KW, st.bs().CW, bits);
+        }
+        if (flag_p) {
+            const TupleSrc sp = make_src(st, st.ps(), js);
+            cp.P = Parted();
+            cp.P = partition(&sp, nullptr, st.KW, st.ps().CW, bits);
+        }
+        RJ_HIP(hipMemsetAsync(counters->as<uint32_t>() + 4, 0, 8, ctx->stream));
+        cp.tasks = BufP();
+        heavy_tasks(cp, counters);
     }
     void heavy_tasks(CoParts& cp, const BufP& counters) {
         cp.max_tasks = (uint32_t)(2 * (cp.P.n_tuples / JN_HEAVY) + 2);
@@ -950,13 +1032,14 @@
         launch_heavy_tasks_zeroed(cp.B, cp.P, cp.tasks, counters, cp.max_tasks);
     }
     CoParts co_partition(JoinState& st, const JoinSpec& js, uint32_t bits, const BufP& counters) {
-        CoParts cp = partition_sides(st, js, bits);
+        CoParts cp = partition_sides(st, js, bits, &counters);
         heavy_tasks(cp, counters);
         return cp;
     }
+    static constexpr size_t COUNTER_BYTES = 32;
     BufP zeroed_counters() {
-        BufP counters = ctx->buf(16);
-        RJ_HIP(hipMemsetAsync(counters->p, 0, 16, ctx->stream));
+        BufP counters = ctx->buf(COUNTER_BYTES);
+        RJ_HIP(hipMemsetAsync(counters->p, 0, COUNTER_BYTES, ctx->stream));
         return counters;
     }
     template <class Params>
@@ -990,9 +1073,11 @@
         std::set<void*> finished;
     };
     template <class LaunchFn>
-    Emitted emit_with_retry(JoinState& st, const BufP& counters, uint64_t cap, LaunchFn&& launch) {
+    Emitted emit_with_retry(JoinState& st, const BufP& counters, uint64_t cap, LaunchFn&& launch,
+                            const std::function<void(bool, bool)>& respec = nullptr) {
         const JoinKind& K = *st.kind;
         Emitted         e;
+        const uint64_t  cap0 = cap;
         e.key_mode = st.need_key_stream ? stream_mode_of(st.is_root, st.KW * 4, true) : ST_NONE;
         for (int attempt = 1;; ++attempt) {
             e.key_stream = e.key_mode != ST_NONE ? ctx->buf(stream_bytes(e.key_mode, cap)) : BufP();
@@ -1003,7 +1088,19 @@
             e.finished.clear();
             finish_paged_streams(st, e, counters, cap);
             unsigned long long h = 0;
-            read_back(&h, counters->p, 8);
+            if (respec) {
+                uint32_t hw[6] = {};
+                read_back(hw, counters->p, sizeof hw);
+                if (hw[4] | hw[5]) {
+                    respec(hw[4] != 0, hw[5] != 0);
+                    cap = cap0;
+                    attempt = 0;
+                    continue;
+                }
+                h = (unsigned long long)hw[0] | ((unsigned long long)hw[1] << 32);
+            } else {
+                read_back(&h, counters->p, 8);
+            }
             e.nrows = h;
             if (e.nrows <= cap) return e;
             if (K.attempts == 1)
@@ -1029,15 +1126,20 @@
             fprintf(stderr, "[rj diag] join build=%llu probe=%llu bits=%u cw=%d/%d\n",
                     (unsigned long long)bs.rel->n, (unsigned long long)ps.rel->n, bits, bs.CW, ps.CW);
         if (broadcast_form(st, js)) return join_finish(st, js, nullptr, bits, root_res);
-        CoParts cp = partition_sides(st, js, bits);
-        return join_finish(st, js, &cp, bits, root_res);
-    }
-
-    Rel join_finish(JoinState& st, const JoinSpec& js, CoParts* cp, uint32_t bits, Result* root_res) {
+        BufP    counters = zeroed_counters();
+        CoParts cp = partition_sides(st, js, bits, &counters);
+        return join_finish(st, js, &cp, bits, root_res, counters);
+    }
+
+    Rel join_finish(JoinState& st, const JoinSpec& js, CoParts* cp, uint32_t bits, Result* root_res,
+                    const BufP& spec_counters = BufP()) {
         Side &    bs = st.bs(), &ps = st.ps();
         const int KW = st.KW;
-        BufP counters = ctx->buf(16);
+        BufP counters = spec_counters ? spec_counters : ctx->buf(COUNTER_BYTES);
         if (cp) heavy_tasks(*cp, counters);
+        std::function<void(bool, bool)> respec;
+        if (cp && spec_counters && (cp->B.spec || cp->P.spec))
+            respec = [&](bool fb, bool fpr) { repartition_exact(st, js, bits, *cp, counters, fb, fpr); };
         plan_carry_streams(st);
         Emitted e = emit_with_retry(st, counters, first_cap(st.cap_hint), [&](const OutStream& key, uint64_t cap) {
             if (!cp) {
@@ -1090,7 +1192,7 @@
                     fprintf(stderr, "[rj diag]   %-16s %6.1f %%  %8.0f cyc/wg\n", names[i],
                             100.0 * hd[i] / tot, (double)hd[i] / PB.NP);
             }
-        });
+        }, respec);
         if (st.vkey && e.nrows) e.nrows = verify_varchar_pairs(st, e.nrows);
         return join_assemble(st, js, e, root_res);
     }
@@ -1131,8 +1233,7 @@
         BufP counters = zeroed_counters();
         fp.out_cursor = counters->as<unsigned long long>();
         CoParts cp;
-        if (!bcast) {
-            cp = co_partition(st, js, bits, counters);
+        auto    bind_parts = [&]() {
             set_heavy(fp, cp, counters, bits);
             fp.Fw = cp.B.w;
             fp.Pw = cp.P.w;
@@ -1140,7 +1241,17 @@
             fp.offP = cp.P.off->as<uint32_t>();
             fp.packP = cp.P.packed ? 1 : 0;
             fp.aosP = cp.P.aos3 ? 1 : 0;
-        }
+        };
+        if (!bcast) {
+            cp = co_partition(st, js, bits, counters);
+            bind_parts();
+        }
+        std::function<void(bool, bool)> respec;
+        if (cp.B.spec || cp.P.spec)
+            respec = [&](bool fb, bool fpr) {
+                repartition_exact(st, js, bits, cp, counters, fb, fpr);
+                bind_parts();
+            };
         Emitted e = emit_with_retry(st, counters, ps.rel->n, [&](const OutStream& key, uint64_t cap) {
             fp.key = key;
             fp.pc = out_stream(ps);
@@ -1152,7 +1263,7 @@
                 if (anti && (fp.P.key.valid || fp.P.key_f64))
                     launch_filter_nullkeys(L, KW, ps.CW, fp, stride_grid(ps.rel->n));
             }
-        });
+        }, respec);
         return join_assemble(st, js, e, root_res);
     }
 
@@ -1240,6 +1351,13 @@
             fp.flags = flags->as<uint32_t>();
             fp.use_flags = bcast ? 1 : 0;
         }
+        std::function<void(bool, bool)> respec;
+        if (cp.B.spec || cp.P.spec)
+            respec = [&](bool fb, bool fpr) {
+                repartition_exact(st, js, bits, cp, counters, fb, fpr);
+                set_parts(op, cp, counters, bits);
+                if (flags) RJ_HIP(hipMemsetAsync(flags->p, 0, ((cp.B.n_tuples) / 32 + 2) * 4, ctx->stream));
+            };
         const uint32_t probe_grid = stride_grid(ps.rel->n), build_grid = stride_grid(bs.rel->n);
         const uint64_t rows0 = std::max(st.cap_hint, full ? bs.rel->n + ps.rel->n : ps.rel->n);
         Emitted e = emit_with_retry(st, counters, first_cap(rows0), [&](const OutStream& key, uint64_t cap) {
@@ -1263,7 +1381,7 @@
                 if (probe_dropped) launch_outer_nullkeys(L, KW, ps.CW, op, probe_grid);
                 if (op.B.key.valid || op.B.key_f64) launch_full_buildrows(L, KW, bs.CW, fp, build_grid);
             }
-        });
+        }, respec);
         return join_assemble(st, js, e, root_res);
     }
 
diff --git a/radix-join_amd/csrc/rj_internal.hpp b/radix-join_amd/csrc/rj_internal.hpp
--- a/radix-join_amd/csrc/rj_internal.hpp
+++ b/radix-join_amd/csrc/rj_internal.hpp
@@ -183,6 +183,10 @@
     int tpg2 = 0;
     int xcd_min_rows = 40 << 20;
     int xcd_split = 1;
+    int spec_p1 = 1;
+    int spec_min_rows = 40 << 20;
+    int spec_sample = 5;
+    int spec_z = 60;
     int bcast = 1;
     int diag = 0;
     int varchar_dev_rows = 200000;
diff --git a/radix-join_amd/csrc/rj_kernels.hpp b/radix-join_amd/csrc/rj_kernels.hpp
--- a/radix-join_amd/csrc/rj_kernels.hpp
+++ b/radix-join_amd/csrc/rj_kernels.hpp
@@ -55,7 +55,14 @@
                       uint32_t* off2, uint32_t* cursor2, uint32_t* off1, uint32_t* cursor1,
                       const uint32_t* coarse_x = nullptr);
 void launch_pass_scatter_src(const Launch& L, const TupleSrc& src, int key_words, int carry_words,
-                             const PassParams& pp, uint32_t n_groups, const Words& out, bool aos3 = false);
+                             const PassParams& pp, uint32_t n_groups, const Words& out, bool aos3 = false,
+                             const SpecParams* spec = nullptr);
+void launch_pass_sample_src(const Launch& L, const TupleSrc& src, int key_words, const PassParams& pp,
+                            const SpecParams& sp, uint32_t n_groups);
+void launch_spec_caps(const Launch& L, const uint32_t* sample, uint32_t nbins, uint32_t sample_log2, float z,
+                      uint32_t cap_max, uint32_t* start, uint32_t* limit, unsigned long long* cursor);
+void launch_spec_close(const Launch& L, const unsigned long long* cursor, const uint32_t* start, const uint32_t* limit,
+                       uint32_t F, uint32_t* seg_end, uint32_t* oseg_off);
 void launch_pass_hist_dense(const Launch& L, const Words& in, const PassParams& pp,
                             uint32_t n_groups);
 void launch_pass_scatter_dense(const Launch& L, const Words& in, int n_words, int pair_word,
@@ -69,7 +76,8 @@
 void launch_pass_hist_packed(const Launch& L, const uint32_t* in_pairs, const PassParams& pp,
                              uint32_t n_groups);
 void launch_pass_scatter_src_packed(const Launch& L, const TupleSrc& src, const PassParams& pp,
-                                    uint32_t n_groups, uint32_t* out_pairs, bool blocked_out = false);
+                                    uint32_t n_groups, uint32_t* out_pairs, bool blocked_out = false,
+                                    const SpecParams* spec = nullptr);
 void launch_pass_hist_blocked(const Launch& L, const uint32_t* in_blocked, const PassParams& pp, uint32_t n_groups);
 void launch_pass_scatter_blocked(const Launch& L, const uint32_t* in_blocked, const PassParams& pp, uint32_t n_groups,
                                  uint32_t* out_pairs, bool blocked_out);
diff --git a/radix-join_amd/csrc/rj_partition.hip b/radix-join_amd/csrc/rj_partition.hip
--- a/radix-join_amd/csrc/rj_partition.hip
+++ b/radix-join_amd/csrc/rj_partition.hip
@@ -662,6 +662,108 @@
         uint32_t c = s_h[d];
         if (c) atomicAdd(&pp.hist[(((size_t)seg * F + d) << pp.xcd_log2) | (blockIdx.x & ((1u << pp.xcd_log2) - 1u))], c);
     }
+}
+
+static_assert((PT_TILE & (PT_TILE - 1)) == 0, "a tile's sample slice is a power-of-two fraction of it");
+template <int KW>
+__global__ __launch_bounds__(PT_THREADS) void k_pass_sample(TupleSrc s, PassParams pp, SpecParams sp) {
+    __shared__ uint32_t s_h[PT_MAXF];
+    uint32_t            seg, begin, end;
+    if (!group_range(pp, blockIdx.x, seg, begin, end)) return;
+    const uint32_t F = 1u << pp.fanout_log2, mask = F - 1u;
+    for (uint32_t d = threadIdx.x; d < F; d += PT_THREADS) s_h[d] = 0;
+    lds_barrier();
+    const uint32_t slog = (uint32_t)__builtin_ctz((unsigned)PT_TILE) - sp.sample_log2, slice = 1u << slog;
+    const uint32_t ntiles = (end - begin + (uint32_t)PT_TILE - 1u) / (uint32_t)PT_TILE;
+    const uint32_t total = ntiles << slog;
+    constexpr int  U = 4;
+    for (uint32_t i0 = threadIdx.x; i0 < total; i0 += U * PT_THREADS) {
+        uint32_t lo[U], hi[U];
+        bool     ok[U];
+#pragma unroll
+        for (int u = 0; u < U; ++u) {
+            const uint32_t i = i0 + u * PT_THREADS, ic = min(i, total - 1u);
+            const uint32_t t = ic >> slog, r = ic & (slice - 1u);
+            const uint32_t tb = begin + t * (uint32_t)PT_TILE, rows = min((uint32_t)PT_TILE, end - tb);
+            const uint32_t rot = ((tb / (uint32_t)PT_TILE) * 7u << slog) & ((uint32_t)PT_TILE - 1u);
+            const uint32_t at = rows > slice ? min(rot, rows - slice) : 0u;
+            const uint32_t row = tb + min(at + r, rows - 1u);
+            ok[u] = i < total && r < rows;
+            if constexpr (KW == 1) {
+                lo[u] = col_load32(s.key, row);
+                hi[u] = 0;
+            } else {
+                const uint64_t k = col_load64(s.key, row);
+                lo[u] = (uint32_t)k;
+                hi[u] = (uint32_t)(k >> 32);
+            }
+            if (s.key.valid && !s.key.valid[row]) ok[u] = false;
+        }
+#pragma unroll
+        for (int u = 0; u < U; ++u) {
+            uint32_t h;
+            if constexpr (KW == 1) {
+                h = s.prehashed ? lo[u] : fmix32(lo[u]);
+            } else {
+                const uint64_t k = (uint64_t)lo[u] | ((uint64_t)hi[u] << 32);
+                if (s.key_f64 && (k & 0x7ff0000000000000ull) == 0x7ff0000000000000ull && (k & 0x000fffffffffffffull))
+                    ok[u] = false;
+                h = (uint32_t)fmix64(k);
+            }
+            if (ok[u]) atomicAdd(&s_h[pass_digit(pp, h, mask)], 1u);
+        }
+    }
+    lds_barrier();
+    for (uint32_t d = threadIdx.x; d < F; d += PT_THREADS) {
+        uint32_t c = s_h[d];
+        if (c) atomicAdd(&pp.hist[(((size_t)seg * F + d) << pp.xcd_log2) | (blockIdx.x & ((1u << pp.xcd_log2) - 1u))], c);
+    }
+}
+
+__global__ __launch_bounds__(1024) void k_spec_caps(const uint32_t* sample, uint32_t nbins, uint32_t sample_log2, float z,
+                                                    uint32_t cap_max, uint32_t* start, uint32_t* limit,
+                                                    unsigned long long* cursor) {
+    __shared__ unsigned long long s_sum[1024];
+    const uint32_t                chunk = (nbins + 1023u) / 1024u;
+    const uint32_t                b = min(nbins, threadIdx.x * chunk), e = min(nbins, b + chunk);
+    auto                          cap_of = [&](uint32_t c) -> unsigned long long {
+        const double zz = (double)z, x = (double)c + zz * sqrt((double)c + 1.0) + 0.5 * zz * zz;
+        const unsigned long long t = (unsigned long long)ceil(ldexp(x, (int)sample_log2));
+        return (t + 31ull) & ~31ull;
+    };
+    unsigned long long sum = 0;
+    for (uint32_t i = b; i < e; ++i) sum += cap_of(sample[i]);
+    s_sum[threadIdx.x] = sum;
+    __syncthreads();
+    unsigned long long run = 0;
+    for (uint32_t k = 0; k < threadIdx.x; ++k) run += s_sum[k];
+    for (uint32_t i = b; i < e; ++i) {
+        const unsigned long long nx = run + cap_of(sample[i]);
+        const uint32_t           st = (uint32_t)min(run, (unsigned long long)cap_max);
+        const uint32_t           lim = (uint32_t)min(nx, (unsigned long long)cap_max);
+        start[i] = st;
+        limit[i] = lim;
+        cursor[i] = (unsigned long long)st | ((unsigned long long)(lim - st) << 32);
+        run = nx;
+    }
+}
+
+__global__ __launch_bounds__(PT_MAXF) void k_spec_close(const unsigned long long* cursor, const uint32_t* start,
+                                                        const uint32_t* limit, uint32_t F, uint32_t* seg_end,
+                                                        uint32_t* oseg_off) {
+    __shared__ uint32_t s_wsum[PT_MAXF / 64];
+    const uint32_t      d = threadIdx.x;
+    uint32_t            v = 0;
+    if (d < F)
+        for (uint32_t x = 0; x < 8; ++x) {
+            const uint32_t i = (d << 3) | x, en = min((uint32_t)cursor[i], limit[i]);
+            seg_end[i] = en;
+            v += en - start[i];
+        }
+    uint32_t       total;
+    const uint32_t ex = block_excl_scan(v, s_wsum, total);
+    if (d < F) oseg_off[d] = ex;
+    if (d == 0) oseg_off[F] = total;
 }
 
 template <class Loader>
@@ -802,220 +904,26 @@
 
 template <int NW, class Loader, int PAIR, bool AOS>
 __global__ __launch_bounds__(PT_THREADS) void k_pass_scatter(Loader ld, PassParams pp, Words out) {
-    static_assert(PAIR < 0 || (PAIR >= 1 && PAIR + 1 < NW), "pair = two carry words behind the key");
-    static_assert(!AOS || (NW == 3 && PAIR == 1), "12-byte tuples: one key word + a two-word carry");
-    __shared__ uint2    s_stage2[PT_TILE];
-    uint32_t* const     s_stage = reinterpret_cast<uint32_t*>(s_stage2);
-    __shared__ uint32_t s_cnt[PT_MAXF + PT_DUMMY];
-    __shared__ uint32_t s_base[PT_MAXF];
-    __shared__ uint32_t s_delta[PT_MAXF];
-    __shared__ uint32_t s_wsum[PT_THREADS / 64];
-    uint32_t            seg, begin, end;
-    if (!group_range(pp, blockIdx.x, seg, begin, end)) return;
-    const uint32_t F = 1u << pp.fanout_log2, mask = F - 1u;
-
-    uint32_t run = 0;
-    uint32_t w[PT_ITEMS][NW];
-
-    for (uint32_t base = begin; base < end; base += PT_TILE) {
-        for (uint32_t d = threadIdx.x; d < F; d += PT_THREADS) s_cnt[d] = 0;
-        lds_barrier();
-
-        const uint32_t ok = ld.template load_tile<NW>(base, end, w);
-        constexpr bool BATCHED = NW == 3 && PAIR == 1 && is_src_loader<Loader>::value;
-        uint32_t       ps[PT_ITEMS / 2];
-        uint32_t       dr[PT_ITEMS];
-        if constexpr (BATCHED) {
-            rank_tile<NW>(pp, mask, ok, w, s_cnt, ps);
-        } else {
-#pragma unroll
-            for (int j = 0; j < PT_ITEMS; ++j) {
-                dr[j] = 0xffffffffu;
-                if ((ok >> j) & 1u) {
-                    uint32_t d = pass_digit(pp, w[j][0], mask);
-                    uint32_t r = atomicAdd(&s_cnt[d], 1u);
-                    dr[j] = (d << 16) | r;
-                }
-            }
-        }
-        lds_barrier();
-
-        uint32_t c = threadIdx.x < F ? s_cnt[threadIdx.x] : 0u;
-        if (c) {
-            run = atomicAdd(&pp.cursor[(((size_t)seg * F + threadIdx.x) << pp.xcd_log2) |
-                                       (blockIdx.x & ((1u << pp.xcd_log2) - 1u))], c);
-        }
-        uint32_t total;
-        uint32_t ex = block_excl_scan(c, s_wsum, total);
-        if (threadIdx.x < F) s_base[threadIdx.x] = ex;
-        lds_barrier();
-
-        if constexpr (BATCHED) {
-            place_tile<NW>(pp, mask, ok, w, s_base, ps);
-        } else {
-#pragma unroll
-            for (int j = 0; j < PT_ITEMS; ++j)
-                if (dr[j] != 0xffffffffu) dr[j] = s_base[dr[j] >> 16] + (dr[j] & 0xffffu);
-        }
-
-        const uint32_t tid = BATCHED ? tile_tid() : threadIdx.x;
-        if constexpr (NW == 3 && PAIR == 1) {
-            constexpr uint32_t HALF = PT_TILE / 2;
-            uint2* const       s_p = s_stage2;
-            uint32_t* const    s_k = reinterpret_cast<uint32_t*>(s_stage2 + HALF);
-            if (!BATCHED && threadIdx.x < F) s_delta[threadIdx.x] = run - ex;
-#pragma unroll
-            for (int h = 0; h < 2; ++h) {
-#pragma unroll
-                for (int j = 0; j < PT_ITEMS; ++j) {
-                    const uint32_t lp = (BATCHED ? tile_pos(ps, j) : dr[j]) - h * HALF;
-                    if (lp < HALF) {
-                        s_k[lp] = w[j][0];
-                        s_p[lp] = make_uint2(w[j][1], w[j][2]);
-                    }
-                }
-                if (BATCHED && h == 0 && threadIdx.x < F) s_delta[threadIdx.x] = run - ex;
-                lds_barrier();
-#pragma unroll
-                for (int k = 0; k < PT_ITEMS / 2; ++k) {
-                    const uint32_t i = k * PT_THREADS + tid, gi = h * HALF + i;
-                    if (gi < total) {
-                        const uint32_t v = s_k[i];
-                        const uint2    c = s_p[i];
-                        const uint32_t g = s_delta[pass_digit(pp, v, mask)] + gi;
-                        if constexpr (AOS) {
-                            uint32_t* o = out.w[0] + (size_t)g * 3u;
-                            o[0] = v;
-                            o[1] = c.x;
-                            o[2] = c.y;
-                            if (pp.side_out) pp.side_out[g] = (uint16_t)((v >> pp.next_shift) & pp.next_mask);
-                        } else {
-                            out.w[0][g] = v;
-                            reinterpret_cast<uint2*>(out.w[1])[g] = c;
-                        }
-                    }
-                }
-                lds_barrier();
-            }
-            continue;
-        }
-#pragma unroll
-        for (int j = 0; j < PT_ITEMS; ++j)
-            if (dr[j] != 0xffffffffu) s_stage[dr[j]] = w[j][0];
-        if (threadIdx.x < F) s_delta[threadIdx.x] = run - ex;
-        lds_barrier();
-        uint32_t dest[PT_ITEMS];
-#pragma unroll
-        for (int k = 0; k < PT_ITEMS; ++k) {
-            const uint32_t i = k * PT_THREADS + tid;
-            dest[k] = 0;
-            if (i < total) {
-                const uint32_t v = s_stage[i];
-                dest[k] = s_delta[pass_digit(pp, v, mask)] + i;
-                out.w[0][dest[k]] = v;
-            }
-        }
-        lds_barrier();
-#pragma unroll
-        for (int a = 1; a < NW; ++a) {
-            if constexpr (PAIR >= 0) {
-                if (a == PAIR + 1) continue;
-                if (a == PAIR) {
-#pragma unroll
-                    for (int j = 0; j < PT_ITEMS; ++j)
-                        if (dr[j] != 0xffffffffu)
-                            s_stage2[dr[j]] = make_uint2(w[j][a], w[j][a + 1 < NW ? a + 1 : a]);
-                    lds_barrier();
-                    uint2* dst2 = reinterpret_cast<uint2*>(out.w[a]);
-#pragma unroll
-                    for (int k = 0; k < PT_ITEMS; ++k) {
-                        const uint32_t i = k * PT_THREADS + tid;
-                        if (i < total) dst2[dest[k]] = s_stage2[i];
-                    }
-                    lds_barrier();
-                    continue;
-                }
-            }
-#pragma unroll
-            for (int j = 0; j < PT_ITEMS; ++j)
-                if (dr[j] != 0xffffffffu) s_stage[dr[j]] = w[j][a];
-            lds_barrier();
-            uint32_t* dst = out.w[a];
-#pragma unroll
-            for (int k = 0; k < PT_ITEMS; ++k) {
-                const uint32_t i = k * PT_THREADS + tid;
-                if (i < total) dst[dest[k]] = s_stage[i];
-            }
-            lds_barrier();
-        }
-    }
+    constexpr bool       SPEC = false;
+    constexpr SpecParams sp{};
+#include "rj_pass_scatter.inc"
+}
+template <int NW, class Loader, int PAIR>
+__global__ __launch_bounds__(PT_THREADS) void k_spec_scatter(Loader ld, PassParams pp, Words out, SpecParams sp) {
+    constexpr bool SPEC = true, AOS = false;
+#include "rj_pass_scatter.inc"
 }
 
 template <class Loader, bool BLK_OUT = false>
 __global__ __launch_bounds__(PT_THREADS) void k_pass_scatter_packed(Loader ld, PassParams pp, uint2* out) {
-    __shared__ uint2    s_stage[PT_TILE];
-    __shared__ uint32_t s_cnt[PT_MAXF];
-    __shared__ uint32_t s_base[PT_MAXF];
-    __shared__ uint32_t s_delta[PT_MAXF];
-    __shared__ uint32_t s_wsum[PT_THREADS / 64];
-    uint32_t            seg, begin, end;
-    if (!group_range(pp, blockIdx.x, seg, begin, end)) return;
-    const uint32_t F = 1u << pp.fanout_log2, mask = F - 1u;
-
-    uint32_t run = 0;
-    uint32_t w[PT_ITEMS][2];
-    uint32_t ok_raw = ld.template issue_tile<2>(begin, end, w);
-    for (uint32_t base = begin; base < end; base += PT_TILE) {
-        for (uint32_t d = threadIdx.x; d < F; d += PT_THREADS) s_cnt[d] = 0;
-        lds_barrier();
-
-        uint32_t       dr[PT_ITEMS];
-        const uint32_t ok = ld.template finish_tile<2>(base, end, ok_raw, w);
-#pragma unroll
-        for (int j = 0; j < PT_ITEMS; ++j) {
-            dr[j] = 0xffffffffu;
-            if ((ok >> j) & 1u) {
-                uint32_t d = pass_digit(pp, w[j][0], mask);
-                uint32_t r = atomicAdd(&s_cnt[d], 1u);
-                dr[j] = (d << 16) | r;
-            }
-        }
-        lds_barrier();
-
-        uint32_t c = threadIdx.x < F ? s_cnt[threadIdx.x] : 0u;
-        if (c)
-            run = atomicAdd(&pp.cursor[(((size_t)seg * F + threadIdx.x) << pp.xcd_log2) |
-                                       (blockIdx.x & ((1u << pp.xcd_log2) - 1u))], c);
-        uint32_t total;
-        uint32_t ex = block_excl_scan(c, s_wsum, total);
-        if (threadIdx.x < F) s_base[threadIdx.x] = ex;
-        lds_barrier();
-
-#pragma unroll
-        for (int j = 0; j < PT_ITEMS; ++j)
-            if (dr[j] != 0xffffffffu)
-                s_stage[s_base[dr[j] >> 16] + (dr[j] & 0xffffu)] = make_uint2(w[j][0], w[j][1]);
-        if (base + PT_TILE < end) ok_raw = ld.template issue_tile<2>(base + PT_TILE, end, w);
-        if (threadIdx.x < F) s_delta[threadIdx.x] = run - ex;
-        lds_barrier();
-
-#pragma unroll
-        for (int k = 0; k < PT_ITEMS; ++k) {
-            const uint32_t i = k * PT_THREADS + threadIdx.x;
-            if (i < total) {
-                const uint2    v = s_stage[i];
-                const uint32_t g = s_delta[pass_digit(pp, v.x, mask)] + i;
-                if constexpr (BLK_OUT) {
-                    uint32_t* o = reinterpret_cast<uint32_t*>(out) + BlockedLoader::key_at(g);
-                    o[0] = v.x;
-                    o[BlockedLoader::BLK] = v.y;
-                } else {
-                    out[g] = v;
-                }
-                if (pp.side_out) pp.side_out[g] = (uint16_t)((v.x >> pp.next_shift) & pp.next_mask);
-            }
-        }
-    }
+    constexpr bool       SPEC = false;
+    constexpr SpecParams sp{};
+#include "rj_pass_scatter_packed.inc"
+}
+template <class Loader, bool BLK_OUT>
+__global__ __launch_bounds__(PT_THREADS) void k_spec_scatter_packed(Loader ld, PassParams pp, uint2* out, SpecParams sp) {
+    constexpr bool SPEC = true;
+#include "rj_pass_scatter_packed.inc"
 }
 
 __global__ void k_heavy_tasks(const uint32_t* offR, const uint32_t* offS, uint32_t NP,
@@ -1065,6 +973,25 @@
     }
 }
 
+void launch_pass_sample_src(const Launch& L, const TupleSrc& src, int key_words, const PassParams& pp,
+                            const SpecParams& sp, uint32_t n_groups) {
+    if (!n_groups) return;
+    if (key_words == 1)
+        RJ_KLAUNCH(L, "pass1_sample", (k_pass_sample<1>), n_groups, PT_THREADS, src, pp, sp);
+    else
+        RJ_KLAUNCH(L, "pass1_sample", (k_pass_sample<2>), n_groups, PT_THREADS, src, pp, sp);
+}
+
+void launch_spec_caps(const Launch& L, const uint32_t* sample, uint32_t nbins, uint32_t sample_log2, float z,
+                      uint32_t cap_max, uint32_t* start, uint32_t* limit, unsigned long long* cursor) {
+    RJ_KLAUNCH(L, "spec_caps", k_spec_caps, 1, 1024, sample, nbins, sample_log2, z, cap_max, start, limit, cursor);
+}
+
+void launch_spec_close(const Launch& L, const unsigned long long* cursor, const uint32_t* start, const uint32_t* limit,
+                       uint32_t F, uint32_t* seg_end, uint32_t* oseg_off) {
+    RJ_KLAUNCH(L, "spec_close", k_spec_close, 1, PT_MAXF, cursor, start, limit, F, seg_end, oseg_off);
+}
+
 void launch_fine_hist_src(const Launch& L, const TupleSrc& src, int key_words, uint32_t shift,
                           uint32_t b1, uint32_t b2, uint32_t grid, uint32_t* fine, uint32_t xcd_tpg,
                           uint32_t* coarse_x) {
@@ -1104,17 +1031,23 @@
 
 template <int KW, int CW, int WIDE = WIDE_NONE>
 static void scatter_src_t(const Launch& L, const TupleSrc& src, const PassParams& pp,
-                          uint32_t n_groups, const Words& out) {
+                          uint32_t n_groups, const Words& out, const SpecParams* spec) {
     SrcLoader<KW, CW, WIDE> ld{src};
+    if (spec) {
+        RJ_KLAUNCH(L, "pass1_scatter", (k_spec_scatter<KW + CW, SrcLoader<KW, CW, WIDE>, (CW >= 2 ? KW + CW - 2 : -1)>),
+                   n_groups, PT_THREADS, ld, pp, out, *spec);
+        return;
+    }
     RJ_KLAUNCH(L, "pass1_scatter", (k_pass_scatter<KW + CW, SrcLoader<KW, CW, WIDE>, (CW >= 2 ? KW + CW - 2 : -1), false>),
                n_groups, PT_THREADS, ld, pp, out);
 }
 
 void launch_pass_scatter_src(const Launch& L, const TupleSrc& src, int key_words, int carry_words,
-                             const PassParams& pp, uint32_t n_groups, const Words& out, bool aos3) {
+                             const PassParams& pp, uint32_t n_groups, const Words& out, bool aos3, const SpecParams* spec) {
     if (!n_groups) return;
     const int wide = src.carry_mode == CARRY_WIDE ? src.wide : WIDE_NONE;
     if (aos3) {
+        if (spec) launch_failed("pass1_scatter", "no speculative kernel writes 12-byte tuples", true);
         if (key_words != 1 || carry_words != 2) launch_failed("pass1_scatter", "12-byte tuples need KW=1, CW=2", true);
         if (wide == WIDE_32S) {
             SrcLoader<1, 2, WIDE_32S> ld{src};
@@ -1127,17 +1060,17 @@
     }
     if (wide != WIDE_NONE) {
         switch (key_words * 100 + carry_words * 10 + wide) {
-        case 121: scatter_src_t<1, 2, WIDE_32S>(L, src, pp, n_groups, out); break;
-        case 131: scatter_src_t<1, 3, WIDE_32S>(L, src, pp, n_groups, out); break;
-        case 132: scatter_src_t<1, 3, WIDE_64_32>(L, src, pp, n_groups, out); break;
-        case 221: scatter_src_t<2, 2, WIDE_32S>(L, src, pp, n_groups, out); break;
+        case 121: scatter_src_t<1, 2, WIDE_32S>(L, src, pp, n_groups, out, spec); break;
+        case 131: scatter_src_t<1, 3, WIDE_32S>(L, src, pp, n_groups, out, spec); break;
+        case 132: scatter_src_t<1, 3, WIDE_64_32>(L, src, pp, n_groups, out, spec); break;
+        case 221: scatter_src_t<2, 2, WIDE_32S>(L, src, pp, n_groups, out, spec); break;
         default: launch_failed("pass1_scatter", "no kernel for this wide carry layout", true);
         }
         return;
     }
     for_shape("pass1_scatter", key_words, carry_words, [&](auto KW, auto CW) {
         if constexpr (CW <= 2)
-            scatter_src_t<KW, CW>(L, src, pp, n_groups, out);
+            scatter_src_t<KW, CW>(L, src, pp, n_groups, out, spec);
         else
             launch_failed("pass1_scatter", "no kernel for this key/carry word count", true);
     });
@@ -1212,9 +1145,18 @@
 }
 
 void launch_pass_scatter_src_packed(const Launch& L, const TupleSrc& src, const PassParams& pp,
-                                    uint32_t n_groups, uint32_t* out_pairs, bool blocked_out) {
+                                    uint32_t n_groups, uint32_t* out_pairs, bool blocked_out, const SpecParams* spec) {
     if (!n_groups) return;
     SrcLoader<1, 1> ld{src};
+    if (spec) {
+        if (blocked_out)
+            RJ_KLAUNCH(L, "pass1_scatter", (k_spec_scatter_packed<SrcLoader<1, 1>, true>), n_groups, PT_THREADS, ld,
+                       pp, reinterpret_cast<uint2*>(out_pairs), *spec);
+        else
+            RJ_KLAUNCH(L, "pass1_scatter", (k_spec_scatter_packed<SrcLoader<1, 1>, false>), n_groups, PT_THREADS, ld,
+                       pp, reinterpret_cast<uint2*>(out_pairs), *spec);
+        return;
+    }
     if (blocked_out)
         RJ_KLAUNCH(L, "pass1_scatter", (k_pass_scatter_packed<SrcLoader<1, 1>, true>), n_groups, PT_THREADS, ld,
                    pp, reinterpret_cast<uint2*>(out_pairs));
diff --git a/radix-join_amd/csrc/rj_pass_scatter.inc b/radix-join_amd/csrc/rj_pass_scatter.inc
--- /dev/null
+++ b/radix-join_amd/csrc/rj_pass_scatter.inc
@@ -0,0 +1,162 @@
+    static_assert(PAIR < 0 || (PAIR >= 1 && PAIR + 1 < NW), "pair = two carry words behind the key");
+    static_assert(!AOS || (NW == 3 && PAIR == 1), "12-byte tuples: one key word + a two-word carry");
+    __shared__ uint2    s_stage2[PT_TILE];
+    uint32_t* const     s_stage = reinterpret_cast<uint32_t*>(s_stage2);
+    __shared__ uint32_t s_cnt[PT_MAXF + PT_DUMMY];
+    __shared__ uint32_t s_base[PT_MAXF];
+    __shared__ uint32_t s_delta[PT_MAXF];
+    __shared__ uint32_t s_wsum[PT_THREADS / 64];
+    uint32_t            seg, begin, end;
+    if (!group_range(pp, blockIdx.x, seg, begin, end)) return;
+    const uint32_t F = 1u << pp.fanout_log2, mask = F - 1u;
+
+    uint32_t run = 0;
+    [[maybe_unused]] unsigned long long res = 0;
+    uint32_t w[PT_ITEMS][NW];
+
+    for (uint32_t base = begin; base < end; base += PT_TILE) {
+        for (uint32_t d = threadIdx.x; d < F; d += PT_THREADS) s_cnt[d] = 0;
+        lds_barrier();
+
+        const uint32_t ok = ld.template load_tile<NW>(base, end, w);
+        constexpr bool BATCHED = NW == 3 && PAIR == 1 && is_src_loader<Loader>::value;
+        uint32_t       ps[PT_ITEMS / 2];
+        uint32_t       dr[PT_ITEMS];
+        if constexpr (BATCHED) {
+            rank_tile<NW>(pp, mask, ok, w, s_cnt, ps);
+        } else {
+#pragma unroll
+            for (int j = 0; j < PT_ITEMS; ++j) {
+                dr[j] = 0xffffffffu;
+                if ((ok >> j) & 1u) {
+                    uint32_t d = pass_digit(pp, w[j][0], mask);
+                    uint32_t r = atomicAdd(&s_cnt[d], 1u);
+                    dr[j] = (d << 16) | r;
+                }
+            }
+        }
+        lds_barrier();
+
+        uint32_t c = threadIdx.x < F ? s_cnt[threadIdx.x] : 0u;
+        if (c) {
+            const size_t at = (((size_t)seg * F + threadIdx.x) << pp.xcd_log2) | (blockIdx.x & ((1u << pp.xcd_log2) - 1u));
+            if constexpr (SPEC)
+                res = atomicAdd(&sp.cursor[at], (unsigned long long)c | ((unsigned long long)(0u - c) << 32));
+            else
+                run = atomicAdd(&pp.cursor[at], c);
+        }
+        uint32_t total;
+        uint32_t ex = block_excl_scan(c, s_wsum, total);
+        if (threadIdx.x < F) s_base[threadIdx.x] = ex;
+        lds_barrier();
+        auto delta_of = [&]() -> uint32_t {
+            if constexpr (SPEC) {
+                if (c && (int32_t)(uint32_t)(res >> 32) < (int32_t)c) {
+                    atomicOr(sp.flag, 1u);
+                    return sp.sink;
+                }
+                return (uint32_t)res - ex;
+            } else {
+                return run - ex;
+            }
+        };
+
+        if constexpr (BATCHED) {
+            place_tile<NW>(pp, mask, ok, w, s_base, ps);
+        } else {
+#pragma unroll
+            for (int j = 0; j < PT_ITEMS; ++j)
+                if (dr[j] != 0xffffffffu) dr[j] = s_base[dr[j] >> 16] + (dr[j] & 0xffffu);
+        }
+
+        const uint32_t tid = BATCHED ? tile_tid() : threadIdx.x;
+        if constexpr (NW == 3 && PAIR == 1) {
+            constexpr uint32_t HALF = PT_TILE / 2;
+            uint2* const       s_p = s_stage2;
+            uint32_t* const    s_k = reinterpret_cast<uint32_t*>(s_stage2 + HALF);
+            if (!BATCHED && threadIdx.x < F) s_delta[threadIdx.x] = delta_of();
+#pragma unroll
+            for (int h = 0; h < 2; ++h) {
+#pragma unroll
+                for (int j = 0; j < PT_ITEMS; ++j) {
+                    const uint32_t lp = (BATCHED ? tile_pos(ps, j) : dr[j]) - h * HALF;
+                    if (lp < HALF) {
+                        s_k[lp] = w[j][0];
+                        s_p[lp] = make_uint2(w[j][1], w[j][2]);
+                    }
+                }
+                if (BATCHED && h == 0 && threadIdx.x < F) s_delta[threadIdx.x] = delta_of();
+                lds_barrier();
+#pragma unroll
+                for (int k = 0; k < PT_ITEMS / 2; ++k) {
+                    const uint32_t i = k * PT_THREADS + tid, gi = h * HALF + i;
+                    if (gi < total) {
+                        const uint32_t v = s_k[i];
+                        const uint2    c = s_p[i];
+                        const uint32_t g = s_delta[pass_digit(pp, v, mask)] + gi;
+                        if constexpr (AOS) {
+                            uint32_t* o = out.w[0] + (size_t)g * 3u;
+                            o[0] = v;
+                            o[1] = c.x;
+                            o[2] = c.y;
+                            if (pp.side_out) pp.side_out[g] = (uint16_t)((v >> pp.next_shift) & pp.next_mask);
+                        } else {
+                            out.w[0][g] = v;
+                            reinterpret_cast<uint2*>(out.w[1])[g] = c;
+                        }
+                    }
+                }
+                lds_barrier();
+            }
+            continue;
+        }
+#pragma unroll
+        for (int j = 0; j < PT_ITEMS; ++j)
+            if (dr[j] != 0xffffffffu) s_stage[dr[j]] = w[j][0];
+        if (threadIdx.x < F) s_delta[threadIdx.x] = delta_of();
+        lds_barrier();
+        uint32_t dest[PT_ITEMS];
+#pragma unroll
+        for (int k = 0; k < PT_ITEMS; ++k) {
+            const uint32_t i = k * PT_THREADS + tid;
+            dest[k] = 0;
+            if (i < total) {
+                const uint32_t v = s_stage[i];
+                dest[k] = s_delta[pass_digit(pp, v, mask)] + i;
+                out.w[0][dest[k]] = v;
+            }
+        }
+        lds_barrier();
+#pragma unroll
+        for (int a = 1; a < NW; ++a) {
+            if constexpr (PAIR >= 0) {
+                if (a == PAIR + 1) continue;
+                if (a == PAIR) {
+#pragma unroll
+                    for (int j = 0; j < PT_ITEMS; ++j)
+                        if (dr[j] != 0xffffffffu)
+                            s_stage2[dr[j]] = make_uint2(w[j][a], w[j][a + 1 < NW ? a + 1 : a]);
+                    lds_barrier();
+                    uint2* dst2 = reinterpret_cast<uint2*>(out.w[a]);
+#pragma unroll
+                    for (int k = 0; k < PT_ITEMS; ++k) {
+                        const uint32_t i = k * PT_THREADS + tid;
+                        if (i < total) dst2[dest[k]] = s_stage2[i];
+                    }
+                    lds_barrier();
+                    continue;
+                }
+            }
+#pragma unroll
+            for (int j = 0; j < PT_ITEMS; ++j)
+                if (dr[j] != 0xffffffffu) s_stage[dr[j]] = w[j][a];
+            lds_barrier();
+            uint32_t* dst = out.w[a];
+#pragma unroll
+            for (int k = 0; k < PT_ITEMS; ++k) {
+                const uint32_t i = k * PT_THREADS + tid;
+                if (i < total) dst[dest[k]] = s_stage[i];
+            }
+            lds_barrier();
+        }
+    }
diff --git a/radix-join_amd/csrc/rj_pass_scatter_packed.inc b/radix-join_amd/csrc/rj_pass_scatter_packed.inc
--- /dev/null
+++ b/radix-join_amd/csrc/rj_pass_scatter_packed.inc
@@ -0,0 +1,79 @@
+    __shared__ uint2    s_stage[PT_TILE];
+    __shared__ uint32_t s_cnt[PT_MAXF];
+    __shared__ uint32_t s_base[PT_MAXF];
+    __shared__ uint32_t s_delta[PT_MAXF];
+    __shared__ uint32_t s_wsum[PT_THREADS / 64];
+    uint32_t            seg, begin, end;
+    if (!group_range(pp, blockIdx.x, seg, begin, end)) return;
+    const uint32_t F = 1u << pp.fanout_log2, mask = F - 1u;
+
+    uint32_t run = 0;
+    [[maybe_unused]] unsigned long long res = 0;
+    uint32_t w[PT_ITEMS][2];
+    uint32_t ok_raw = ld.template issue_tile<2>(begin, end, w);
+    for (uint32_t base = begin; base < end; base += PT_TILE) {
+        for (uint32_t d = threadIdx.x; d < F; d += PT_THREADS) s_cnt[d] = 0;
+        lds_barrier();
+
+        uint32_t       dr[PT_ITEMS];
+        const uint32_t ok = ld.template finish_tile<2>(base, end, ok_raw, w);
+#pragma unroll
+        for (int j = 0; j < PT_ITEMS; ++j) {
+            dr[j] = 0xffffffffu;
+            if ((ok >> j) & 1u) {
+                uint32_t d = pass_digit(pp, w[j][0], mask);
+                uint32_t r = atomicAdd(&s_cnt[d], 1u);
+                dr[j] = (d << 16) | r;
+            }
+        }
+        lds_barrier();
+
+        uint32_t c = threadIdx.x < F ? s_cnt[threadIdx.x] : 0u;
+        if (c) {
+            const size_t at = (((size_t)seg * F + threadIdx.x) << pp.xcd_log2) | (blockIdx.x & ((1u << pp.xcd_log2) - 1u));
+            if constexpr (SPEC)
+                res = atomicAdd(&sp.cursor[at], (unsigned long long)c | ((unsigned long long)(0u - c) << 32));
+            else
+                run = atomicAdd(&pp.cursor[at], c);
+        }
+        uint32_t total;
+        uint32_t ex = block_excl_scan(c, s_wsum, total);
+        if (threadIdx.x < F) s_base[threadIdx.x] = ex;
+        lds_barrier();
+
+#pragma unroll
+        for (int j = 0; j < PT_ITEMS; ++j)
+            if (dr[j] != 0xffffffffu)
+                s_stage[s_base[dr[j] >> 16] + (dr[j] & 0xffffu)] = make_uint2(w[j][0], w[j][1]);
+        if (base + PT_TILE < end) ok_raw = ld.template issue_tile<2>(base + PT_TILE, end, w);
+        if (threadIdx.x < F) {
+            if constexpr (SPEC) {
+                if (c && (int32_t)(uint32_t)(res >> 32) < (int32_t)c) {
+                    atomicOr(sp.flag, 1u);
+                    s_delta[threadIdx.x] = sp.sink;
+                } else {
+                    s_delta[threadIdx.x] = (uint32_t)res - ex;
+                }
+            } else {
+                s_delta[threadIdx.x] = run - ex;
+            }
+        }
+        lds_barrier();
+
+#pragma unroll
+        for (int k = 0; k < PT_ITEMS; ++k) {
+            const uint32_t i = k * PT_THREADS + threadIdx.x;
+            if (i < total) {
+                const uint2    v = s_stage[i];
+                const uint32_t g = s_delta[pass_digit(pp, v.x, mask)] + i;
+                if constexpr (BLK_OUT) {
+                    uint32_t* o = reinterpret_cast<uint32_t*>(out) + BlockedLoader::key_at(g);
+                    o[0] = v.x;
+                    o[BlockedLoader::BLK] = v.y;
+                } else {
+                    out[g] = v;
+                }
+                if (pp.side_out) pp.side_out[g] = (uint16_t)((v.x >> pp.next_shift) & pp.next_mask);
+            }
+        }
+    }
```

Measured after the change: 33.92 billion (median of 6 runs). 1.03x the previous value.
